# THU-DA-6D-Pose-Group/GDR-Net

Hardware: NVIDIA B200
Metric: crops/sec (fwd+bwd, 256x256, bs64 per GPU) (higher is better)
Workload: dtype fp16x3 fwd / fp16 bwd, f32 accumulate

## Files before the change

### gdr_net_b200/csrc/elementwise.cu

```cuda
#include <stdlib.h>

#include "gdrn_internal.h"
#include "ptx.cuh"

namespace gdrn {

typedef __nv_bfloat16 bf16;

__device__ __forceinline__ void unpack8(const uint4& q, float (&f)[8]) {
    const uint32_t w[4] = {q.x, q.y, q.z, q.w};
#pragma unroll
    for (int j = 0; j < 4; ++j) {
        unpack_hi2(w[j], f[2 * j], f[2 * j + 1]);
    }
}
__device__ __forceinline__ void load8(const bf16* hi, const bf16* lo, long off8, float (&f)[8]) {
    unpack8(__ldg(reinterpret_cast<const uint4*>(hi) + off8), f);
    if (lo != nullptr) {
        const uint4 q = __ldg(reinterpret_cast<const uint4*>(lo) + off8);
        const uint32_t w[4] = {q.x, q.y, q.z, q.w};
#pragma unroll
        for (int j = 0; j < 4; ++j) {
            float a, b;
            unpack_lo2(w[j], a, b);
// ... 127 lines not shown
                    if (LO) unpack8_lo(rl[t], r);
#pragma unroll
                    for (int j = 0; j < 8; ++j) v[j] += r[j];
                }
                if (relu) {
                    if (mask_out != nullptr) {
                        uint32_t bits = 0;
#pragma unroll
                        for (int j = 0; j < 8; ++j) bits |= (v[j] > 0.f ? 1u : 0u) << j;
                        mask_out[it] = (uint8_t)bits;
                    }
#pragma unroll
                    for (int j = 0; j < 8; ++j) v[j] = fmaxf(v[j], 0.f);
                }
                store8(y_hi, LO ? y_lo : nullptr, it, v);
            }
        }
    }
}

template <bool LO, bool RES>
__global__ void __launch_bounds__(256, 4) bn_act_kernel(const bf16* __restrict__ x_hi, const bf16* __restrict__ x_lo,
                                                        const bf16* __restrict__ r_hi, const bf16* __restrict__ r_lo,
                                                        bf16* __restrict__ y_hi, bf16* __restrict__ y_lo,
                                                        const float* __restrict__ scale, const float* __restrict__ shift,
                                                        long rows, int C, int relu) {
    pdl_ew_entry();
    __shared__ float s_sc[512], s_sh[512];
    for (int c = threadIdx.x; c < C; c += blockDim.x) {
        s_sc[c] = scale[c];
        s_sh[c] = shift[c];
    }
    __syncthreads();
    bn_apply_loop<LO, RES>(x_hi, x_lo, r_hi, r_lo, y_hi, y_lo, s_sc, s_sh, rows * (C / 8), C / 8, relu, nullptr);
}

template <bool LO, bool RES>
__global__ void __launch_bounds__(256, 4) bn_fwd_kernel(const bf16* __restrict__ x_hi, const bf16* __restrict__ x_lo,
                                                        const bf16* __restrict__ r_hi, const bf16* __restrict__ r_lo,
                                                        bf16* __restrict__ y_hi, bf16* __restrict__ y_lo,
                                                        const float* __restrict__ stats, const float* __restrict__ gamma,
                                                        const float* __restrict__ beta, float* running_mean, float* running_var,
                                                        float* __restrict__ mean_out, float* __restrict__ invstd_out, long rows,
                                                        int C, float eps, float momentum, int train, int relu,
                                                        uint8_t* __restrict__ mask_out, int rev) {
    pdl_ew_entry();
    __shared__ float s_sc[512], s_sh[512];
    const float count = (float)rows;
    for (int c = threadIdx.x; c < C; c += blockDim.x) {
        float mean, var;
        if (train) {
            const double m = (double)stats[c] / count;
            double v = (double)stats[C + c] / count - m * m;
            if (v < 0) v = 0;
            mean = (float)m;
            var = (float)v;
        } else {
            mean = running_mean[c];
            var = running_var[c];
        }
        const float invstd = rsqrtf(var + eps);
        const float sc = gamma[c] * invstd;
        s_sc[c] = sc;
        s_sh[c] = beta[c] - mean * sc;
        if (blockIdx.x == 0) {
            if (mean_out != nullptr) {
                mean_out[c] = mean;
                invstd_out[c] = invstd;
            }
            if (train && running_mean != nullptr) {
                running_mean[c] = (1.f - momentum) * running_mean[c] + momentum * mean;
                const float unbiased = count > 1.f ? var * (count / (count - 1.f)) : var;
                running_var[c] = (1.f - momentum) * running_var[c] + momentum * unbiased;
            }
        }
    }
    __syncthreads();
    bn_apply_loop<LO, RES>(x_hi, x_lo, r_hi, r_lo, y_hi, y_lo, s_sc, s_sh, rows * (C / 8), C / 8, relu, mask_out, rev != 0);
}


struct Pix {
    int g, x, y, b;
};
__device__ __forceinline__ bool is_pow2(int v) { return v > 0 && (v & (v - 1)) == 0; }
__device__ __forceinline__ Pix decode_pix(long idx, int cg, int W, int H) {
    unsigned t = (unsigned)idx;
    Pix p;
    if (is_pow2(cg) && is_pow2(W) && is_pow2(H)) {
        const int lc = 31 - __clz(cg), lw = 31 - __clz(W), lh = 31 - __clz(H);
        p.g = (int)(t & (unsigned)(cg - 1));
        t >>= lc;
        p.x = (int)(t & (unsigned)(W - 1));
        t >>= lw;
        p.y = (int)(t & (unsigned)(H - 1));
        p.b = (int)(t >> lh);
        return p;
    }
    unsigned q = t / (unsigned)cg;
    p.g = (int)(t - q * (unsigned)cg);
    t = q;
    q = t / (unsigned)W;
    p.x = (int)(t - q * (unsigned)W);
    t = q;
    q = t / (unsigned)H;
    p.y = (int)(t - q * (unsigned)H);
    p.b = (int)q;
    return p;
}

__global__ void maxpool_fwd_kernel(const bf16* __restrict__ x_hi, const bf16* __restrict__ x_lo, bf16* __restrict__ y_hi,
                                   bf16* __restrict__ y_lo, uint8_t* __restrict__ arg_out, int B, int H, int W, int C) {
    pdl_ew_entry();
    const int cg = C / 8, Ho = H / 2, Wo = W / 2;
    const long total = (long)B * Ho * Wo * cg;
    for (long idx = blockIdx.x * (long)blockDim.x + threadIdx.x; idx < total; idx += (long)gridDim.x * blockDim.x) {
        const Pix px = decode_pix(idx, cg, Wo, Ho);
        const int g = px.g, ox = px.x, oy = px.y, b = px.b;
        float m[8];
        uint32_t arg[8];
#pragma unroll
        for (int j = 0; j < 8; ++j) {
            m[j] = -INFINITY;
            arg[j] = 0;
        }
#pragma unroll
        for (int dy = 0; dy < 3; ++dy) {
            const int iy = oy * 2 + dy - 1;
            if (iy < 0 || iy >= H) continue;
#pragma unroll
            for (int dx = 0; dx < 3; ++dx) {
                const int ix = ox * 2 + dx - 1;
                if (ix < 0 || ix >= W) continue;
                float v[8];
                load8(x_hi, x_lo, (((long)b * H + iy) * W + ix) * cg + g, v);
#pragma unroll
                for (int j = 0; j < 8; ++j)
                    if (v[j] > m[j]) {
                        m[j] = v[j];
                        arg[j] = dy * 3 + dx;
                    }
            }
        }
        store8(y_hi, y_lo, idx, m);
        if (arg_out != nullptr) {
            uint2 packed;
            packed.x = arg[0] | (arg[1] << 8) | (arg[2] << 16) | (arg[3] << 24);
            packed.y = arg[4] | (arg[5] << 8) | (arg[6] << 16) | (arg[7] << 24);
            reinterpret_cast<uint2*>(arg_out)[idx] = packed;
        }
    }
}

__global__ void maxpool_bwd_kernel(const uint8_t* __restrict__ arg_in, const bf16* __restrict__ g_hi,
                                   const bf16* __restrict__ g_lo, bf16* __restrict__ dx_hi, bf16* __restrict__ dx_lo, int B, int H,
                                   int W, int C) {
    pdl_ew_entry();
    const int cg = C / 8, Ho = H / 2, Wo = W / 2;
    const long total = (long)B * H * W * cg;
    for (long idx = blockIdx.x * (long)blockDim.x + threadIdx.x; idx < total; idx += (long)gridDim.x * blockDim.x) {
        const Pix px = decode_pix(idx, cg, W, H);
        const int g = px.g, ix = px.x, iy = px.y, b = px.b;
        float acc[8];
#pragma unroll
        for (int j = 0; j < 8; ++j) acc[j] = 0.f;
        const int oyA = iy >> 1, oyB = (iy + 1) >> 1, oxA = ix >> 1, oxB = (ix + 1) >> 1;
        const bool vyB = (oyB != oyA) && (oyB < Ho), vxB = (oxB != oxA) && (oxB < Wo);
        const int oys[2] = {oyA, vyB ? oyB : oyA}, oxs[2] = {oxA, vxB ? oxB : oxA};
        uint2 codes[4];
        uint4 gh[4], gl[4];
#pragma unroll
        for (int q = 0; q < 4; ++q) {
            const long o = (((long)b * Ho + oys[q >> 1]) * Wo + oxs[q & 1]) * cg + g;
            codes[q] = __ldg(reinterpret_cast<const uint2*>(arg_in) + o);
            gh[q] = ld16(g_hi, o);
            if (g_lo != nullptr) gl[q] = ld16(g_lo, o);
        }
#pragma unroll
        for (int q = 0; q < 4; ++q) {
            const bool valid = ((q >> 1) == 0 || vyB) && ((q & 1) == 0 || vxB);
            if (!valid) continue;
            const uint32_t code = (uint32_t)((iy - (oys[q >> 1] * 2 - 1)) * 3 + (ix - (oxs[q & 1] * 2 - 1)));
            float gv[8];
            unpack8(gh[q], gv);
            if (g_lo != nullptr) unpack8_lo(gl[q], gv);
#pragma unroll
            for (int j = 0; j < 8; ++j) {
                const uint32_t aj = ((j < 4 ? codes[q].x : codes[q].y) >> (8 * (j & 3))) & 0xffu;
                if (aj == code) acc[j] += gv[j];
            }
        }
        store8(dx_hi, dx_lo, idx, acc);
    }
}

__global__ void upsample2x_fwd_kernel(const bf16* __restrict__ x_hi, const bf16* __restrict__ x_lo, bf16* __restrict__ y_hi,
                                      bf16* __restrict__ y_lo, int B, int H, int W, int C) {
    pdl_ew_entry();
    const int cg = C / 8, Ho = 2 * H, Wo = 2 * W;
    const float sh = (float)(H - 1) / (float)(Ho - 1), sw = (float)(W - 1) / (float)(Wo - 1);
    const long total = (long)B * Ho * Wo * cg;
    for (long idx = blockIdx.x * (long)blockDim.x + threadIdx.x; idx < total; idx += (long)gridDim.x * blockDim.x) {
        const Pix px = decode_pix(idx, cg, Wo, Ho);
        const int g = px.g, ox = px.x, oy = px.y, b = px.b;
        const float fy = sh * oy, fx = sw * ox;
        const int y0 = (int)fy, x0 = (int)fx;
        const int y1 = y0 + (y0 < H - 1 ? 1 : 0), x1 = x0 + (x0 < W - 1 ? 1 : 0);
        const float ly1 = fy - y0, lx1 = fx - x0, ly0 = 1.f - ly1, lx0 = 1.f - lx1;
        float v00[8], v01[8], v10[8], v11[8], o[8];
        const long base = (long)b * H;
        load8(x_hi, x_lo, ((base + y0) * W + x0) * cg + g, v00);
        load8(x_hi, x_lo, ((base + y0) * W + x1) * cg + g, v01);
        load8(x_hi, x_lo, ((base + y1) * W + x0) * cg + g, v10);
        load8(x_hi, x_lo, ((base + y1) * W + x1) * cg + g, v11);
#pragma unroll
        for (int j = 0; j < 8; ++j) o[j] = ly0 * (lx0 * v00[j] + lx1 * v01[j]) + ly1 * (lx0 * v10[j] + lx1 * v11[j]);
        store8(y_hi, y_lo, idx, o);
    }
}

__global__ void upsample2x_bwd_kernel(const bf16* __restrict__ g_hi, const bf16* __restrict__ g_lo, bf16* __restrict__ dx_hi,
                                      bf16* __restrict__ dx_lo, int B, int H, int W, int C) {
    pdl_ew_entry();
    const int cg = C / 8, Ho = 2 * H, Wo = 2 * W;
    const float sh = (float)(H - 1) / (float)(Ho - 1), sw = (float)(W - 1) / (float)(Wo - 1);
    const long total = (long)B * H * W * cg;
    for (long idx = blockIdx.x * (long)blockDim.x + threadIdx.x; idx < total; idx += (long)gridDim.x * blockDim.x) {
        const Pix px = decode_pix(idx, cg, W, H);
        const int g = px.g, ix = px.x, iy = px.y, b = px.b;
        float acc[8];
#pragma unroll
        for (int j = 0; j < 8; ++j) acc[j] = 0.f;
        const int oy0 = 2 * iy - 2, ox0 = 2 * ix - 2;
        float wxs[6];
#pragma unroll
        for (int c = 0; c < 6; ++c) {
            const int ox = ox0 + c;
            float wx = 0.f;
            if (ox >= 0 && ox < Wo) {
                const float fx = sw * ox;
                const int x0 = (int)fx;
                const int x1 = x0 + (x0 < W - 1 ? 1 : 0);
                const float lx1 = fx - x0, lx0 = 1.f - lx1;
                if (x0 == ix) wx += lx0;
                if (x1 == ix) wx += lx1;
            }
            wxs[c] = wx;
        }
        for (int r = 0; r < 6; ++r) {
            const int oy = oy0 + r;
            if (oy < 0 || oy >= Ho) continue;
            const float fy = sh * oy;
            const int y0 = (int)fy;
            const int y1 = y0 + (y0 < H - 1 ? 1 : 0);
            const float ly1 = fy - y0, ly0 = 1.f - ly1;
            float wy = 0.f;
            if (y0 == iy) wy += ly0;
            if (y1 == iy) wy += ly1;
            if (wy == 0.f) continue;
            const long rowbase = (((long)b * Ho + oy) * Wo + ox0) * cg + g;
            uint4 vh[6], vl[6];
#pragma unroll
            for (int c = 0; c < 6; ++c) {
                if (wxs[c] != 0.f) {
                    vh[c] = ld16(g_hi, rowbase + (long)c * cg);
                    if (g_lo != nullptr) vl[c] = ld16(g_lo, rowbase + (long)c * cg);
                }
            }
#pragma unroll
            for (int c = 0; c < 6; ++c) {
                if (wxs[c] != 0.f) {
                    float gv[8];
                    unpack8(vh[c], gv);
                    if (g_lo != nullptr) unpack8_lo(vl[c], gv);
                    const float w = wy * wxs[c];
#pragma unroll
                    for (int j = 0; j < 8; ++j) acc[j] = fmaf(w, gv[j], acc[j]);
                }
            }
        }
        store8(dx_hi, dx_lo, idx, acc);
    }
}

__global__ void zero_insert_kernel(const bf16* __restrict__ x_hi, const bf16* __restrict__ x_lo, bf16* __restrict__ y_hi,
                                   bf16* __restrict__ y_lo, int B, int H, int W, int C, int mode) {
    pdl_ew_entry();
    const int cg = C / 8;
    const int Hy = mode == 0 ? 2 * H : H, Wy = mode == 0 ? 2 * W : W;
    const long total = (long)B * Hy * Wy * cg;
    for (long idx = blockIdx.x * (long)blockDim.x + threadIdx.x; idx < total; idx += (long)gridDim.x * blockDim.x) {
        const int g = (int)(idx % cg);
        long t = idx / cg;
        const int x = (int)(t % Wy);
        t /= Wy;
        const int y = (int)(t % Hy);
        const int b = (int)(t / Hy);
        uint4 h = make_uint4(0, 0, 0, 0), l = make_uint4(0, 0, 0, 0);
        if (mode == 0) {
            if (((x | y) & 1) == 0) {
                const long s = (((long)b * H + (y >> 1)) * W + (x >> 1)) * cg + g;
                h = __ldg(reinterpret_cast<const uint4*>(x_hi) + s);
                if (x_lo != nullptr) l = __ldg(reinterpret_cast<const uint4*>(x_lo) + s);
            }
        } else {
            const long s = (((long)b * 2 * H + 2 * y) * 2 * W + 2 * x) * cg + g;
            h = __ldg(reinterpret_cast<const uint4*>(x_hi) + s);
            if (x_lo != nullptr) l = __ldg(reinterpret_cast<const uint4*>(x_lo) + s);
        }
        reinterpret_cast<uint4*>(y_hi)[idx] = h;
        if (y_lo != nullptr) reinterpret_cast<uint4*>(y_lo)[idx] = l;
    }
}

constexpr int kBnBwdThreads = 256;
constexpr int kRedRows = 4;

template <bool LO>
__device__ __forceinline__ void masked_grad(const uint4& gah, const uint4& gal, const uint4& gbh, const uint4& gbl, const uint4& yh,
                                            bool has_gb, bool has_y, float (&g)[8], bool has_bits = false, uint32_t bits = 0) {
    unpack8(gah, g);
    if (LO) unpack8_lo(gal, g);
    if (has_gb) {
        float t[8];
        unpack8(gbh, t);
        if (LO) unpack8_lo(gbl, t);
#pragma unroll
        for (int j = 0; j < 8; ++j) g[j] += t[j];
    }
    if (has_bits) {
#pragma unroll
        for (int j = 0; j < 8; ++j) g[j] = ((bits >> j) & 1u) ? g[j] : 0.f;
    } else if (has_y) {
        float y[8];
        unpack8(yh, y);
#pragma unroll
        for (int j = 0; j < 8; ++j) g[j] = y[j] > 0.f ? g[j] : 0.f;
    }
}
__device__ __forceinline__ void lds8(const float* p, float (&v)[8]) {
    const float4 a = *reinterpret_cast<const float4*>(p), b = *reinterpret_cast<const float4*>(p + 4);
    v[0] = a.x; v[1] = a.y; v[2] = a.z; v[3] = a.w;
    v[4] = b.x; v[5] = b.y; v[6] = b.z; v[7] = b.w;
}
__device__ __forceinline__ void mask_from_u(const float (&u)[8], const float* sc_, const float* sh_, float (&g)[8]) {
    float sc[8], sh[8];
    lds8(sc_, sc);
    lds8(sh_, sh);
#pragma unroll
    for (int j = 0; j < 8; ++j) g[j] = fmaf(sc[j], u[j], sh[j]) > 0.f ? g[j] : 0.f;
}

template <bool LO, bool MASKU>
__global__ void __launch_bounds__(kBnBwdThreads, 2) bn_bwd_reduce_kernel(
    const bf16* __restrict__ ga_hi, const bf16* __restrict__ ga_lo, const bf16* __restrict__ gb_hi,
    const bf16* __restrict__ gb_lo, const bf16* __restrict__ y_hi, const bf16* __restrict__ u_hi,
    const bf16* __restrict__ u_lo, const float* __restrict__ mean, const float* __restrict__ invstd,
    const float* __restrict__ gamma, const float* __restrict__ beta, float* __restrict__ sums, long rows, int C,
    const uint8_t* __restrict__ mask_in, float* __restrict__ partial_out) {
    pdl_ew_entry();
    const int cg = C / 8;
    const int rpb = kBnBwdThreads / cg;
    const int g = threadIdx.x % cg;
    const int rl = threadIdx.x / cg;
    __shared__ __align__(16) float s_mu[512], s_is[512], s_sc[512], s_sh[512];
    __shared__ float red[2][kBnBwdThreads][8 + 1];
    for (int c = threadIdx.x; c < C; c += kBnBwdThreads) {
        s_mu[c] = mean[c];
        s_is[c] = invstd[c];
        if (MASKU) {
            const float sc = gamma[c] * invstd[c];
            s_sc[c] = sc;
            s_sh[c] = beta[c] - mean[c] * sc;
        }
    }
    __syncthreads();
    const bool has_bits = !MASKU && mask_in != nullptr;
    const bool has_gb = gb_hi != nullptr, has_y = !MASKU && !has_bits && y_hi != nullptr;
    float s0[8], s1[8];
#pragma unroll
    for (int j = 0; j < 8; ++j) s0[j] = s1[j] = 0.f;
    const long rstride = (long)gridDim.x * rpb;
    for (long r0 = (long)blockIdx.x * rpb + rl; r0 < rows; r0 += kRedRows * rstride) {
        uint4 gah[kRedRows], gal[kRedRows], gbh[kRedRows], gbl[kRedRows], yh[kRedRows], uh[kRedRows], ul[kRedRows];
        uint32_t mb[kRedRows] = {};
#pragma unroll
        for (int t = 0; t < kRedRows; ++t) {
            const long r = r0 + t * rstride;
            if (r < rows) {
                const long off = r * cg + g;
                gah[t] = ld16(ga_hi, off);
                uh[t] = ld16(u_hi, off);
                if (has_bits) mb[t] = __ldg(mask_in + off);
                if (has_y) yh[t] = ld16(y_hi, off);
                if (has_gb) gbh[t] = ld16(gb_hi, off);
                if (LO) {
                    gal[t] = ld16(ga_lo, off);
                    ul[t] = ld16(u_lo, off);
                    if (has_gb) gbl[t] = ld16(gb_lo, off);
                }
            }
        }
#pragma unroll
        for (int t = 0; t < kRedRows; ++t) {
            const long r = r0 + t * rstride;
            if (r < rows) {
                float gv[8], u[8];
                masked_grad<LO>(gah[t], gal[t], gbh[t], gbl[t], yh[t], has_gb, has_y, gv, has_bits, mb[t]);
                unpack8(uh[t], u);
                if (LO) unpack8_lo(ul[t], u);
                if (MASKU) mask_from_u(u, s_sc + g * 8, s_sh + g * 8, gv);
                float mu[8], is[8];
                lds8(s_mu + g * 8, mu);
                lds8(s_is + g * 8, is);
#pragma unroll
                for (int j = 0; j < 8; ++j) {
                    s0[j] += gv[j];
                    s1[j] = fmaf(gv[j], (u[j] - mu[j]) * is[j], s1[j]);
                }
            }
        }
    }
#pragma unroll
    for (int j = 0; j < 8; ++j) {
        red[0][threadIdx.x][j] = s0[j];
        red[1][threadIdx.x][j] = s1[j];
    }
    __syncthreads();
    for (int t = threadIdx.x; t < 2 * C; t += kBnBwdThreads) {
        const int which = t / C, c = t % C;
        const int gg = c / 8, j = c % 8;
        float a = 0.f;
        for (int q = 0; q < rpb; ++q) a += red[which][q * cg + gg][j];
        if (partial_out != nullptr) partial_out[((long)blockIdx.x * 2 + which) * C + c] = a;
        else atomicAdd(sums + which * C + c, a);
    }
}

template <bool LO>
__global__ void __launch_bounds__(kBnBwdThreads, 3) bn_stats_partial_kernel(const bf16* __restrict__ u_hi, const bf16* __restrict__ u_lo,
                                                                            float* __restrict__ partials, long rows, int C) {
    const int cg = C / 8;
    const int rpb = kBnBwdThreads / cg;
    const int g = threadIdx.x % cg, rl = threadIdx.x / cg;
    __shared__ float red[2][kBnBwdThreads][8 + 1];
    float s0[8], s1[8];
#pragma unroll
    for (int j = 0; j < 8; ++j) s0[j] = s1[j] = 0.f;
    const long rstride = (long)gridDim.x * rpb;
    for (long r = (long)blockIdx.x * rpb + rl; r < rows; r += rstride) {
        float v[8];
        const long off = r * cg + g;
        unpack8(ld16(u_hi, off), v);
        if (LO) unpack8_lo(ld16(u_lo, off), v);
#pragma unroll
        for (int j = 0; j < 8; ++j) {
            s0[j] += v[j];
            s1[j] = fmaf(v[j], v[j], s1[j]);
        }
    }
#pragma unroll
    for (int j = 0; j < 8; ++j) {
        red[0][threadIdx.x][j] = s0[j];
        red[1][threadIdx.x][j] = s1[j];
    }
    __syncthreads();
    for (int t = threadIdx.x; t < 2 * C; t += kBnBwdThreads) {
        const int which = t / C, c = t % C;
        float a = 0.f;
        for (int q = 0; q < rpb; ++q) a += red[which][q * cg + c / 8][c % 8];
        partials[((long)blockIdx.x * 2 + which) * C + c] = a;
    }
}
__global__ void sum_partials_kernel(const float* __restrict__ partials, int nparts, int n, float* __restrict__ out) {
    const int i = blockIdx.x * blockDim.x + threadIdx.x;
    if (i >= n) return;
    double a = 0.0;
    for (int p = 0; p < nparts; ++p) a += (double)partials[(long)p * n + i];
    out[i] = (float)a;
}

template <bool LO, bool MASKU>
__global__ void __launch_bounds__(256, 4) bn_bwd_apply_kernel(
    const bf16* __restrict__ ga_hi, const bf16* __restrict__ ga_lo, const bf16* __restrict__ gb_hi,
    const bf16* __restrict__ gb_lo, const bf16* __restrict__ y_hi, const bf16* __restrict__ u_hi,
    const bf16* __restrict__ u_lo, const float* __restrict__ mean, const float* __restrict__ invstd,
    const float* __restrict__ gamma, const float* __restrict__ beta, const float* __restrict__ sums, bf16* __restrict__ du_hi,
    bf16* __restrict__ du_lo, bf16* __restrict__ gout_hi, bf16* __restrict__ gout_lo, float* __restrict__ dgamma,
    float* __restrict__ dbeta, long rows, int C, int train, const uint8_t* __restrict__ mask_in, int rev) {
    pdl_ew_entry();
    __shared__ __align__(16) float s_k1[512], s_k2[512], s_k3[512], s_sc[512], s_sh[512];
    const int cg = C / 8;
    const long total = rows * cg;
    const float inv_n = 1.f / (float)rows;
    for (int c = threadIdx.x; c < C; c += blockDim.x) {
        const float is = invstd[c];
        const float k1 = gamma[c] * is;
        float k2 = 0.f, k3 = 0.f;
        if (train) {
            const float m0 = sums[c] * inv_n, m1 = sums[C + c] * inv_n;
            k2 = -k1 * is * m1;
            k3 = k1 * (mean[c] * is * m1 - m0);
        }
        s_k1[c] = k1;
        s_k2[c] = k2;
        s_k3[c] = k3;
        if (MASKU) {
            s_sc[c] = k1;
            s_sh[c] = beta[c] - mean[c] * k1;
        }
        if (blockIdx.x == 0 && dgamma != nullptr) {
            dbeta[c] = sums[c];
            dgamma[c] = sums[C + c];
        }
    }
    __syncthreads();
    const bool has_bits = !MASKU && mask_in != nullptr;
    const bool has_gb = gb_hi != nullptr, has_y = !MASKU && !has_bits && y_hi != nullptr, has_gout = gout_hi != nullptr;
    const long stride = (long)gridDim.x * blockDim.x;
    const long first = blockIdx.x * (long)blockDim.x + threadIdx.x;
    const int c0 = (rev ? cg - 1 - (int)(first % cg) : (int)(first % cg)) * 8;
    for (long idx = first; idx < total; idx += 2 * stride) {
        uint4 gah[2], gal[2], gbh[2], gbl[2], yh[2], uh[2], ul[2];
        uint32_t mb[2] = {0, 0};
#pragma unroll
        for (int t = 0; t < 2; ++t) {
            const long it0 = idx + t * stride;
            const long it = rev ? total - 1 - it0 : it0;
            if (it0 < total) {
                gah[t] = ld16(ga_hi, it);
                uh[t] = ld16(u_hi, it);
                if (has_bits) mb[t] = __ldg(mask_in + it);
                if (has_y) yh[t] = ld16(y_hi, it);
                if (has_gb) gbh[t] = ld16(gb_hi, it);
                if (LO) {
                    gal[t] = ld16(ga_lo, it);
                    ul[t] = ld16(u_lo, it);
                    if (has_gb) gbl[t] = ld16(gb_lo, it);
                }
            }
        }
#pragma unroll
        for (int t = 0; t < 2; ++t) {
            const long it0 = idx + t * stride;
            const long it = rev ? total - 1 - it0 : it0;
            if (it0 < total) {
                float gv[8], u[8], o[8];
                masked_grad<LO>(gah[t], gal[t], gbh[t], gbl[t], yh[t], has_gb, has_y, gv, has_bits, mb[t]);
                unpack8(uh[t], u);
                if (LO) unpack8_lo(ul[t], u);
                if (MASKU) mask_from_u(u, s_sc + c0, s_sh + c0, gv);
                float k1[8], k2[8], k3[8];
                lds8(s_k1 + c0, k1);
                lds8(s_k2 + c0, k2);
                lds8(s_k3 + c0, k3);
#pragma unroll
                for (int j = 0; j < 8; ++j) o[j] = fmaf(k1[j], gv[j], fmaf(k2[j], u[j], k3[j]));
                store8(du_hi, LO ? du_lo : nullptr, it, o);
                if (has_gout) store8(gout_hi, LO ? gout_lo : nullptr, it, gv);
            }
        }
    }
}

constexpr int kGnCluster = 4;
__device__ __forceinline__ unsigned gn_cluster_rank() {
    unsigned r;
    asm volatile("mov.u32 %0, %%cluster_ctarank;" : "=r"(r));
    return r;
}
__device__ __forceinline__ void gn_cluster_sync() {
    asm volatile("barrier.cluster.arrive.release.aligned;\n\tbarrier.cluster.wait.acquire.aligned;" ::: "memory");
}
__device__ __forceinline__ double gn_remote_f64(const double* local_smem_ptr, unsigned rank) {
    const unsigned a = (unsigned)__cvta_generic_to_shared(local_smem_ptr);
    unsigned ra;
    asm volatile("mapa.shared::cluster.u32 %0, %1, %2;" : "=r"(ra) : "r"(a), "r"(rank));
    double v;
    asm volatile("ld.shared::cluster.f64 %0, [%1];" : "=d"(v) : "r"(ra) : "memory");
    return v;
}

__global__ void __launch_bounds__(256) gn_relu_fwd_kernel(const bf16* __restrict__ u_hi, const bf16* __restrict__ u_lo,
                                                          bf16* __restrict__ y_hi, bf16* __restrict__ y_lo,
                                                          const float* __restrict__ gamma, const float* __restrict__ beta,
                                                          float* __restrict__ stats, int HW, int C, int G, float eps, int ncl) {
    pdl_ew_entry();
    const int b = blockIdx.x / ncl;
    const unsigned crank = ncl > 1 ? gn_cluster_rank() : 0u;
    const int cg = C / 8;
    const int g = threadIdx.x % cg;
    const int rl = threadIdx.x / cg;
    const int rpb = 256 / cg;
    const int cpg = C / G;
    const int rows = HW / ncl, r_begin = (int)crank * rows;
    __shared__ float sm[2][256][8 + 1];
    __shared__ float gstat[64][2];
    __shared__ double part[64][2];
    float s0[8], s1[8];
#pragma unroll
    for (int j = 0; j < 8; ++j) s0[j] = s1[j] = 0.f;
    const long base = (long)b * HW * cg;
    for (int r = r_begin + rl; r < r_begin + rows; r += rpb) {
        float v[8];
        load8(u_hi, u_lo, base + (long)r * cg + g, v);
#pragma unroll
        for (int j = 0; j < 8; ++j) {
            s0[j] += v[j];
            s1[j] = fmaf(v[j], v[j], s1[j]);
        }
    }
#pragma unroll
    for (int j = 0; j < 8; ++j) {
        sm[0][threadIdx.x][j] = s0[j];
        sm[1][threadIdx.x][j] = s1[j];
    }
    __syncthreads();
    if (threadIdx.x < G) {
        const int grp = threadIdx.x;
        double a0 = 0, a1 = 0;
        for (int c = grp * cpg; c < (grp + 1) * cpg; ++c) {
            const int gg = c / 8, j = c % 8;
            for (int q = 0; q < rpb; ++q) {
                a0 += sm[0][q * cg + gg][j];
                a1 += sm[1][q * cg + gg][j];
            }
        }
        part[grp][0] = a0;
        part[grp][1] = a1;
    }
    if (ncl > 1) gn_cluster_sync(); else __syncthreads();
    if (threadIdx.x < G) {
// ... 122 lines not shown
        gred[grp][1] = (float)(a1 / n);
    }
    __syncthreads();
    for (int r = r_begin + rl; r < r_begin + rows; r += rpb) {
        const long off = base + (long)r * cg + g;
        float gv[8], y[8], u[8], o[8];
        load8(g_hi, g_lo, off, gv);
        unpack8(__ldg(reinterpret_cast<const uint4*>(y_hi) + off), y);
        load8(u_hi, u_lo, off, u);
#pragma unroll
        for (int j = 0; j < 8; ++j) {
            const int grp = (g * 8 + j) / cpg;
            const float gg = y[j] > 0.f ? gv[j] : 0.f;
            const float xh = (u[j] - mu[j]) * rs[j];
            o[j] = rs[j] * (gg * ga[j] - gred[grp][0] - xh * gred[grp][1]);
        }
        store8(du_hi, du_lo, off, o);
    }
    if (ncl > 1) gn_cluster_sync();
}

__global__ void add2_kernel(const bf16* __restrict__ a_hi, const bf16* __restrict__ a_lo, const bf16* __restrict__ b_hi,
                            const bf16* __restrict__ b_lo, bf16* __restrict__ o_hi, bf16* __restrict__ o_lo, long n8) {
    pdl_ew_entry();
    for (long idx = blockIdx.x * (long)blockDim.x + threadIdx.x; idx < n8; idx += (long)gridDim.x * blockDim.x) {
        float a[8], b[8];
        load8(a_hi, a_lo, idx, a);
        load8(b_hi, b_lo, idx, b);
#pragma unroll
        for (int j = 0; j < 8; ++j) a[j] += b[j];
        store8(o_hi, o_lo, idx, a);
    }
}

__global__ void f32_to_planes_kernel(const float* __restrict__ x, bf16* __restrict__ y_hi, bf16* __restrict__ y_lo, long n8) {
    for (long idx = blockIdx.x * (long)blockDim.x + threadIdx.x; idx < n8; idx += (long)gridDim.x * blockDim.x) {
        const float4 a = __ldg(reinterpret_cast<const float4*>(x) + 2 * idx), b = __ldg(reinterpret_cast<const float4*>(x) + 2 * idx + 1);
        const float v[8] = {a.x, a.y, a.z, a.w, b.x, b.y, b.z, b.w};
        store8(y_hi, y_lo, idx, v);
    }
}
__global__ void planes_to_f32_kernel(const bf16* __restrict__ x_hi, const bf16* __restrict__ x_lo, float* __restrict__ y, long n8) {
    for (long idx = blockIdx.x * (long)blockDim.x + threadIdx.x; idx < n8; idx += (long)gridDim.x * blockDim.x) {
        float v[8];
        load8(x_hi, x_lo, idx, v);
        reinterpret_cast<float4*>(y)[2 * idx] = make_float4(v[0], v[1], v[2], v[3]);
        reinterpret_cast<float4*>(y)[2 * idx + 1] = make_float4(v[4], v[5], v[6], v[7]);
    }
}


__global__ void __launch_bounds__(256) colsum_kernel(const bf16* __restrict__ x_hi, const bf16* __restrict__ x_lo,
                                                     float* __restrict__ out, long rows, int ld) {
    pdl_ew_entry();
    const int cg = ld / 8;
    const int rpb = 256 / cg;
    const int g = threadIdx.x % cg, rl = threadIdx.x / cg;
    float s[8];
#pragma unroll
    for (int j = 0; j < 8; ++j) s[j] = 0.f;
    if (rl < rpb) {
        for (long r = (long)blockIdx.x * rpb + rl; r < rows; r += (long)gridDim.x * rpb) {
            float v[8];
            load8(x_hi, x_lo, r * cg + g, v);
#pragma unroll
            for (int j = 0; j < 8; ++j) s[j] += v[j];
        }
    }
    __shared__ float red[256][8 + 1];
#pragma unroll
    for (int j = 0; j < 8; ++j) red[threadIdx.x][j] = s[j];
    __syncthreads();
    for (int c = threadIdx.x; c < ld; c += 256) {
        float a = 0.f;
        for (int q = 0; q < rpb; ++q) a += red[q * cg + c / 8][c % 8];
        atomicAdd(out + c, a);
    }
}

__global__ void leaky_bwd_kernel(const bf16* __restrict__ g_hi, const bf16* __restrict__ g_lo, const bf16* __restrict__ y_hi,
                                 bf16* __restrict__ o_hi, bf16* __restrict__ o_lo, long n8) {
    pdl_ew_entry();
    for (long idx = blockIdx.x * (long)blockDim.x + threadIdx.x; idx < n8; idx += (long)gridDim.x * blockDim.x) {
        float g[8], y[8];
        load8(g_hi, g_lo, idx, g);
        unpack8(__ldg(reinterpret_cast<const uint4*>(y_hi) + idx), y);
#pragma unroll
        for (int j = 0; j < 8; ++j) g[j] = y[j] > 0.f ? g[j] : 0.1f * g[j];
        store8(o_hi, o_lo, idx, g);
    }
}

}

using namespace gdrn;
#define STREAM cudaStream_t stream = reinterpret_cast<cudaStream_t>(stream_)
#define BF(p) reinterpret_cast<bf16*>(p)
#define CBF(p) reinterpret_cast<const bf16*>(p)
#define LAUNCH_DONE()                  \
    GDRN_CUDA_OK(cudaGetLastError()); \
    count_launch();                    \
    return 0

static int bn_reverse() {
    static int v = -1;
    if (v < 0) {
        const char* e = getenv("GDRN_BN_REVERSE");
        v = e ? atoi(e) : 1;
    }
    return v;
}

extern "C" int gdrn_bn_finalize(const float* stats, const float* gamma, const float* beta, float* running_mean,
                                float* running_var, float* scale, float* shift, float* mean_out, float* invstd_out, int C,
                                float count, float eps, float momentum, int train, void* stream_) {
    STREAM;
    bn_finalize_kernel<<<(C + 127) / 128, 128, 0, stream>>>(stats, gamma, beta, running_mean, running_var, scale, shift,
                                                          mean_out, invstd_out, C, count, eps, momentum, train);
    LAUNCH_DONE();
}

extern "C" int gdrn_bn_fold_batched(const void* jobs_dev, int njobs, void* stream_) {
    STREAM;
    static_assert(sizeof(BnFoldJob) == 64, "BnFoldJob layout is mirrored by the host (gdr_net_b200/engine.py)");
    if (njobs <= 0) return 0;
    bn_fold_batched_kernel<<<dim3(njobs, 2), 256, 0, stream>>>(reinterpret_cast<const BnFoldJob*>(jobs_dev));
    LAUNCH_DONE();
}

extern "C" int gdrn_bn_act(const void* x_hi, const void* x_lo, const void* r_hi, const void* r_lo, void* y_hi, void* y_lo,
                           const float* scale, const float* shift, long rows, int C, int relu, void* stream_) {
    STREAM;
    if (C % 8) return set_error(GDRN_ERR_ARG, "bn_act: C %% 8 != 0");
    if (C > 512 || 256 % (C / 8)) return set_error(GDRN_ERR_ARG, "bn_act: unsupported C=%d", C);
    const int grid = ew_grid_amortised(rows * (C / 8), 256, 4);
#define GDRN_BN_ACT(LO, RES) \
    GDRN_LAUNCH_PDL_FWD((bn_act_kernel<LO, RES>), grid, 256, 0, stream, CBF(x_hi), CBF(x_lo), CBF(r_hi), CBF(r_lo), BF(y_hi), BF(y_lo), scale, shift, rows, C, relu)
    if (x_lo != nullptr) {
        if (r_hi != nullptr) GDRN_BN_ACT(true, true); else GDRN_BN_ACT(true, false);
    } else {
        if (r_hi != nullptr) GDRN_BN_ACT(false, true); else GDRN_BN_ACT(false, false);
    }
#undef GDRN_BN_ACT
    LAUNCH_DONE();
}

extern "C" int gdrn_maxpool_fwd(const void* x_hi, const void* x_lo, void* y_hi, void* y_lo, void* arg_out, int B, int H,
                                int W, int C, void* stream_) {
    STREAM;
    GDRN_LAUNCH_PDL_FWD(maxpool_fwd_kernel, ew_grid((long)B * (H / 2) * (W / 2) * (C / 8), 256), 256, 0, stream, 
        CBF(x_hi), CBF(x_lo), BF(y_hi), BF(y_lo), reinterpret_cast<uint8_t*>(arg_out), B, H, W, C);
    LAUNCH_DONE();
}
extern "C" int gdrn_maxpool_bwd(const void* arg_in, const void* g_hi, const void* g_lo, void* dx_hi, void* dx_lo, int B,
                                int H, int W, int C, void* stream_) {
    STREAM;
    GDRN_LAUNCH_PDL(maxpool_bwd_kernel, ew_grid((long)B * H * W * (C / 8), 256), 256, 0, stream, 
        reinterpret_cast<const uint8_t*>(arg_in), CBF(g_hi), CBF(g_lo), BF(dx_hi), BF(dx_lo), B, H, W, C);
    LAUNCH_DONE();
}
extern "C" int gdrn_upsample2x_fwd(const void* x_hi, const void* x_lo, void* y_hi, void* y_lo, int B, int H, int W, int C,
                                   void* stream_) {
    STREAM;
    GDRN_LAUNCH_PDL_FWD(upsample2x_fwd_kernel, ew_grid((long)B * 4 * H * W * (C / 8), 256), 256, 0, stream, CBF(x_hi), CBF(x_lo), BF(y_hi),
                                                                                           BF(y_lo), B, H, W, C);
    LAUNCH_DONE();
}
extern "C" int gdrn_upsample2x_bwd(const void* g_hi, const void* g_lo, void* dx_hi, void* dx_lo, int B, int H, int W, int C,
                                   void* stream_) {
    STREAM;
    GDRN_LAUNCH_PDL(upsample2x_bwd_kernel, ew_grid((long)B * H * W * (C / 8), 256), 256, 0, stream, CBF(g_hi), CBF(g_lo), BF(dx_hi),
                                                                                       BF(dx_lo), B, H, W, C);
    LAUNCH_DONE();
}
extern "C" int gdrn_zero_insert(const void* x_hi, const void* x_lo, void* y_hi, void* y_lo, int B, int H, int W, int C,
                                int mode, void* stream_) {
    STREAM;
    const long total = (long)B * H * W * (C / 8) * (mode == 0 ? 4 : 1);
    GDRN_LAUNCH_PDL_FWD(zero_insert_kernel, ew_grid(total, 256), 256, 0, stream, CBF(x_hi), CBF(x_lo), BF(y_hi), BF(y_lo), B, H, W, C, mode);
    LAUNCH_DONE();
}

extern "C" int gdrn_bn_bwd(const void* ga_hi, const void* ga_lo, const void* gb_hi, const void* gb_lo, const void* y_hi,
                           const void* u_hi, const void* u_lo, const float* mean, const float* invstd, const float* gamma,
                           const float* beta, float* sums, void* du_hi, void* du_lo, void* gout_hi, void* gout_lo,
                           float* dgamma, float* dbeta, const void* relu_mask, float* det_ws, long rows, int C, int train,
                           int flags, void* stream_) {
    STREAM;
    const uint8_t* mask_in = reinterpret_cast<const uint8_t*>(relu_mask);
    const bool det = (flags & 4) != 0;
    if (det && det_ws == nullptr) return set_error(GDRN_ERR_ARG, "bn_bwd: deterministic mode needs a workspace of 2*C*%d floats", 2 * num_sms());
    if (C % 64 || C > 512) return set_error(GDRN_ERR_ARG, "bn_bwd: unsupported C=%d", C);
    const int mask_u = flags & 1;
    if (mask_u && (y_hi != nullptr || beta == nullptr)) return set_error(GDRN_ERR_ARG, "bn_bwd: mask-from-u needs beta and no y");
    {
        if (!(flags & 2) && !det) GDRN_CUDA_OK(cudaMemsetAsync(sums, 0, sizeof(float) * 2 * C, stream));
        const int rpb = kBnBwdThreads / (C / 8);
        long blocks = (rows + (long)rpb * 16 - 1) / ((long)rpb * 16);
        const long cap = (long)num_sms() * 2;
        if (blocks > cap) blocks = cap;
        if (blocks < 1) blocks = 1;
#define GDRN_BN_RED(LO, MU)                                                                                                   \
    GDRN_LAUNCH_PDL((bn_bwd_reduce_kernel<LO, MU>), (int)blocks, kBnBwdThreads, 0, stream, CBF(ga_hi), CBF(ga_lo), CBF(gb_hi), CBF(gb_lo),       \
                                                                            CBF(y_hi), CBF(u_hi), CBF(u_lo), mean, invstd, gamma, \
                                                                            beta, sums, rows, C, mask_in, det ? det_ws : nullptr)
        if (u_lo != nullptr) {
            if (mask_u) GDRN_BN_RED(true, true); else GDRN_BN_RED(true, false);
        } else {
            if (mask_u) GDRN_BN_RED(false, true); else GDRN_BN_RED(false, false);
        }
#undef GDRN_BN_RED
        GDRN_CUDA_OK(cudaGetLastError());
        count_launch();
        if (det) {
            sum_partials_kernel<<<(2 * C + 255) / 256, 256, 0, stream>>>(det_ws, (int)blocks, 2 * C, sums);
            GDRN_CUDA_OK(cudaGetLastError());
            count_launch();
        }
    }
    const int agrid = ew_grid_amortised(rows * (C / 8), 256, 4);
#define GDRN_BN_APP(LO, MU)                                                                                                      \
    GDRN_LAUNCH_PDL((bn_bwd_apply_kernel<LO, MU>), agrid, 256, 0, stream, CBF(ga_hi), CBF(ga_lo), CBF(gb_hi), CBF(gb_lo), CBF(y_hi), CBF(u_hi),    \
                                                           CBF(u_lo), mean, invstd, gamma, beta, sums, BF(du_hi), BF(du_lo),       \
                                                           BF(gout_hi), BF(gout_lo), dgamma, dbeta, rows, C, train, mask_in, bn_reverse())
    if (u_lo != nullptr) {
        if (mask_u) GDRN_BN_APP(true, true); else GDRN_BN_APP(true, false);
    } else {
        if (mask_u) GDRN_BN_APP(false, true); else GDRN_BN_APP(false, false);
    }
#undef GDRN_BN_APP
    LAUNCH_DONE();
}

extern "C" int gdrn_det_parts() { return 2 * num_sms(); }
extern "C" int gdrn_bn_stats(const void* u_hi, const void* u_lo, float* ws, float* stats, long rows, int C, void* stream_) {
    STREAM;
    if (C % 64 || C > 512) return set_error(GDRN_ERR_ARG, "bn_stats: unsupported C=%d", C);
    const int rpb = kBnBwdThreads / (C / 8);
    long blocks = (rows + (long)rpb * 16 - 1) / ((long)rpb * 16);
    const long cap = (long)num_sms() * 2;
    if (blocks > cap) blocks = cap;
    if (blocks < 1) blocks = 1;
    if (u_lo != nullptr) bn_stats_partial_kernel<true><<<(int)blocks, kBnBwdThreads, 0, stream>>>(CBF(u_hi), CBF(u_lo), ws, rows, C);
    else bn_stats_partial_kernel<false><<<(int)blocks, kBnBwdThreads, 0, stream>>>(CBF(u_hi), CBF(u_lo), ws, rows, C);
    GDRN_CUDA_OK(cudaGetLastError());
    count_launch();
    sum_partials_kernel<<<(2 * C + 255) / 256, 256, 0, stream>>>(ws, (int)blocks, 2 * C, stats);
    LAUNCH_DONE();
}

extern "C" int gdrn_gn_relu_fwd(const void* u_hi, const void* u_lo, void* y_hi, void* y_lo, const float* gamma,
                                const float* beta, float* stats, int B, int HW, int C, int G, float eps, void* stream_) {
    STREAM;
    if (C != 128 || G > 64 || C % G) return set_error(GDRN_ERR_ARG, "gn_relu_fwd: only C=128 supported");
    const int ncl = (HW % (kGnCluster * 16) == 0) ? kGnCluster : 1;
    cudaLaunchConfig_t cfg;
    memset(&cfg, 0, sizeof(cfg));
    cfg.gridDim = dim3(B * ncl);
    cfg.blockDim = dim3(256);
    cfg.stream = stream;
    cudaLaunchAttribute attr[1];
    attr[0].id = cudaLaunchAttributeClusterDimension;
    attr[0].val.clusterDim.x = ncl;
    attr[0].val.clusterDim.y = 1;
    attr[0].val.clusterDim.z = 1;
    cfg.attrs = attr;
    cfg.numAttrs = 1;
    GDRN_CUDA_OK(cudaLaunchKernelEx(&cfg, gn_relu_fwd_kernel, CBF(u_hi), CBF(u_lo), BF(y_hi), BF(y_lo), gamma, beta, stats, HW, C, G, eps, ncl));
    count_launch();
    return 0;
}
extern "C" int gdrn_gn_relu_bwd(const void* g_hi, const void* g_lo, const void* y_hi, const void* u_hi, const void* u_lo,
                                const float* gamma, const float* stats, void* du_hi, void* du_lo, float* dgamma,
                                float* dbeta, int B, int HW, int C, int G, void* stream_) {
    STREAM;
    if (C != 128 || G > 64 || C % G) return set_error(GDRN_ERR_ARG, "gn_relu_bwd: only C=128 supported");
    const int ncl = (HW % (kGnCluster * 16) == 0) ? kGnCluster : 1;
    cudaLaunchConfig_t cfg;
    memset(&cfg, 0, sizeof(cfg));
    cfg.gridDim = dim3(B * ncl);
    cfg.blockDim = dim3(256);
    cfg.stream = stream;
    cudaLaunchAttribute attr[1];
    attr[0].id = cudaLaunchAttributeClusterDimension;
    attr[0].val.clusterDim.x = ncl;
    attr[0].val.clusterDim.y = 1;
    attr[0].val.clusterDim.z = 1;
    cfg.attrs = attr;
    cfg.numAttrs = 1;
    GDRN_CUDA_OK(cudaLaunchKernelEx(&cfg, gn_relu_bwd_kernel, CBF(g_hi), CBF(g_lo), CBF(y_hi), CBF(u_hi), CBF(u_lo), gamma, stats,
                                    BF(du_hi), BF(du_lo), dgamma, dbeta, HW, C, G, ncl));
    count_launch();
    return 0;
}
extern "C" int gdrn_add2(const void* a_hi, const void* a_lo, const void* b_hi, const void* b_lo, void* o_hi, void* o_lo,
                         long n, void* stream_) {
    STREAM;
    GDRN_LAUNCH_PDL(add2_kernel, ew_grid(n / 8, 256), 256, 0, stream, CBF(a_hi), CBF(a_lo), CBF(b_hi), CBF(b_lo), BF(o_hi), BF(o_lo), n / 8);
    LAUNCH_DONE();
}
extern "C" int gdrn_f32_to_planes(const float* x, void* y_hi, void* y_lo, long n, void* stream_) {
    STREAM;
    f32_to_planes_kernel<<<ew_grid(n / 8, 256), 256, 0, stream>>>(x, BF(y_hi), BF(y_lo), n / 8);
    LAUNCH_DONE();
}
extern "C" int gdrn_planes_to_f32(const void* x_hi, const void* x_lo, float* y, long n, void* stream_) {
    STREAM;
    planes_to_f32_kernel<<<ew_grid(n / 8, 256), 256, 0, stream>>>(CBF(x_hi), CBF(x_lo), y, n / 8);
    LAUNCH_DONE();
}

extern "C" int gdrn_colsum(const void* x_hi, const void* x_lo, float* out, long rows, int ld, void* stream_) {
    STREAM;
    if (ld % 8 || ld / 8 > 256 || 256 % (ld / 8)) return set_error(GDRN_ERR_ARG, "colsum: unsupported ld=%d", ld);
    GDRN_CUDA_OK(cudaMemsetAsync(out, 0, sizeof(float) * ld, stream));
    const int rpb = 256 / (ld / 8);
    long blocks = (rows + rpb - 1) / rpb;
    const long cap = (long)num_sms() * 4;
    if (blocks > cap) blocks = cap;
    if (blocks < 1) blocks = 1;
    GDRN_LAUNCH_PDL(colsum_kernel, (int)blocks, 256, 0, stream, CBF(x_hi), CBF(x_lo), out, rows, ld);
    LAUNCH_DONE();
}
extern "C" int gdrn_leaky_bwd(const void* g_hi, const void* g_lo, const void* y_hi, void* o_hi, void* o_lo, long n,
                              void* stream_) {
    STREAM;
    GDRN_LAUNCH_PDL(leaky_bwd_kernel, ew_grid(n / 8, 256), 256, 0, stream, CBF(g_hi), CBF(g_lo), CBF(y_hi), BF(o_hi), BF(o_lo), n / 8);
    LAUNCH_DONE();
}

extern "C" int gdrn_bn_fwd(const void* x_hi, const void* x_lo, const void* r_hi, const void* r_lo, void* y_hi, void* y_lo,
                           const float* stats, const float* gamma, const float* beta, float* running_mean, float* running_var,
                           float* mean_out, float* invstd_out, void* relu_mask_out, long rows, int C, float eps, float momentum,
                           int train, int relu, void* stream_) {
    STREAM;
    if (C % 8 || C > 512 || 256 % (C / 8)) return set_error(GDRN_ERR_ARG, "bn_fwd: unsupported C=%d", C);
    if (train && stats == nullptr) return set_error(GDRN_ERR_ARG, "bn_fwd: batch statistics missing");
    const int grid = ew_grid_amortised(rows * (C / 8), 256, 4);
#define GDRN_BN_FWD(LO, RES)                                                                                                  \
    GDRN_LAUNCH_PDL_FWD((bn_fwd_kernel<LO, RES>), grid, 256, 0, stream, CBF(x_hi), CBF(x_lo), CBF(r_hi), CBF(r_lo), BF(y_hi), BF(y_lo), stats, gamma, beta, \
                                                     running_mean, running_var, mean_out, invstd_out, rows, C, eps, momentum, train, relu,  \
                                                     reinterpret_cast<uint8_t*>(relu_mask_out), bn_reverse())
    if (x_lo != nullptr) {
        if (r_hi != nullptr) GDRN_BN_FWD(true, true); else GDRN_BN_FWD(true, false);
    } else {
        if (r_hi != nullptr) GDRN_BN_FWD(false, true); else GDRN_BN_FWD(false, false);
    }
#undef GDRN_BN_FWD
// ... 3 lines not shown
```

### gdr_net_b200/csrc/gdrn_internal.h

```cpp
#pragma once
#include <cuda.h>
#include <cuda_bf16.h>
#include <cuda_runtime.h>
#include <stdint.h>
#include <stdio.h>
#include <string.h>

#define GDRN_OK 0
#define GDRN_ERR_ARG (-1)
#define GDRN_ERR_CUDA (-2)

namespace gdrn {

int set_error(int code, const char* fmt, ...);
int cuda_error(cudaError_t e, const char* file, int line);
int num_sms();
void count_launch();
bool pdl_enabled();
bool pdl_ew_enabled(bool forward_kernel);
void set_pdl(int on);

int make_tmap(CUtensorMap* out, const void* base, int rank, const uint64_t* dims, const uint64_t* strides_bytes,
              const uint32_t* box);

}

#ifdef __CUDACC__
namespace gdrn {
template <typename... KArgs, typename... Args>
inline cudaError_t launch_pdl(bool forward_kernel, void (*kernel)(KArgs...), dim3 grid, dim3 block, size_t smem, cudaStream_t stream,
                              Args&&... args) {
    cudaLaunchConfig_t cfg;
    memset(&cfg, 0, sizeof(cfg));
    cfg.gridDim = grid;
    cfg.blockDim = block;
    cfg.dynamicSmemBytes = smem;
    cfg.stream = stream;
    cudaLaunchAttribute attr[1];
    int na = 0;
    if (pdl_ew_enabled(forward_kernel)) {
        attr[0].id = cudaLaunchAttributeProgrammaticStreamSerialization;
        attr[0].val.programmaticStreamSerializationAllowed = 1;
        na = 1;
    }
    cfg.attrs = attr;
    cfg.numAttrs = na;
    return cudaLaunchKernelEx(&cfg, kernel, static_cast<KArgs>(args)...);
}
}
#define GDRN_LAUNCH_PDL(kernel, grid, block, smem, stream, ...) \
    (void)gdrn::launch_pdl(false, kernel, dim3(grid), dim3(block), smem, stream, __VA_ARGS__)
#define GDRN_LAUNCH_PDL_FWD(kernel, grid, block, smem, stream, ...) \
    (void)gdrn::launch_pdl(true, kernel, dim3(grid), dim3(block), smem, stream, __VA_ARGS__)
#endif

#ifndef GDRN_LAUNCH_SMEM
#define GDRN_LAUNCH_SMEM(kernel, grid, block, smem, stream, ...) kernel<<<grid, block, smem, stream>>>(__VA_ARGS__)
#endif

#define GDRN_CUDA_OK(expr)                                                      \
    do {                                                                        \
        cudaError_t _e = (expr);                                                \
        if (_e != cudaSuccess) return gdrn::cuda_error(_e, __FILE__, __LINE__); \
    } while (0)
```

### gdr_net_b200/csrc/gemm_epilogue.cuh

```cuda
#pragma once
#include "gdrn_internal.h"
#include "gemm_params.h"
#include "ptx.cuh"

namespace gdrn {

template <int BLOCK_N, int NSPLIT, int NMAIN>
__device__ __forceinline__ void gemm_epilogue_tile(const GemmParams& p, uint32_t t_acc, int lane, int row, int m_tile, int n_tile, int ph,
                                                   int c_begin, int c_end, float* tr, float* s_stats) {
    __nv_bfloat16* out_hi = reinterpret_cast<__nv_bfloat16*>(p.out_hi);
    __nv_bfloat16* out_lo = reinterpret_cast<__nv_bfloat16*>(p.out_lo);
    const long mrow = (long)m_tile * 128 + row;
    const bool row_ok = mrow < p.M;
    const bool all_rows = (long)(m_tile + 1) * 128 <= p.M;
    long grow = mrow;
    if (p.nphase) {
        const long j = mrow & ((1L << p.pw_log2) - 1);
        const long t = mrow >> p.pw_log2;
        const long i = t & ((1L << p.ph_log2) - 1);
        const long n = t >> p.ph_log2;
        grow = (((n << (p.ph_log2 + 1)) + 2 * i + p.ph_a[ph]) << (p.pw_log2 + 1)) + 2 * j + p.ph_b[ph];
    }
#pragma unroll 1
    for (int c = c_begin; c < c_end; ++c) {
        const int col0 = n_tile * BLOCK_N + c * 32;
        if (col0 >= p.N) continue;
        float f[32];
        {
            const uint32_t t0 = t_acc + c * 32;
            uint32_t raw[32];
            tmem_ld_32x32(t0, raw);
            tmem_ld_wait();
#pragma unroll
            for (int j = 0; j < 32; ++j) f[j] = __uint_as_float(raw[j]);
            if (NSPLIT == 3) {
                const int nmain = p.num_kb < NMAIN ? p.num_kb : NMAIN;
                for (int a2 = 1; a2 <= NMAIN; ++a2) {
                    if (a2 < NMAIN && a2 >= nmain) continue;
                    tmem_ld_32x32(t0 + a2 * BLOCK_N, raw);
                    tmem_ld_wait();
                    const float sc = (a2 == NMAIN) ? kLoInvScale : 1.f;
#pragma unroll
                    for (int j = 0; j < 32; ++j) f[j] = fmaf(__uint_as_float(raw[j]), sc, f[j]);
                }
            }
        }
        const bool full_chunk = (col0 + 32 <= p.N);
        if (p.bias != nullptr) {
#pragma unroll
            for (int j = 0; j < 32; ++j)
                if (full_chunk || col0 + j < p.N) f[j] += __ldg(p.bias + col0 + j);
        }
        if (p.res_hi != nullptr && row_ok && full_chunk) {
            const __nv_bfloat16* rh = reinterpret_cast<const __nv_bfloat16*>(p.res_hi) + grow * p.ldc + col0;
            const __nv_bfloat16* rl = p.res_lo ? reinterpret_cast<const __nv_bfloat16*>(p.res_lo) + grow * p.ldc + col0 : nullptr;
#pragma unroll
            for (int j = 0; j < 4; ++j) {
                const uint4 rq = __ldg(reinterpret_cast<const uint4*>(rh) + j);
                const uint32_t w[4] = {rq.x, rq.y, rq.z, rq.w};
#pragma unroll
                for (int t = 0; t < 4; ++t) {
                    float a, b;
                    unpack_hi2(w[t], a, b);
                    f[8 * j + 2 * t] += a;
                    f[8 * j + 2 * t + 1] += b;
                }
                if (rl != nullptr) {
                    const uint4 q2 = __ldg(reinterpret_cast<const uint4*>(rl) + j);
                    const uint32_t w2[4] = {q2.x, q2.y, q2.z, q2.w};
#pragma unroll
                    for (int t = 0; t < 4; ++t) {
                        float a, b;
                        unpack_lo2(w2[t], a, b);
                        f[8 * j + 2 * t] += a;
                        f[8 * j + 2 * t + 1] += b;
                    }
                }
            }
        }
        if (p.act == 1) {
#pragma unroll
            for (int j = 0; j < 32; ++j) f[j] = f[j] > 0.f ? f[j] : 0.1f * f[j];
        } else if (p.act == 2) {
#pragma unroll
            for (int j = 0; j < 32; ++j) f[j] = fmaxf(f[j], 0.f);
        }
        if (row_ok) {
            if (p.out_f32 != nullptr) {
                float* dst = p.out_f32 + grow * p.ldc + col0;
                if (full_chunk) {
#pragma unroll
                    for (int j = 0; j < 32; j += 4)
                        *reinterpret_cast<float4*>(dst + j) = make_float4(f[j], f[j + 1], f[j + 2], f[j + 3]);
                } else {
#pragma unroll
                    for (int j = 0; j < 32; ++j)
                        if (col0 + j < p.ldc) dst[j] = (col0 + j < p.N) ? f[j] : 0.f;
                }
            }
            if (out_hi != nullptr) {
                uint32_t hi[16], lo[16];
#pragma unroll
                for (int j = 0; j < 16; ++j) {
                    float a = f[2 * j], b = f[2 * j + 1];
                    if (!full_chunk) {
                        if (col0 + 2 * j >= p.N) a = 0.f;
                        if (col0 + 2 * j + 1 >= p.N) b = 0.f;
                    }
                    if (out_lo != nullptr) split2(a, b, hi[j], lo[j]); else hi[j] = pack_hi2(a, b);
                }
                const int ncopy = full_chunk ? 4 : ((min(p.ldc, col0 + 32) - col0) / 8);
                uint4* dh = reinterpret_cast<uint4*>(out_hi + grow * p.ldc + col0);
#pragma unroll
                for (int j = 0; j < 4; ++j)
                    if (j < ncopy) dh[j] = make_uint4(hi[4 * j], hi[4 * j + 1], hi[4 * j + 2], hi[4 * j + 3]);
                if (out_lo != nullptr) {
                    uint4* dl = reinterpret_cast<uint4*>(out_lo + grow * p.ldc + col0);
#pragma unroll
                    for (int j = 0; j < 4; ++j)
                        if (j < ncopy)
                            dl[j] = make_uint4(lo[4 * j], lo[4 * j + 1], lo[4 * j + 2], lo[4 * j + 3]);
                }
            }
        }
        if (p.stats != nullptr) {
#pragma unroll
            for (int h = 0; h < 2; ++h) {
                if (all_rows) {
#pragma unroll
                    for (int j = 0; j < 16; ++j) tr[lane * 17 + j] = f[h * 16 + j];
                } else {
#pragma unroll
                    for (int j = 0; j < 16; ++j) tr[lane * 17 + j] = row_ok ? f[h * 16 + j] : 0.f;
                }
                __syncwarp();
                float s1 = 0.f, s2 = 0.f;
                const int col = lane & 15, r0 = (lane >> 4) * 16;
#pragma unroll
                for (int i = 0; i < 16; ++i) {
                    const float v = tr[(r0 + i) * 17 + col];
                    s1 += v;
                    s2 = fmaf(v, v, s2);
                }
                s1 += __shfl_xor_sync(0xffffffffu, s1, 16);
                s2 += __shfl_xor_sync(0xffffffffu, s2, 16);
                __syncwarp();
                if (lane < 16) {
                    atomicAdd(&s_stats[c * 32 + h * 16 + lane], s1);
                    atomicAdd(&s_stats[BLOCK_N + c * 32 + h * 16 + lane], s2);
                }
            }
        }
    }
}

}
```

### gdr_net_b200/csrc/gemm_fwd.cu

```cuda
#include <stdlib.h>

#include <atomic>

#include "gdrn_internal.h"
#include "gemm_epilogue.cuh"
#include "gemm_params.h"
#include "ptx.cuh"

namespace gdrn {

constexpr int kBlockM = 128;
constexpr int kBlockK = 64;
constexpr int kSmemBudget = 227 * 1024;
constexpr int kEpiWarps = 8;
constexpr int kTrBytes = kEpiWarps * 32 * 17 * 4;
constexpr int kAuxBytes = 4096 + kTrBytes;

template <int BLOCK_N, int NSPLIT>
struct GemmCfg {
    static constexpr int NPL = (NSPLIT == 1) ? 1 : 2;
    static constexpr int A_BYTES = kBlockM * kBlockK * 2;
    static constexpr int B_BYTES = BLOCK_N * kBlockK * 2;
    static constexpr int STAGE_BYTES = NPL * (A_BYTES + B_BYTES);
    static constexpr int STAGES_RAW = (kSmemBudget - kAuxBytes - 1024) / STAGE_BYTES;
// ... 197 lines not shown
#pragma unroll
                        for (int k = 0; k < kBlockK / 16; ++k) {
                            const uint32_t ac = (k == 0) ? accum : 1u;
                            if (NSPLIT == 3) {
                                umma_bf16(d_main, da + 2 * k, db + 2 * k, idesc_wide, ac);
                                umma_bf16(d_cross, da + (Cfg::A_BYTES >> 4) + 2 * k, db + 2 * k, idesc, 1u);
                            } else {
                                umma_bf16(d_main, da + 2 * k, db + 2 * k, idesc, ac);
                            }
                        }
                        umma_commit_u32(empty0 + stage * 8);
                    }
                    __syncwarp();
                    accum = 1u;
                    if (++stage == STAGES) {
                        stage = 0;
                        phase ^= 1;
                    }
                }
                if (elect_one()) umma_commit_u32(tfull0 + acc * 8);
                __syncwarp();
            }
        }
    } else if (warp >= 4) {
        const int q = warp & 3;
        const int grp = (warp - 4) >> 2;
        const int row = q * 32 + lane;
        float* tr = s_tr + (warp - 4) * (32 * 17);
        constexpr int NCH = BLOCK_N / 32;
        const bool split_epi = num_groups <= num_clusters && !p.no_split_epi;
        const int c_begin = split_epi ? grp * (NCH / 2) : 0;
        const int c_end = split_epi ? (grp + 1) * (NCH / 2) : NCH;
        for (int tg = split_epi ? my_cluster : my_cluster + grp * num_clusters, it = split_epi ? 0 : grp; tg < num_groups;
             tg += 2 * num_clusters, it += 2) {
            int rem = tg, ph = 0;
            if (p.nphase) {
                ph = tg / num_tiles;
                rem = tg - ph * num_tiles;
            }
            const int n_tile = rem % p.num_n_tiles;
            const int m_tile = rem / p.num_n_tiles;
            const int acc = it & 1;
            const uint32_t acc_phase = (it >> 1) & 1;
            mbar_wait(&tfull_bar[acc], acc_phase);
            tc_fence_after();
            gemm_epilogue_tile<BLOCK_N, NSPLIT, Cfg::NMAIN>(p, tmem_base + ((uint32_t)(q * 32) << 16) + acc * Cfg::NACC * BLOCK_N, lane, row,
                                                            m_tile, n_tile, ph, c_begin, c_end, tr, s_stats);
            tc_fence_before();
            __syncwarp();
            if (lane == 0 && !(split_epi && grp == 1)) mbar_arrive(&tempty_bar[acc]);
        }
        if (p.stats != nullptr) {
            asm volatile("bar.sync 1, 256;" ::: "memory");
            const int n_tile = my_cluster % p.num_n_tiles;
            for (int i = threadIdx.x - 128; i < BLOCK_N; i += 256) {
                const int col = n_tile * BLOCK_N + i;
                if (col < p.N) {
                    atomicAdd(p.stats + col, s_stats[i]);
                    atomicAdd(p.stats + p.N + col, s_stats[BLOCK_N + i]);
                }
            }
        }
    }

    tc_fence_before();
    __syncthreads();
    if (warp == 2) {
        tc_fence_after();
        tmem_dealloc(tmem_base, Cfg::TMEM_COLS);
    }
}

template <int BLOCK_N, int NSPLIT>
static int launch_gemm(const GemmParams& p, cudaStream_t stream) {
    using Cfg = GemmCfg<BLOCK_N, NSPLIT>;
    auto kern = gemm_fwd_kernel<BLOCK_N, NSPLIT>;
    static bool attr_set = false;
    if (!attr_set) {
        GDRN_CUDA_OK(cudaFuncSetAttribute(kern, cudaFuncAttributeMaxDynamicSharedMemorySize, Cfg::SMEM_BYTES));
        attr_set = true;
    }
    const int groups = (p.nphase ? p.nphase : 1) * p.num_m_tiles * p.num_n_tiles;
    int clusters = groups < num_sms() ? groups : num_sms();
    clusters -= clusters % p.num_n_tiles;
    if (clusters <= 0) clusters = p.num_n_tiles;
    cudaLaunchConfig_t cfg;
    memset(&cfg, 0, sizeof(cfg));
    cfg.gridDim = dim3(clusters);
    cfg.blockDim = dim3(128 + 32 * kEpiWarps);
    cfg.dynamicSmemBytes = Cfg::SMEM_BYTES;
    cfg.stream = stream;
    cudaLaunchAttribute attr[2];
    attr[0].id = cudaLaunchAttributeClusterDimension;
    attr[0].val.clusterDim.x = 1;
    attr[0].val.clusterDim.y = 1;
    attr[0].val.clusterDim.z = 1;
    int na = 1;
    if (pdl_enabled()) {
        attr[na].id = cudaLaunchAttributeProgrammaticStreamSerialization;
        attr[na].val.programmaticStreamSerializationAllowed = 1;
        ++na;
    }
    cfg.attrs = attr;
    cfg.numAttrs = na;
    GDRN_CUDA_OK(cudaLaunchKernelEx(&cfg, kern, p));
    count_launch();
    return 0;
}

static thread_local int g_last_variant = 0;

static int dispatch_gemm(const GemmParams& p_in, int block_n, int nsplit, cudaStream_t stream) {
    static int no_split = -1;
    if (no_split < 0) {
        const char* e = getenv("GDRN_NO_SPLIT_EPI");
        no_split = e ? atoi(e) : 0;
    }
    GemmParams p = p_in;
    p.no_split_epi = no_split;
    g_last_variant = block_n * 10 + nsplit;
    if (nsplit == 1) {
        if (block_n == 256) return launch_gemm<256, 1>(p, stream);
        if (block_n == 128) return launch_gemm<128, 1>(p, stream);
        if (block_n == 64) return launch_gemm<64, 1>(p, stream);
    } else if (nsplit == 3) {
        if (block_n == 128) return launch_gemm<128, 3>(p, stream);
        if (block_n == 64) return launch_gemm<64, 3>(p, stream);
    }
    return set_error(GDRN_ERR_ARG, "gemm: unsupported block_n=%d nsplit=%d", block_n, nsplit);
}

static int pick_block_n(int n_pad, int nsplit, int num_m_tiles) {
    const int want = (num_sms() * 3) / 4;
    if (nsplit == 1 && n_pad % 256 == 0 && num_m_tiles * (n_pad / 256) >= want) return 256;
    if (n_pad % 128 == 0 && num_m_tiles * (n_pad / 128) >= want) return 128;
    if (n_pad % 64 == 0 && num_m_tiles * (n_pad / 128) < num_sms() / 2) return 64;
    if (n_pad % 128 == 0) return 128;
    if (n_pad % 64 == 0) return 64;
    return -1;
}

static int g_2cta_mode = -1;
static std::atomic<long> g_2cta_launches{0};
static bool want_2cta(int nsplit, int block_n, int num_m_tiles, int num_n_tiles) {
    if (g_2cta_mode < 0) {
        const char* e = getenv("GDRN_2CTA");
        g_2cta_mode = e ? atoi(e) : 1;
    }
    if (g_2cta_mode != 1 || (num_m_tiles & 1)) return false;
    if (!((nsplit == 1 && (block_n == 256 || block_n == 128)) || (nsplit == 3 && block_n == 128))) return false;
    return (num_m_tiles / 2) * num_n_tiles * 4 >= num_sms();
}

}

using namespace gdrn;

extern "C" int gdrn_set_2cta(int on) {
    g_2cta_mode = on ? 1 : 0;
    return 0;
}
extern "C" long gdrn_2cta_launch_count() { return gdrn::g_2cta_launches.load(); }

extern "C" int gdrn_conv_fwd(const void* x_hi, const void* x_lo, const void* w_hi, const void* w_lo, void* y_hi,
                             void* y_lo, float* y_f32, const float* bias, const void* res_hi, const void* res_lo, float* stats,
                             int N, int H, int W, int Cin, int Cout, int Cout_pad, int KH, int KW, int stride, int pad, int ldc,
                             int act, int nsplit, void* stream_) {
    cudaStream_t stream = reinterpret_cast<cudaStream_t>(stream_);
    if (nsplit != 1 && nsplit != 3) return set_error(GDRN_ERR_ARG, "conv_fwd: nsplit must be 1 or 3");
    if (nsplit == 3 && (x_lo == nullptr || w_lo == nullptr)) return set_error(GDRN_ERR_ARG, "conv_fwd: lo planes missing");
    if (Cin % 64 != 0) return set_error(GDRN_ERR_ARG, "conv_fwd: Cin=%d must be a multiple of 64", Cin);
    if (stride != 1 && stride != 2) return set_error(GDRN_ERR_ARG, "conv_fwd: stride must be 1 or 2");
    if (H % stride || W % stride) return set_error(GDRN_ERR_ARG, "conv_fwd: H, W must be divisible by stride");
    if (ldc % 8 != 0 || ldc < Cout) return set_error(GDRN_ERR_ARG, "conv_fwd: bad ldc=%d", ldc);
    if (res_hi != nullptr && (Cout % 32 != 0 || y_hi == nullptr))
        return set_error(GDRN_ERR_ARG, "conv_fwd: a residual needs Cout %% 32 == 0 and a 16-bit output");
    if (act < 0 || act > 2) return set_error(GDRN_ERR_ARG, "conv_fwd: act must be 0 (none), 1 (LeakyReLU 0.1) or 2 (ReLU)");
    const int Ho = H / stride, Wo = W / stride;
    if (Wo > 128 || 128 % Wo != 0) return set_error(GDRN_ERR_ARG, "conv_fwd: unsupported output width %d", Wo);
    int TH = 128 / Wo;
    if (TH > Ho) TH = Ho;
    const int TN = 128 / (Wo * TH);
    if (Ho % TH != 0) return set_error(GDRN_ERR_ARG, "conv_fwd: Ho=%d not divisible by tile rows %d", Ho, TH);
    const int block_n = pick_block_n(Cout_pad, nsplit, (N * Ho * Wo + 127) / 128);
    if (block_n < 0) return set_error(GDRN_ERR_ARG, "conv_fwd: Cout_pad=%d must be a multiple of 64", Cout_pad);

    GemmParams p;
    memset(&p, 0, sizeof(p));
    const bool two_cta = want_2cta(nsplit, block_n, (N * Ho * Wo + 127) / 128, Cout_pad / block_n);
    const int cluster = two_cta ? 2 : 1;
    const int npl = nsplit == 1 ? 1 : 2;
    const void* xs[2] = {x_hi, x_lo};
    const void* ws[2] = {w_hi, w_lo};
    const int K = KH * KW * Cin;
    for (int pl = 0; pl < npl; ++pl) {
        const __nv_bfloat16* xb = reinterpret_cast<const __nv_bfloat16*>(xs[pl]);
        for (int ph = 0; ph < (stride == 2 ? 4 : 1); ++ph) {
            const int phh = ph >> 1, phw = ph & 1;
            uint64_t dims[4] = {(uint64_t)Cin, (uint64_t)Wo, (uint64_t)Ho, (uint64_t)N};
            uint64_t strides[3] = {(uint64_t)stride * Cin * 2, (uint64_t)stride * W * Cin * 2, (uint64_t)H * W * Cin * 2};
            uint32_t box[4] = {64, (uint32_t)Wo, (uint32_t)TH, (uint32_t)TN};
            const void* base = xb + ((size_t)phh * W + phw) * Cin;
            if (make_tmap(&p.tmA[pl][ph], base, 4, dims, strides, box)) return GDRN_ERR_CUDA;
        }
        uint64_t wdims[2] = {(uint64_t)K, (uint64_t)Cout_pad};
        uint64_t wstr[1] = {(uint64_t)K * 2};
        uint32_t wbox[2] = {64, (uint32_t)(block_n / cluster)};
        if (make_tmap(&p.tmB[pl], ws[pl], 2, wdims, wstr, wbox)) return GDRN_ERR_CUDA;
    }
    p.cluster = cluster;
    p.mode = 1;
    p.M = N * Ho * Wo;
    p.N = Cout;
    p.num_m_tiles = (p.M + 127) / 128;
    p.num_n_tiles = Cout_pad / block_n;
    p.cchunks = Cin / 64;
    p.num_kb = KH * KW * p.cchunks;
    p.KW = KW;
    p.pad = pad;
    p.stride = stride;
    p.TH = TH;
    p.TN = TN;
    p.tiles_per_img = (TN == 1) ? Ho / TH : 0;
    p.out_hi = y_hi;
    p.out_lo = y_lo;
    p.out_f32 = y_f32;
    p.ldc = ldc;
    p.bias = bias;
    p.res_hi = res_hi;
    p.res_lo = res_lo;
    p.act = act;
    p.stats = stats;
    if (two_cta) {
        g_2cta_launches.fetch_add(1, std::memory_order_relaxed);
        g_last_variant = 10000 + block_n * 10 + nsplit;
        return launch_gemm_2cta(p, block_n, nsplit, stream);
    }
    return dispatch_gemm(p, block_n, nsplit, stream);
}

extern "C" int gdrn_conv_dgrad_s2(const void* du_hi, const void* du_lo, const void* w_hi, const void* w_lo, void* dx_hi,
                                  void* dx_lo, const float* bias, float* stats, int N, int Ho, int Wo, int Cy, int Cx, int Cx_pad,
                                  int K, int pad, int ldc, int act, int nsplit, void* stream_) {
    cudaStream_t stream = reinterpret_cast<cudaStream_t>(stream_);
    if (nsplit != 1 && nsplit != 3) return set_error(GDRN_ERR_ARG, "conv_dgrad_s2: nsplit must be 1 or 3");
    if (nsplit == 3 && (du_lo == nullptr || w_lo == nullptr)) return set_error(GDRN_ERR_ARG, "conv_dgrad_s2: lo planes missing");
    if (!((K == 3 && pad == 1) || (K == 1 && pad == 0))) return set_error(GDRN_ERR_ARG, "conv_dgrad_s2: k3 p1 or k1 p0 only");
    if (Cy % 64 != 0) return set_error(GDRN_ERR_ARG, "conv_dgrad_s2: Cy=%d must be a multiple of 64", Cy);
    if (ldc % 8 != 0 || ldc < Cx) return set_error(GDRN_ERR_ARG, "conv_dgrad_s2: bad ldc=%d", ldc);
    if (Wo > 128 || 128 % Wo != 0 || (Ho & (Ho - 1)) != 0) return set_error(GDRN_ERR_ARG, "conv_dgrad_s2: unsupported dY size %dx%d", Ho, Wo);
    int TH = 128 / Wo;
    if (TH > Ho) TH = Ho;
    const int TN = 128 / (Wo * TH);
    if (Ho % TH != 0) return set_error(GDRN_ERR_ARG, "conv_dgrad_s2: Ho=%d not divisible by tile rows %d", Ho, TH);
    const int num_m_tiles = (N * Ho * Wo + 127) / 128;
    const int nphase = K == 3 ? 4 : 1;
    const int block_n = pick_block_n(Cx_pad, nsplit, num_m_tiles * nphase);
    if (block_n < 0) return set_error(GDRN_ERR_ARG, "conv_dgrad_s2: Cx_pad=%d must be a multiple of 64", Cx_pad);

    GemmParams p;
    memset(&p, 0, sizeof(p));
    const int npl = nsplit == 1 ? 1 : 2;
    const void* xs[2] = {du_hi, du_lo};
    const void* ws[2] = {w_hi, w_lo};
    const int Kw = K * K * Cy;
    for (int pl = 0; pl < npl; ++pl) {
        uint64_t dims[4] = {(uint64_t)Cy, (uint64_t)Wo, (uint64_t)Ho, (uint64_t)N};
        uint64_t strides[3] = {(uint64_t)Cy * 2, (uint64_t)Wo * Cy * 2, (uint64_t)Ho * Wo * Cy * 2};
        uint32_t box[4] = {64, (uint32_t)Wo, (uint32_t)TH, (uint32_t)TN};
        if (make_tmap(&p.tmA[pl][0], xs[pl], 4, dims, strides, box)) return GDRN_ERR_CUDA;
        uint64_t wdims[2] = {(uint64_t)Kw, (uint64_t)Cx_pad};
        uint64_t wstr[1] = {(uint64_t)Kw * 2};
        uint32_t wbox[2] = {64, (uint32_t)block_n};
        if (make_tmap(&p.tmB[pl], ws[pl], 2, wdims, wstr, wbox)) return GDRN_ERR_CUDA;
    }
    p.cluster = 1;
    p.mode = 1;
    p.M = N * Ho * Wo;
    p.N = Cx;
    p.num_m_tiles = num_m_tiles;
    p.num_n_tiles = Cx_pad / block_n;
    p.cchunks = Cy / 64;
    p.KW = K;
    p.pad = pad;
    p.stride = 1;
    p.TH = TH;
    p.TN = TN;
    p.tiles_per_img = (TN == 1) ? Ho / TH : 0;
    p.out_hi = dx_hi;
    p.out_lo = dx_lo;
    p.ldc = ldc;
    p.bias = bias;
    p.act = act;
    p.stats = stats;
    p.nphase = nphase;
    int nt = 0;
    const int order[4][2] = {{1, 1}, {1, 0}, {0, 1}, {0, 0}};
    for (int q = 0; q < nphase; ++q) {
        const int a = K == 3 ? order[q][0] : 0, b = K == 3 ? order[q][1] : 0;
        p.ph_a[q] = a;
        p.ph_b[q] = b;
        p.ph_tap0[q] = nt;
        for (int r = 0; r < K; ++r) {
            if ((a + pad - r) & 1) continue;
            for (int s2 = 0; s2 < K; ++s2) {
                if ((b + pad - s2) & 1) continue;
                p.tap_dh[nt] = (signed char)((a + pad - r) / 2);
                p.tap_dw[nt] = (signed char)((b + pad - s2) / 2);
                p.tap_w[nt] = (signed char)((K - 1 - r) * K + (K - 1 - s2));
                ++nt;
            }
        }
    }
    p.ph_tap0[nphase] = nt;
    p.num_kb = nt * p.cchunks;
    for (p.pw_log2 = 0; (1 << p.pw_log2) < Wo; ++p.pw_log2) {}
    for (p.ph_log2 = 0; (1 << p.ph_log2) < Ho; ++p.ph_log2) {}
    return dispatch_gemm(p, block_n, nsplit, stream);
}

extern "C" int gdrn_gemm_fwd(const void* a_hi, const void* a_lo, const void* w_hi, const void* w_lo, void* y_hi,
                             void* y_lo, float* y_f32, const float* bias, float* stats, int M, int N, int N_pad, int K,
                             int ldc, int act, int nsplit, void* stream_) {
    cudaStream_t stream = reinterpret_cast<cudaStream_t>(stream_);
    if (nsplit != 1 && nsplit != 3) return set_error(GDRN_ERR_ARG, "gemm_fwd: nsplit must be 1 or 3");
    if (nsplit == 3 && (a_lo == nullptr || w_lo == nullptr)) return set_error(GDRN_ERR_ARG, "gemm_fwd: lo planes missing");
    if (K % 64 != 0) return set_error(GDRN_ERR_ARG, "gemm_fwd: K=%d must be a multiple of 64", K);
    if (ldc % 8 != 0 || ldc < N) return set_error(GDRN_ERR_ARG, "gemm_fwd: bad ldc=%d", ldc);
    const int block_n = pick_block_n(N_pad, nsplit, (M + 127) / 128);
    if (block_n < 0) return set_error(GDRN_ERR_ARG, "gemm_fwd: N_pad=%d must be a multiple of 64", N_pad);
    GemmParams p;
    memset(&p, 0, sizeof(p));
    const int cluster = 1;
    const int npl = nsplit == 1 ? 1 : 2;
    const void* as[2] = {a_hi, a_lo};
    const void* ws[2] = {w_hi, w_lo};
    for (int pl = 0; pl < npl; ++pl) {
        uint64_t adims[2] = {(uint64_t)K, (uint64_t)M};
        uint64_t astr[1] = {(uint64_t)K * 2};
        uint32_t abox[2] = {64, 128};
        if (make_tmap(&p.tmA[pl][0], as[pl], 2, adims, astr, abox)) return GDRN_ERR_CUDA;
        uint64_t wdims[2] = {(uint64_t)K, (uint64_t)N_pad};
        uint32_t wbox[2] = {64, (uint32_t)(block_n / cluster)};
        if (make_tmap(&p.tmB[pl], ws[pl], 2, wdims, astr, wbox)) return GDRN_ERR_CUDA;
    }
    p.cluster = cluster;
    p.mode = 0;
    p.M = M;
    p.N = N;
    p.num_m_tiles = (M + 127) / 128;
    p.num_n_tiles = N_pad / block_n;
    p.num_kb = K / 64;
    p.out_hi = y_hi;
    p.out_lo = y_lo;
    p.out_f32 = y_f32;
    p.ldc = ldc;
    p.bias = bias;
    p.act = act;
    p.stats = stats;
    return dispatch_gemm(p, block_n, nsplit, stream);
}

extern "C" int gdrn_last_gemm_variant() { return g_last_variant; }
```

### gdr_net_b200/csrc/gemm_params.h

```cpp
#pragma once
#include <cuda.h>

namespace gdrn {

struct GemmParams {
    CUtensorMap tmA[2][4];
    CUtensorMap tmB[2];
    int mode;
    int M, N;
    int num_m_tiles, num_n_tiles, num_kb;
    int cchunks, KW, pad, stride;
    int tiles_per_img, TH, TN;
    void* out_hi;
    void* out_lo;
    float* out_f32;
    int ldc;
    const float* bias;
    const void* res_hi;
    const void* res_lo;
    int act;
    float* stats;
    int cluster;
    int nphase;
    int ph_tap0[5];
    int ph_a[4], ph_b[4];
    signed char tap_dh[12], tap_dw[12], tap_w[12];
    int pw_log2, ph_log2;
    int no_split_epi;
};


int launch_gemm_2cta(const GemmParams& p, int block_n, int nsplit, cudaStream_t stream);

}
```

### gdr_net_b200/engine.py

```python
from __future__ import annotations

from typing import Dict, List, Optional

import torch

from . import ops
from .capi import C
from .ops import PT, _stream

import os

_DGRAD_ZERO_INSERT = os.environ.get("GDRN_DGRAD_ZERO_INSERT") == "1"

_BN_MASK_FROM_U = os.environ.get("GDRN_BN_MASK_FROM_U") == "1"
_DECONV_PHASES = os.environ.get("GDRN_DECONV_PHASES", "1") == "1"
_BN_BITMASK = os.environ.get("GDRN_BN_BITMASK", "1") == "1"

LOSS_NAMES = ["loss_coor_x", "loss_coor_y", "loss_coor_z", "loss_mask", "loss_region", "loss_PM_R", "loss_centroid", "loss_z"]
HEAD_CONVS = [(3, 4, False), (6, 7, False), (10, 11, True), (13, 14, False), (17, 18, True), (20, 21, False)]


class _BN:

    def __init__(self, C_, dev):
        self.scale = torch.empty(C_, device=dev)
        self.shift = torch.empty(C_, device=dev)
        self.mean = torch.empty(C_, device=dev)
        self.invstd = torch.empty(C_, device=dev)
        self.sums = torch.empty(2, C_, device=dev)
        self.stats = None


class SymTable:

    CAPACITY = 16384

    def __init__(self, dev):
        self.dev = dev
        self.table = torch.zeros(self.CAPACITY, 3, 3, device=dev)
        self.rows = 0
        self._by_id = {}
        self._by_bytes = {}

    def _register(self, s):
        import numpy as np

        arr = s.detach().cpu().numpy() if isinstance(s, torch.Tensor) else np.asarray(s)
        arr = np.ascontiguousarray(arr, dtype=np.float32).reshape(-1, 3, 3)
        key = arr.tobytes()
        ent = self._by_bytes.get(key)
        if ent is None:
            k = arr.shape[0]
            if self.rows + k > self.CAPACITY:
                raise RuntimeError(f"symmetry table full ({self.rows} + {k} > {self.CAPACITY} rows)")
            self.table[self.rows:self.rows + k].copy_(torch.from_numpy(arr))
            ent = (self.rows, k)
            self.rows += k
            self._by_bytes[key] = ent
        return ent

    def indices(self, sym_infos) -> torch.Tensor:
        out = torch.zeros(len(sym_infos), 2, dtype=torch.int32).pin_memory()
        for b, s in enumerate(sym_infos):
            if s is None:
                continue
            hit = self._by_id.get(id(s))
            if hit is None or hit[0] is not s:
                first, count = self._register(s)
                if len(self._by_id) > 4096:
                    self._by_id.clear()
                self._by_id[id(s)] = (s, first, count)
            else:
                first, count = hit[1], hit[2]
            out[b, 0], out[b, 1] = first, count
        return out.to(self.dev, non_blocking=True)


class Engine:
    def __init__(self, model, precision: str = "half"):
        precision = {"bf16": "half", "fp16": "half"}.get(precision, precision)
        assert precision in ("half", "fp32x3", "mixed"), precision
        C.load()
        self.model = model
        self.precision = precision
        self.planes = 1 if precision == "half" else 2
        self.bplanes = 2 if precision == "fp32x3" else 1
        self.dev = next(model.parameters()).device
        if self.dev.type != "cuda":
            raise RuntimeError("gdr_net_b200 engine needs CUDA parameters (model.to('cuda')); no CPU fallback exists")
        self.ws = ops.Workspace(self.dev)
        self.sym_table = SymTable(self.dev)
        self.wgrad_side_stream = os.environ.get("GDRN_WGRAD_STREAM", "1") == "1"
        self._side_stream, self._side_keep = None, []
        self.deterministic = os.environ.get("GDRN_DETERMINISTIC") == "1"
        self._det_ws = None
        self.fold_eval = os.environ.get("GDRN_NO_FOLD_EVAL") != "1"
        self.with_2d = int(model.pnp_net.features[0].in_channels == 69)
        assert model.pnp_net.features[0].in_channels in (67, 69), model.pnp_net.features[0].in_channels
        self.named_params = list(model.named_parameters())
        self.bn: Dict[str, _BN] = {}
        total = 0
        self._bn_mods = {}
        for name, m in model.named_modules():
            if isinstance(m, torch.nn.BatchNorm2d):
                self.bn[name] = _BN(m.num_features, self.dev)
                self._bn_mods[name] = m
                total += 2 * m.num_features
        self.stats_all = torch.zeros(total, device=self.dev)
        self.bwd_sums_all = torch.zeros(total, device=self.dev)
        off = 0
        for name, m in self._bn_mods.items():
            n = 2 * m.num_features
            self.bn[name].stats = self.stats_all[off:off + n]
            self.bn[name].sums = self.bwd_sums_all[off:off + n].view(2, m.num_features)
            off += n
        self.flat_grad = torch.zeros(sum(p.numel() for _, p in self.named_params), device=self.dev)
        self.grads: Dict[str, torch.Tensor] = {}
        off = 0
        for name, p in self.named_params:
            self.grads[name] = self.flat_grad[off:off + p.numel()].view_as(p)
            off += p.numel()
        self.saved = None
        self.wf: Dict[str, PT] = {}
        self.wd: Dict[str, PT] = {}
        self.grad_hook = None
        self.use_cuda_graphs = False
        self._graphed = None
        self.storage_name = ops.storage_format()[2]
        self.grad_scale = 1024.0 if self.storage_name == "fp16" else 1.0
        from .dist import SEGMENTS, segment_bounds

        self._seg = segment_bounds(self.named_params, SEGMENTS)

    def _conv_modules(self):
        m = self.model
        out = [("backbone.conv1", m.backbone.conv1)]
        for li in range(1, 5):
            for bi, blk in enumerate(getattr(m.backbone, f"layer{li}")):
                p = f"backbone.layer{li}.{bi}"
                out.append((p + ".conv1", blk.conv1))
                out.append((p + ".conv2", blk.conv2))
                if blk.downsample is not None:
                    out.append((p + ".downsample.0", blk.downsample[0]))
        for ci, _bi, _u in HEAD_CONVS:
            out.append((f"rot_head_net.features.{ci}", m.rot_head_net.features[ci]))
        out.append(("rot_head_net.features.23", m.rot_head_net.features[23]))
        for ci in (0, 3, 6):
            out.append((f"pnp_net.features.{ci}", m.pnp_net.features[ci]))
        return out

    def prepare_weights(self, need_dgrad: bool):
        import numpy as np

        key = (need_dgrad, tuple(p.data_ptr() for _, p in self.named_params))
        tables = self.__dict__.setdefault("_pack_tables", {})
        tab = tables.get(key)
        if tab is None:
            ops._pack_recorder = []
            try:
                self._prepare_weights_calls(need_dgrad)
                self._pack_stem()
                jobs = ops._pack_recorder
            finally:
                ops._pack_recorder = None
            dt = np.dtype([("src", "<u8"), ("hi", "<u8"), ("lo", "<u8"), ("so", "<i8"), ("si", "<i8"), ("sr", "<i8"), ("ss", "<i8"),
                           ("begin", "<i8"), ("O", "<i4"), ("I", "<i4"), ("KH", "<i4"), ("KW", "<i4"), ("opad", "<i4"),
                           ("ipad", "<i4"), ("krow", "<i4"), ("flip", "<i4"), ("row_scale", "<u8")])
            assert dt.itemsize == 104
            arr = np.zeros(len(jobs), dtype=dt)
            begin = 0
            for n, (src, out, O, I, KH, KW, opad, ipad, krow, so, si, sr, ss, flip) in enumerate(jobs):
                arr[n] = (src.data_ptr(), out.hi_ptr, out.lo_ptr or 0, so, si, sr, ss, begin, O, I, KH, KW, opad, ipad, krow, flip, 0)
                begin += -(-opad // 16) * -(-ipad // 64) * -(-(KH * KW) // 9)
            tab = dict(jobs=torch.from_numpy(arr.view(np.uint8).copy()).to(self.dev), njobs=len(jobs), blocks=begin,
                       keep=[j[0] for j in jobs] + [j[1] for j in jobs])
            tables[key] = tab
        with torch.no_grad():
            torch.cat([self.model.pnp_net.fc_r.weight, self.model.pnp_net.fc_t.weight], 0, out=self.w_rt)
            torch.cat([self.model.pnp_net.fc_r.bias, self.model.pnp_net.fc_t.bias], 0, out=self.b_rt)
        C.gdrn_pack_weight_batched(tab["jobs"].data_ptr(), tab["njobs"], tab["blocks"], _stream())

    def _conv_bn_pairs(self):
        m = self.model
        out = [("stem", "backbone.bn1")]
        for li in range(1, 5):
            for bi, blk in enumerate(getattr(m.backbone, f"layer{li}")):
                p = f"backbone.layer{li}.{bi}"
                out += [(p + ".conv1", p + ".bn1"), (p + ".conv2", p + ".bn2")]
                if blk.downsample is not None:
                    out.append((p + ".downsample.0", p + ".downsample.1"))
        out.append(("deconv", "rot_head_net.features.1"))
        out += [(f"rot_head_net.features.{ci}", f"rot_head_net.features.{bi}") for ci, bi, _u in HEAD_CONVS]
        return out

    def prepare_weights_folded(self):
        import numpy as np

        key = tuple(p.data_ptr() for _, p in self.named_params)
        fold = getattr(self, "_fold", None)
        if fold is None or fold["key"] != key:
            pl = self.planes
            pairs = self._conv_bn_pairs()
            convs = dict(self._conv_modules())
            wfe, sc, sh = {}, {}, {}
            fdt = np.dtype([("gamma", "<u8"), ("beta", "<u8"), ("mean", "<u8"), ("var", "<u8"), ("scale", "<u8"), ("shift", "<u8"),
                            ("C", "<i4"), ("eps", "<f4"), ("pad", "<i8")])
            assert fdt.itemsize == 64
            farr = np.zeros(len(pairs), dtype=fdt)
            for n, (ck, bk) in enumerate(pairs):
                mod = self._bn_mods[bk]
                sc[bk] = torch.empty(mod.num_features, device=self.dev)
                sh[bk] = torch.empty(mod.num_features, device=self.dev)
                farr[n] = (mod.weight.data_ptr(), mod.bias.data_ptr(), mod.running_mean.data_ptr(), mod.running_var.data_ptr(),
                           sc[bk].data_ptr(), sh[bk].data_ptr(), mod.num_features, float(mod.eps), 0)
            ops._pack_recorder = []
            try:
                scales = []
                for ck, bk in pairs:
                    if ck == "stem":
                        w = self.model.backbone.conv1.weight
                        wfe[ck] = PT((64, 192), pl, device=self.dev, zero=True)
                        ops._pack(w, wfe[ck], 64, 3, 7, 7, 64, 3, 192, 147, 49, 7, 1, 0)
                    elif ck == "deconv":
                        pk = ops.pack_deconv_fwd_phases if _DECONV_PHASES else ops.pack_deconv_fwd
                        wfe[ck] = pk(self.model.rot_head_net.features[0].weight, pl)
                    else:
                        wfe[ck] = ops.pack_conv_fwd(convs[ck].weight, pl)
                    scales.append(sc[bk])
                jobs = ops._pack_recorder
            finally:
                ops._pack_recorder = None
            dt = np.dtype([("src", "<u8"), ("hi", "<u8"), ("lo", "<u8"), ("so", "<i8"), ("si", "<i8"), ("sr", "<i8"), ("ss", "<i8"),
                           ("begin", "<i8"), ("O", "<i4"), ("I", "<i4"), ("KH", "<i4"), ("KW", "<i4"), ("opad", "<i4"),
                           ("ipad", "<i4"), ("krow", "<i4"), ("flip", "<i4"), ("row_scale", "<u8")])
            assert dt.itemsize == 104
            arr = np.zeros(len(jobs), dtype=dt)
            begin = 0
            for n, (src, out, O, I, KH, KW, opad, ipad, krow, so, si, sr, ss, flip) in enumerate(jobs):
                arr[n] = (src.data_ptr(), out.hi_ptr, out.lo_ptr or 0, so, si, sr, ss, begin, O, I, KH, KW, opad, ipad, krow, flip,
                          scales[n].data_ptr())
                begin += -(-opad // 16) * -(-ipad // 64) * -(-(KH * KW) // 9)
            fold = self._fold = dict(key=key, wf=wfe, scale=sc, shift=sh, njobs=len(jobs), blocks=begin, nfold=len(pairs),
                                     fjobs=torch.from_numpy(farr.view(np.uint8).copy()).to(self.dev),
                                     jobs=torch.from_numpy(arr.view(np.uint8).copy()).to(self.dev), keep=[j[0] for j in jobs])
        C.gdrn_bn_fold_batched(fold["fjobs"].data_ptr(), fold["nfold"], _stream())
        C.gdrn_pack_weight_batched(fold["jobs"].data_ptr(), fold["njobs"], fold["blocks"], _stream())
        return fold

    def forward_eval_folded(self, x: torch.Tensor, aux: dict, want_maps: bool = False) -> dict:
        m, pl, dev = self.model, self.planes, self.dev
        B = x.shape[0]
        assert x.shape[1:] == (3, 256, 256), x.shape
        fold_box = {}

        def packs():
            self.prepare_weights(need_dgrad=False)
            fold_box["F"] = self.prepare_weights_folded()

        self._on_side(packs)

        def cbr(xin, ck, bk, conv, relu=True, res=None, kind="conv"):
            if kind == "deconv":
                if _DECONV_PHASES:
                    return ops.conv_dgrad_s2(xin, wfe[ck], conv.out_channels, 3, 1, bias=shift[bk], act=2 if relu else 0)
                return ops.conv_fwd(ops.zero_insert(xin), wfe[ck], conv.out_channels, 3, 3, 1, 1, bias=shift[bk], act=2 if relu else 0,
                                    res=res, algo_scale=0.25)
            k, stride, pad = conv.kernel_size[0], conv.stride[0], conv.padding[0]
            return ops.conv_fwd(xin, wfe[ck], conv.out_channels, k, k, stride, pad, bias=shift[bk], act=2 if relu else 0, res=res)

        a_col = PT((B * 128 * 128, 192), pl, device=dev)
        C.gdrn_stem_im2col(x.data_ptr(), a_col.hi_ptr, a_col.lo_ptr, B, 256, 256, _stream())
        self._join_side(force=True)
        wfe, shift = fold_box["F"]["wf"], fold_box["F"]["shift"]
        a0 = ops.gemm_fwd(a_col, wfe["stem"], 64, bias=shift["backbone.bn1"], act=2).view(B, 128, 128, 64)
        cur = ops.maxpool_fwd(a0)
        for li in range(1, 5):
            for bi, blk in enumerate(getattr(m.backbone, f"layer{li}")):
                p = f"backbone.layer{li}.{bi}"
                a1 = cbr(cur, p + ".conv1", p + ".bn1", blk.conv1)
                idn = cur
                if blk.downsample is not None:
                    idn = cbr(cur, p + ".downsample.0", p + ".downsample.1", blk.downsample[0], relu=False)
                cur = cbr(a1, p + ".conv2", p + ".bn2", blk.conv2, res=idn)
        hf = m.rot_head_net.features
        cur = cbr(cur, "deconv", "rot_head_net.features.1", hf[0], kind="deconv")
        for ci, bi, up in HEAD_CONVS:
            if up:
                cur = ops.upsample2x_fwd(cur)
            cur = cbr(cur, f"rot_head_net.features.{ci}", f"rot_head_net.features.{bi}", hf[ci])
        return self._tail_inference(cur, aux, want_maps)

    def _eval_graphed(self, x: torch.Tensor, aux: dict, want_maps: bool) -> dict:
        tens = {k: v for k, v in aux.items() if isinstance(v, torch.Tensor)}
        key = (tuple(x.shape), want_maps, tuple(sorted((k, tuple(v.shape)) for k, v in tens.items())),
               tuple(p.data_ptr() for _, p in self.named_params))
        cache = self.__dict__.setdefault("_eval_graphs", {})
        g = cache.get(key)
        if g is None:
            st = dict(x=x.clone(), aux={k: (v.clone() if isinstance(v, torch.Tensor) else v) for k, v in aux.items()})
            side = torch.cuda.Stream()
            side.wait_stream(torch.cuda.current_stream())
            with torch.cuda.stream(side):
                self.forward_eval_folded(st["x"], st["aux"], want_maps=want_maps)
            torch.cuda.current_stream().wait_stream(side)
            torch.cuda.synchronize()
            st["graph"] = torch.cuda.CUDAGraph()
            with torch.cuda.graph(st["graph"], capture_error_mode=_capture_mode()):
                st["res"] = self.forward_eval_folded(st["x"], st["aux"], want_maps=want_maps)
            if len(cache) > 8:
                cache.clear()
            g = cache[key] = st
        g["x"].copy_(x, non_blocking=True)
        for k, v in tens.items():
            g["aux"][k].copy_(v, non_blocking=True)
        g["graph"].replay()
        return {k: (v.clone() if isinstance(v, torch.Tensor) else v) for k, v in g["res"].items()}

    def _tail_inference(self, head_in: PT, aux: dict, want_maps: bool) -> dict:
        m, pl, dev = self.model, self.planes, self.dev
        B = head_in.shape[0]
        hf, pn, pf = m.rot_head_net.features, m.pnp_net, m.pnp_net.features
        logits = torch.empty(B * 4096, 72, device=dev)
        ops.conv_fwd(head_in, self.wf["rot_head_net.features.23"], 69, 1, 1, 1, 0, out_f32=logits, bias=hf[23].bias, ldc=72,
                     want_planes=False)
        pnp_in = PT((B, 64, 64, 128), pl, device=dev)
        C.gdrn_head_glue_fwd(logits.data_ptr(), ops.ptr(aux.get("roi_coord_2d")), aux["roi_extents"].data_ptr(), pnp_in.hi_ptr,
                             pnp_in.lo_ptr, B, 4096, self.with_2d, _stream())
        cur = pnp_in
        for ci, gi in ((0, 1), (3, 4), (6, 7)):
            u = ops.conv_fwd(cur, self.wf[f"pnp_net.features.{ci}"], 128, 3, 3, 2, 1)
            gstats = torch.empty(B, 32, 2, device=dev)
            cur = ops.gn_relu_fwd(u, pf[gi].weight, pf[gi].bias, gstats, G=pf[gi].num_groups, eps=pf[gi].eps)
        h1 = ops.gemm_fwd(cur.view(B, 8192), self.wf["fc1"], 1024, bias=pn.fc1.bias, act=1)
        h2 = ops.gemm_fwd(h1, self.wf["fc2"], 256, bias=pn.fc2.bias, act=1)
        pred = torch.zeros(B, 16, device=dev)
        ops.gemm_fwd(h2, self.wf["fc_rt"], 9, out_f32=pred, bias=self.b_rt, ldc=16, want_planes=False)
        out_rot = torch.empty(B, 3, 3, device=dev)
        out_trans = torch.empty(B, 3, device=dev)
        C.gdrn_pose_loss(pred.data_ptr(), 16, aux["roi_cams"].data_ptr(), aux["roi_centers"].data_ptr(),
                         aux["roi_whs"].data_ptr(), aux["resize_ratios"].data_ptr(), aux["roi_extents"].data_ptr(), None,
                         None, None, None, None, None, None, out_rot.data_ptr(), out_trans.data_ptr(), None, None, None,
                         None, B, 0, 0, 0.0, _stream())
        res = dict(rot=out_rot, trans=out_trans, pred=pred, logits=logits)
        if want_maps:
            maps = logits.view(B, 64, 64, 72).permute(0, 3, 1, 2)
            res.update(mask=maps[:, 0:1], coor_x=maps[:, 1:2], coor_y=maps[:, 2:3], coor_z=maps[:, 3:4], region=maps[:, 4:69])
        return res

    def _prepare_weights_calls(self, need_dgrad: bool):
        m, pl, bpl = self.model, self.planes, self.bplanes
        wf, wd = self.wf, self.wd
        for key, conv in self._conv_modules():
            if key == "backbone.conv1":
                continue
            wf[key] = ops.pack_conv_fwd(conv.weight, pl, out=wf.get(key))
            if need_dgrad:
                wd[key] = ops.pack_conv_dgrad(conv.weight, bpl, out=wd.get(key))
        dc = m.rot_head_net.features[0]
        wf["deconv"] = (ops.pack_deconv_fwd_phases if _DECONV_PHASES else ops.pack_deconv_fwd)(dc.weight, pl, out=wf.get("deconv"))
        if need_dgrad:
            wd["deconv"] = ops.pack_deconv_dgrad(dc.weight, bpl, out=wd.get("deconv"))
        pn = m.pnp_net
        wf["fc1"] = ops.pack_linear(pn.fc1.weight, pl, out=wf.get("fc1"), nhwc_from=(128, 8, 8))
        wf["fc2"] = ops.pack_linear(pn.fc2.weight, pl, out=wf.get("fc2"))
        if not hasattr(self, "w_rt"):
            self.w_rt = torch.empty(pn.fc_r.out_features + 3, pn.fc_r.in_features, device=self.dev)
            self.b_rt = torch.empty(pn.fc_r.out_features + 3, device=self.dev)
        wf["fc_rt"] = ops.pack_linear(self.w_rt, pl, out=wf.get("fc_rt"))
        if need_dgrad:
            wd["fc1"] = ops.pack_linear(pn.fc1.weight, bpl, out=wd.get("fc1"), nhwc_from=(128, 8, 8), transpose=True)
            wd["fc2"] = ops.pack_linear(pn.fc2.weight, bpl, out=wd.get("fc2"), transpose=True)
            wd["fc_rt"] = ops.pack_linear(self.w_rt, bpl, out=wd.get("fc_rt"), transpose=True)

    def _pack_stem(self):
        w = self.model.backbone.conv1.weight
        out = self.wf.get("stem") or PT((64, 192), self.planes, device=self.dev, zero=True)
        ops._pack(w, out, 64, 3, 7, 7, 64, 3, 192, 147, 49, 7, 1, 0)
        self.wf["stem"] = out

    def _bn_fwd(self, key: str, u: PT, relu: bool, train_bn: bool, res: Optional[PT] = None) -> PT:
        mod, st = self._bn_mods[key], self.bn[key]
        Cc = mod.num_features
        count = u.numel() // Cc
        mom = mod.momentum if mod.momentum is not None else 0.1
        if train_bn and mod.num_batches_tracked is not None:
            self._nbt.append(mod.num_batches_tracked)
        if train_bn and self.deterministic:
            C.gdrn_bn_stats(u.hi_ptr, u.lo_ptr, self._det_workspace().data_ptr(), st.stats.data_ptr(), count, Cc, _stream())
        y = ops.like(u)
        mask = None
        if relu and getattr(self, "_want_masks", False) and _BN_BITMASK:
            mask = torch.empty(u.numel() // 8, dtype=torch.uint8, device=self.dev)
        self._last_mask = mask
        C.gdrn_bn_fwd(u.hi_ptr, u.lo_ptr, res.hi_ptr if res else None, res.lo_ptr if res else None, y.hi_ptr, y.lo_ptr,
                      ops.ptr(st.stats) if train_bn else None, mod.weight.data_ptr(), mod.bias.data_ptr(),
                      mod.running_mean.data_ptr(), mod.running_var.data_ptr(), st.mean.data_ptr(), st.invstd.data_ptr(),
                      ops.ptr(mask), count, Cc, float(mod.eps), float(mom), int(train_bn), int(relu), _stream())
        return y

    def _det_workspace(self):
        if self._det_ws is None:
            self._det_ws = torch.empty(2 * 512 * int(C.load().gdrn_det_parts()), device=self.dev)
        return self._det_ws

    def _conv_bn(self, x: PT, ckey: str, conv, bkey: str, relu: bool, train_bn: bool, res: Optional[PT] = None,
                 wkey: Optional[str] = None, kind: str = "conv"):
        st = self.bn[bkey]
        stats = st.stats if (train_bn and not self.deterministic) else None
        k, stride, pad = conv.kernel_size[0], conv.stride[0], conv.padding[0]
        if kind == "deconv" and _DECONV_PHASES:
            u = ops.conv_dgrad_s2(x, self.wf["deconv"], conv.out_channels, 3, 1, stats=stats)
        elif kind == "deconv":
            u = ops.conv_fwd(x, self.wf["deconv"], conv.out_channels, 3, 3, 1, 1, stats=stats, algo_scale=0.25)
        else:
            u = ops.conv_fwd(x, self.wf[wkey or ckey], conv.out_channels, k, k, stride, pad, stats=stats)
        y = self._bn_fwd(bkey, u, relu, train_bn, res)
        return u, y

    def run(self, x, *, roi_coord_2d, roi_cams, roi_centers, roi_whs, roi_extents, resize_ratios, gt_xyz=None,
            gt_mask_trunc=None, gt_mask_visib=None, gt_region=None, gt_ego_rot=None, gt_points=None, sym_infos=None,
            gt_trans=None, gt_trans_ratio=None, do_loss=False, train_bn=False, want_maps=False):
        aux = dict(roi_coord_2d=roi_coord_2d, roi_cams=roi_cams, roi_centers=roi_centers, roi_whs=roi_whs,
                   roi_extents=roi_extents, resize_ratios=resize_ratios, gt_xyz=gt_xyz, gt_mask_trunc=gt_mask_trunc,
                   gt_mask_visib=gt_mask_visib, gt_region=gt_region, gt_ego_rot=gt_ego_rot, gt_points=gt_points,
                   sym_infos=sym_infos, gt_trans=gt_trans, gt_trans_ratio=gt_trans_ratio)
        B = x.shape[0]
        for k_, v in aux.items():
            if isinstance(v, torch.Tensor):
                v = v.to(self.dev)
                aux[k_] = (v.long() if k_ == "gt_region" else v.float()).contiguous()
        if roi_cams is not None and aux["roi_cams"].dim() == 2:
            aux["roi_cams"] = aux["roi_cams"].unsqueeze(0).expand(B, 3, 3).contiguous()
        want = dict(roi_coord_2d=(B, 2, 64, 64), roi_cams=(B, 3, 3), roi_centers=(B, 2), roi_whs=(B, 2), roi_extents=(B, 3),
                    resize_ratios=(B,), gt_xyz=(B, 3, 64, 64), gt_mask_trunc=(B, 64, 64), gt_mask_visib=(B, 64, 64),
                    gt_region=(B, 64, 64), gt_ego_rot=(B, 3, 3), gt_trans=(B, 3), gt_trans_ratio=(B, 3))
        for k_, shp in want.items():
            v = aux.get(k_)
            if isinstance(v, torch.Tensor):
                if v.numel() != int(torch.Size(shp).numel()):
                    raise ValueError(f"{k_}: expected shape {shp} for a batch of {B}, got {tuple(v.shape)}")
                aux[k_] = v.view(shp)
        if isinstance(aux.get("gt_points"), torch.Tensor) and (aux["gt_points"].dim() != 3 or aux["gt_points"].shape[0] != B
                                                               or aux["gt_points"].shape[2] != 3):
            raise ValueError(f"gt_points: expected [B={B}, n, 3], got {tuple(aux['gt_points'].shape)}")
        if aux.get("sym_infos") is not None:
            if len(aux["sym_infos"]) != B:
                raise ValueError(f"sym_infos: expected a list of {B} entries, got {len(aux['sym_infos'])}")
            aux["sym_idx"] = self.sym_table.indices(aux["sym_infos"])
        aux.pop("sym_infos", None)
        x = x.to(self.dev).float().contiguous()
        if not do_loss:
            with torch.no_grad():
                if not train_bn and self.fold_eval:
                    if self.use_cuda_graphs:
                        return self._eval_graphed(x, aux, want_maps)
                    return self.forward_eval_folded(x, aux, want_maps=want_maps)
                return self.forward(x, aux, train_bn=train_bn, do_loss=False, want_maps=want_maps)
        params = [p for _, p in self.named_params]
        losses, vis = _GDRNFunction.apply(self, x, aux, train_bn, *params)
        return dict(losses=losses, vis=vis)

    def forward(self, x: torch.Tensor, aux: dict, train_bn: bool, do_loss: bool, want_maps: bool = False) -> dict:
        m, pl, dev = self.model, self.planes, self.dev
        B = x.shape[0]
        assert x.shape[1:] == (3, 256, 256), x.shape
        self._on_side(lambda: self.prepare_weights(need_dgrad=do_loss))
        self._nbt = []
        if train_bn:
            self.stats_all.zero_()
        S = dict(B=B, train_bn=train_bn) if do_loss else None
        self._want_masks = do_loss

        a_col = PT((B * 128 * 128, 192), pl, device=dev)
        C.gdrn_stem_im2col(x.data_ptr(), a_col.hi_ptr, a_col.lo_ptr, B, 256, 256, _stream())
        self._join_side(force=True)
        st0 = self.bn["backbone.bn1"]
        u0 = ops.gemm_fwd(a_col, self.wf["stem"], 64, stats=st0.stats if (train_bn and not self.deterministic) else None).view(B, 128, 128, 64)
        a0 = self._bn_fwd("backbone.bn1", u0, True, train_bn)
        if S is not None:
            cur, pool_arg = ops.maxpool_fwd(a0, want_arg=True)
            S["stem"] = dict(a_col=a_col, u0=u0, a0=a0, pool_arg=pool_arg, m0=self._last_mask)
            S["blocks"] = []
        else:
            cur = ops.maxpool_fwd(a0)
        for li in range(1, 5):
            for bi, blk in enumerate(getattr(m.backbone, f"layer{li}")):
                p = f"backbone.layer{li}.{bi}"
                u1, a1 = self._conv_bn(cur, p + ".conv1", blk.conv1, p + ".bn1", True, train_bn)
                m1 = self._last_mask
                ud = None
                if blk.downsample is not None:
                    ud, idn = self._conv_bn(cur, p + ".downsample.0", blk.downsample[0], p + ".downsample.1", False, train_bn)
                else:
                    idn = cur
                u2, out = self._conv_bn(a1, p + ".conv2", blk.conv2, p + ".bn2", True, train_bn, res=idn)
                if S is not None:
                    S["blocks"].append(dict(p=p, blk=blk, x_in=cur, u1=u1, a1=a1, u2=u2, out=out, ud=ud, m1=m1, m2=self._last_mask))
                cur = out
        feat = cur

        hf = m.rot_head_net.features
        z = feat if _DECONV_PHASES else ops.zero_insert(feat)
        u, y = self._conv_bn(z, "deconv", hf[0], "rot_head_net.features.1", True, train_bn, kind="deconv")
        if S is not None:
            S["deconv"] = dict(z=z, u=u, y=y, m=self._last_mask)
            S["head"] = []
        cur = y
        for ci, bi, up in HEAD_CONVS:
            if up:
                cur = ops.upsample2x_fwd(cur)
            u, y = self._conv_bn(cur, f"rot_head_net.features.{ci}", hf[ci], f"rot_head_net.features.{bi}", True, train_bn)
            if S is not None:
                S["head"].append(dict(ci=ci, bi=bi, up=up, x_in=cur, u=u, y=y, m=self._last_mask))
            cur = y
        head_in = cur
        if self._nbt:
            torch._foreach_add_(self._nbt, 1)
        logits = torch.empty(B * 4096, 72, device=dev)
        ops.conv_fwd(head_in, self.wf["rot_head_net.features.23"], 69, 1, 1, 1, 0, out_f32=logits, bias=hf[23].bias, ldc=72,
                     want_planes=False)

        pnp_in = PT((B, 64, 64, 128), pl, device=dev)
        C.gdrn_head_glue_fwd(logits.data_ptr(), ops.ptr(aux.get("roi_coord_2d")), aux["roi_extents"].data_ptr(), pnp_in.hi_ptr,
                             pnp_in.lo_ptr, B, 4096, self.with_2d, _stream())
        pf = m.pnp_net.features
        cur = pnp_in
        pnp_saved = []
        for ci, gi in ((0, 1), (3, 4), (6, 7)):
            u = ops.conv_fwd(cur, self.wf[f"pnp_net.features.{ci}"], 128, 3, 3, 2, 1)
            gstats = torch.empty(B, 32, 2, device=dev)
            y = ops.gn_relu_fwd(u, pf[gi].weight, pf[gi].bias, gstats, G=pf[gi].num_groups, eps=pf[gi].eps)
            pnp_saved.append(dict(ci=ci, gi=gi, x_in=cur, u=u, y=y, gstats=gstats))
            cur = y
        flat = cur.view(B, 8192)
        pn = m.pnp_net
        h1 = ops.gemm_fwd(flat, self.wf["fc1"], 1024, bias=pn.fc1.bias, act=1)
        h2 = ops.gemm_fwd(h1, self.wf["fc2"], 256, bias=pn.fc2.bias, act=1)
        pred = torch.zeros(B, 16, device=dev)
        ops.gemm_fwd(h2, self.wf["fc_rt"], 9, out_f32=pred, bias=self.b_rt, ldc=16, want_planes=False)

        out_rot = torch.empty(B, 3, 3, device=dev)
        out_trans = torch.empty(B, 3, device=dev)
        res = dict(rot=out_rot, trans=out_trans, pred=pred)
        if not do_loss:
            C.gdrn_pose_loss(pred.data_ptr(), 16, aux["roi_cams"].data_ptr(), aux["roi_centers"].data_ptr(),
                             aux["roi_whs"].data_ptr(), aux["resize_ratios"].data_ptr(), aux["roi_extents"].data_ptr(), None,
                             None, None, None, None, None, None, out_rot.data_ptr(), out_trans.data_ptr(), None, None, None,
                             None, B, 0, 0, 0.0, _stream())
            if want_maps:
                maps = logits.view(B, 64, 64, 72).permute(0, 3, 1, 2)
                res.update(mask=maps[:, 0:1], coor_x=maps[:, 1:2], coor_y=maps[:, 2:3], coor_z=maps[:, 3:4], region=maps[:, 4:69])
            res["logits"] = logits
            return res

        pix_sums = torch.empty(6, dtype=torch.float64, device=dev)
        C.gdrn_pixel_loss_fwd(logits.data_ptr(), aux["gt_xyz"].data_ptr(), aux["gt_mask_visib"].data_ptr(),
                              aux["gt_mask_trunc"].data_ptr(), aux["gt_region"].data_ptr(), pix_sums.data_ptr(), B, 4096, _stream())
        S.update(logits=logits, pnp_in=pnp_in, pnp=pnp_saved, flat=flat, h1=h1, h2=h2, pred=pred, head_in=head_in,
                 pix_sums=pix_sums, aux=aux)
        self.saved = S
        self._pose(S, gw=None)
        losses = torch.empty(8, device=dev)
        vis2 = torch.empty(2, device=dev)
        n_pts = aux["gt_points"].shape[1]
        C.gdrn_loss_finalize(pix_sums.data_ptr(), S["pose_sums"].data_ptr(), S["vis_ps"].data_ptr(), losses.data_ptr(),
                             vis2.data_ptr(), B, 4096, n_pts, _stream())
        vis = torch.cat([vis2, out_trans_first(S["out_trans"]), pred[0, 6:9], aux["gt_trans"][0], aux["gt_trans_ratio"][0]])
        res.update(rot=S["out_rot"], trans=S["out_trans"], losses=losses, vis=vis, logits=logits)
        return res

    def _pose(self, S, gw):
        aux, B, dev = S["aux"], S["B"], self.dev
        if "out_rot" not in S:
            S["out_rot"] = torch.empty(B, 3, 3, device=dev)
            S["out_trans"] = torch.empty(B, 3, device=dev)
            S["pose_sums"] = torch.empty(4, dtype=torch.float64, device=dev)
            S["vis_ps"] = torch.empty(B, 2, device=dev)
            S["dy9"] = PT((B, 64), self.bplanes, device=dev)
        sym_idx = aux.get("sym_idx")
        if sym_idx is None and aux.get("sym_infos") is not None:
            sym_idx = aux["sym_idx"] = self.sym_table.indices(aux["sym_infos"])
        syms = self.sym_table.table if sym_idx is not None else None
        if gw is None:
            gw = torch.ones(3, device=dev)
        n_pts = aux["gt_points"].shape[1]
        C.gdrn_pose_loss(S["pred"].data_ptr(), 16, aux["roi_cams"].data_ptr(), aux["roi_centers"].data_ptr(),
                         aux["roi_whs"].data_ptr(), aux["resize_ratios"].data_ptr(), aux["roi_extents"].data_ptr(),
                         aux["gt_points"].data_ptr(), aux["gt_ego_rot"].data_ptr(), aux["gt_trans"].data_ptr(),
                         aux["gt_trans_ratio"].data_ptr(), ops.ptr(syms), ops.ptr(sym_idx), gw.data_ptr(),
                         S["out_rot"].data_ptr(), S["out_trans"].data_ptr(), S["pose_sums"].data_ptr(), S["vis_ps"].data_ptr(),
                         S["dy9"].hi_ptr, S["dy9"].lo_ptr, B, n_pts, 1, 1e-4, _stream())

    def _on_side(self, fn, keep=()):
        if not self.wgrad_side_stream:
            return fn()
        if self._side_stream is None:
            self._side_stream = torch.cuda.Stream()
        side = self._side_stream
        side.wait_stream(torch.cuda.current_stream())
        with torch.cuda.stream(side):
            fn()
        self._side_keep.extend(keep)

    def _join_side(self, force: bool = False):
        if self._side_stream is not None and (self._side_keep or force):
            torch.cuda.current_stream().wait_stream(self._side_stream)
        self._side_keep.clear()

    def _wgrad_conv(self, du: PT, x_in: PT, conv, wname: str, ipad: Optional[int] = None):
        O, I, k = conv.out_channels, conv.in_channels, conv.kernel_size[0]

        def work():
            buf, ks, kss = ops.conv_wgrad(du, x_in, self.ws, O, k, k, conv.stride[0], conv.padding[0])
            ops.unpack_wgrad(buf, self.grads[wname], O, I, k, k, ipad or x_in.shape[-1], ks, kss, I * k * k, k * k, k, 1)

        self._on_side(work, keep=(du, x_in))

    def _dgrad_conv(self, du: PT, conv, wkey: str) -> PT:
        k, stride, pad = conv.kernel_size[0], conv.stride[0], conv.padding[0]
        if stride == 2 and not _DGRAD_ZERO_INSERT:
            return ops.conv_dgrad_s2(du, self.wd[wkey], conv.in_channels, k, pad)
        z = ops.zero_insert(du) if stride == 2 else du
        return ops.conv_fwd(z, self.wd[wkey], conv.in_channels, k, k, 1, k - 1 - pad, algo_scale=0.25 if stride == 2 else 1.0)

    def _bn_bwd(self, bkey: str, ga: PT, gb: Optional[PT], y: Optional[PT], u: PT, want_gout=False, relu_from_u=False, mask=None):
        mod, st = self._bn_mods[bkey], self.bn[bkey]
        relu_from_u = relu_from_u and _BN_MASK_FROM_U and mask is None
        return ops.bn_bwd(ga, gb, None if (relu_from_u or mask is not None) else y, u, st.mean, st.invstd, mod.weight, st.sums,
                          self.grads[bkey + ".weight"], self.grads[bkey + ".bias"], self.saved["train_bn"], want_gout=want_gout,
                          beta=mod.bias, relu_from_u=relu_from_u, sums_zeroed=True, relu_mask=mask,
                          det_ws=self._det_workspace() if self.deterministic else None)

    def backward(self, grad_losses: torch.Tensor):
        S, m, dev = self.saved, self.model, self.dev
        assert S is not None, "backward called without a do_loss forward"
        B, aux, pn = S["B"], S["aux"], m.pnp_net
        bp = self.bplanes

        def h(t: PT) -> PT:
            return t.as_planes(bp)

        self.flat_grad.zero_()
        self.bwd_sums_all.zero_()
        gw = grad_losses.float().contiguous()
        if self.grad_scale != 1.0:
            gw = gw * self.grad_scale
        self._pose(S, gw=gw[5:8].contiguous())
        dy9 = S["dy9"]
        tmp = torch.empty(1024, device=dev)

        buf, ks, kss = ops.gemm_wgrad(dy9, h(S["h2"]), self.ws)
        ops.unpack_wgrad(buf, self.grads["pnp_net.fc_r.weight"], 6, 256, 1, 1, 256, ks, kss, 256, 1, 0, 0)
        ops.unpack_wgrad(buf[6 * 256:], self.grads["pnp_net.fc_t.weight"], 3, 256, 1, 1, 256, ks, kss, 256, 1, 0, 0)
        C.gdrn_colsum(dy9.hi_ptr, dy9.lo_ptr, tmp.data_ptr(), B, 64, _stream())
        self.grads["pnp_net.fc_r.bias"].copy_(tmp[0:6])
        self.grads["pnp_net.fc_t.bias"].copy_(tmp[6:9])
        dh2 = ops.gemm_fwd(dy9, self.wd["fc_rt"], 256)
        dz2 = self._leaky_bwd(dh2, h(S["h2"]))
        buf, ks, kss = ops.gemm_wgrad(dz2, h(S["h1"]), self.ws)
        ops.unpack_wgrad(buf, self.grads["pnp_net.fc2.weight"], 256, 1024, 1, 1, 1024, ks, kss, 1024, 1, 0, 0)
        C.gdrn_colsum(dz2.hi_ptr, dz2.lo_ptr, self.grads["pnp_net.fc2.bias"].data_ptr(), B, 256, _stream())
        dh1 = ops.gemm_fwd(dz2, self.wd["fc2"], 1024)
        dz1 = self._leaky_bwd(dh1, h(S["h1"]))
        buf, ks, kss = ops.gemm_wgrad(dz1, h(S["flat"]), self.ws)
        ops.unpack_wgrad(buf, self.grads["pnp_net.fc1.weight"], 1024, 128, 8, 8, 128, ks, kss, 8192, 64, 8, 1)
        C.gdrn_colsum(dz1.hi_ptr, dz1.lo_ptr, self.grads["pnp_net.fc1.bias"].data_ptr(), B, 1024, _stream())
        g = ops.gemm_fwd(dz1, self.wd["fc1"], 8192).view(B, 8, 8, 128)

        pf = pn.features
        for L in reversed(S["pnp"]):
            ci, gi = L["ci"], L["gi"]
            du = ops.gn_relu_bwd(g, h(L["y"]), h(L["u"]), pf[gi].weight, L["gstats"], self.grads[f"pnp_net.features.{gi}.weight"],
                                 self.grads[f"pnp_net.features.{gi}.bias"], G=pf[gi].num_groups)
            self._wgrad_conv(du, h(L["x_in"]), pf[ci], f"pnp_net.features.{ci}.weight")
            g = self._dgrad_conv(du, pf[ci], f"pnp_net.features.{ci}")
        d_pnp_in = g
        self._segment_done("pnp_net")

        dlog = PT((B * 4096, 128), bp, device=dev)
        C.gdrn_head_bwd(S["logits"].data_ptr(), aux["gt_xyz"].data_ptr(), aux["gt_mask_visib"].data_ptr(),
                        aux["gt_mask_trunc"].data_ptr(), aux["gt_region"].data_ptr(), S["pix_sums"].data_ptr(), gw.data_ptr(),
                        d_pnp_in.hi_ptr, d_pnp_in.lo_ptr, aux["roi_extents"].data_ptr(), dlog.hi_ptr, dlog.lo_ptr, B, 4096,
                        self.with_2d, _stream())
        hf = m.rot_head_net.features
        head_in = h(S["head_in"])
        def head_out_wgrad():
            buf, ks, kss = ops.gemm_wgrad(dlog, head_in.view(B * 4096, 256), self.ws)
            ops.unpack_wgrad(buf, self.grads["rot_head_net.features.23.weight"], 69, 256, 1, 1, 256, ks, kss, 256, 1, 0, 0)

        self._on_side(head_out_wgrad, keep=(dlog,))
        tmp128 = torch.empty(128, device=dev)
        C.gdrn_colsum(dlog.hi_ptr, dlog.lo_ptr, tmp128.data_ptr(), B * 4096, 128, _stream())
        self.grads["rot_head_net.features.23.bias"].copy_(tmp128[:69])
        g = ops.gemm_fwd(dlog, self.wd["rot_head_net.features.23"], 256).view(B, 64, 64, 256)

        for L in reversed(S["head"]):
            ci, bi = L["ci"], L["bi"]
            du, _ = self._bn_bwd(f"rot_head_net.features.{bi}", g, None, h(L["y"]), h(L["u"]), relu_from_u=True, mask=L["m"])
            self._wgrad_conv(du, h(L["x_in"]), hf[ci], f"rot_head_net.features.{ci}.weight")
            g = self._dgrad_conv(du, hf[ci], f"rot_head_net.features.{ci}")
            if L["up"]:
                g = ops.upsample2x_bwd(g)
        D = S["deconv"]
        du, _ = self._bn_bwd("rot_head_net.features.1", g, None, h(D["y"]), h(D["u"]), relu_from_u=True, mask=D["m"])
        def deconv_wgrad(du=du):
            if _DECONV_PHASES:
                buf, ks, kss = ops.conv_wgrad(h(D["z"]), du, self.ws, 512, 3, 3, 2, 1)
                ops.unpack_wgrad(buf, self.grads["rot_head_net.features.0.weight"], 512, 256, 3, 3, 256, ks, kss, 256 * 9, 9, 3, 1)
                return
            buf, ks, kss = ops.conv_wgrad(du, h(D["z"]), self.ws, 256, 3, 3, 1, 1)
            ops.unpack_wgrad(buf, self.grads["rot_head_net.features.0.weight"], 256, 512, 3, 3, 512, ks, kss, 9, 256 * 9, 3, 1, flip=1)

        self._on_side(deconv_wgrad, keep=(du,))
        g = ops.conv_fwd(du, self.wd["deconv"], 512, 3, 3, 2, 1)
        self._segment_done("rot_head_net")

        ga, gb = g, None
        for Lb in reversed(S["blocks"]):
            p, blk = Lb["p"], Lb["blk"]
            du2, gout = self._bn_bwd(p + ".bn2", ga, gb, h(Lb["out"]), h(Lb["u2"]), want_gout=True, mask=Lb["m2"])
            self._wgrad_conv(du2, h(Lb["a1"]), blk.conv2, p + ".conv2.weight")
            da1 = self._dgrad_conv(du2, blk.conv2, p + ".conv2")
            du1, _ = self._bn_bwd(p + ".bn1", da1, None, h(Lb["a1"]), h(Lb["u1"]), relu_from_u=True, mask=Lb["m1"])
            self._wgrad_conv(du1, h(Lb["x_in"]), blk.conv1, p + ".conv1.weight")
            dx_main = self._dgrad_conv(du1, blk.conv1, p + ".conv1")
            if blk.downsample is not None:
                dud, _ = self._bn_bwd(p + ".downsample.1", gout, None, None, h(Lb["ud"]))
                self._wgrad_conv(dud, h(Lb["x_in"]), blk.downsample[0], p + ".downsample.0.weight")
                dx_ds = self._dgrad_conv(dud, blk.downsample[0], p + ".downsample.0")
                ga, gb = dx_main, dx_ds
            else:
                ga, gb = dx_main, gout
            if p.endswith(".0") and not p.startswith("backbone.layer1"):
                self._segment_done(p[:-2])
        g_pool = ops.add2(ga, gb)
        St = S["stem"]
        g_a0 = ops.maxpool_bwd(St["pool_arg"], g_pool)
        du0, _ = self._bn_bwd("backbone.bn1", g_a0, None, h(St["a0"]), h(St["u0"]), relu_from_u=True, mask=St["m0"])
        def stem_wgrad():
            buf, ks, kss = ops.gemm_wgrad(du0.view(B * 128 * 128, 64), h(St["a_col"]), self.ws)
            ops.unpack_wgrad(buf, self.grads["backbone.conv1.weight"], 64, 3, 7, 7, 3, ks, kss, 147, 49, 7, 1, krow=192)

        self._on_side(stem_wgrad, keep=(du0,))
        self._segment_done("backbone.stem")
        self.saved = None
        return self.grads

    def materialize_aliased_grads(self):
        lo = self.flat_grad.data_ptr()
        hi = lo + self.flat_grad.numel() * self.flat_grad.element_size()
        for _, p in self.named_params:
            g = p.grad
            if g is not None and lo <= g.data_ptr() < hi:
                p.grad = g.clone()

    def _segment_done(self, stage: str):
        self._join_side()
        self._segment_done_joined(stage)

    def _segment_done_joined(self, stage: str):
        if self.grad_scale != 1.0:
            names = ("backbone.conv1", "backbone.bn1", "backbone.layer1") if stage == "backbone.stem" else (stage,)
            lo = min(self._seg[n][0] for n in names)
            hi = max(self._seg[n][1] for n in names)
            C.gdrn_scale_f32(self.flat_grad.data_ptr() + 4 * lo, hi - lo, 1.0 / self.grad_scale, _stream())
        if self.grad_hook:
            self.grad_hook(self, stage)

    def _leaky_bwd(self, g: PT, y: PT) -> PT:
        out = ops.like(g)
        C.gdrn_leaky_bwd(g.hi_ptr, g.lo_ptr, y.hi_ptr, out.hi_ptr, out.lo_ptr, g.numel(), _stream())
        return out


def out_trans_first(t):
    return t[0]


def _bn_snapshot(engine: "Engine"):
    return [(m, m.running_mean.clone(), m.running_var.clone(),
             None if m.num_batches_tracked is None else m.num_batches_tracked.clone()) for m in engine._bn_mods.values()]


def _bn_restore(snap):
    with torch.no_grad():
        for m, rm, rv, nbt in snap:
            m.running_mean.copy_(rm)
            m.running_var.copy_(rv)
            if nbt is not None:
                m.num_batches_tracked.copy_(nbt)


def _capture_mode():
    import torch.distributed as dist

    return "thread_local" if (dist.is_available() and dist.is_initialized()) else "global"


def _finish_hook(engine: "Engine"):
    hook = engine.grad_hook
    if hook is not None and hasattr(hook, "finish"):
        hook.finish()


class GraphedTrainStep:

    def __init__(self, engine: "Engine", x: torch.Tensor, aux: dict, train_bn: bool = True, warmup: int = 2, after_backward=None):
        self.engine = engine
        self.x = x.clone()
        self.aux = {k: (v.clone() if isinstance(v, torch.Tensor) else v) for k, v in aux.items()}
        if self.aux.get("sym_infos") is not None:
            self.aux["sym_idx"] = engine.sym_table.indices(self.aux["sym_infos"])
        self.aux.pop("sym_infos", None)
        self.gw = torch.ones(8, device=x.device)

        def one_step():
            res = engine.forward(self.x, self.aux, train_bn=train_bn, do_loss=True)
            engine.backward(self.gw)
            _finish_hook(engine)
            if after_backward is not None:
                after_backward()
            return res

        snap = _bn_snapshot(engine)
        side = torch.cuda.Stream()
        side.wait_stream(torch.cuda.current_stream())
        with torch.cuda.stream(side):
            for _ in range(warmup):
                one_step()
        torch.cuda.current_stream().wait_stream(side)
        torch.cuda.synchronize()
        _bn_restore(snap)
        self.graph = torch.cuda.CUDAGraph()
        with torch.cuda.graph(self.graph, capture_error_mode=_capture_mode()):
            res = one_step()
        self.losses, self.vis, self.rot, self.trans = res["losses"], res["vis"], res["rot"], res["trans"]
        self.logits = res["logits"]

    def __call__(self, x: Optional[torch.Tensor] = None, aux: Optional[dict] = None, grad_losses: Optional[torch.Tensor] = None):
        if x is not None:
            self.x.copy_(x, non_blocking=True)
        if aux is not None:
            if aux.get("sym_infos") is not None:
                self.aux["sym_idx"].copy_(self.engine.sym_table.indices(aux["sym_infos"]), non_blocking=True)
            for k, v in aux.items():
                if isinstance(v, torch.Tensor):
                    self.aux[k].copy_(v, non_blocking=True)
        if grad_losses is not None:
            self.gw.copy_(grad_losses)
        self.graph.replay()
        return self.losses


class GraphedFwdBwd:

    def __init__(self, engine: "Engine", x: torch.Tensor, aux: dict, train_bn: bool):
        self.engine, self.train_bn = engine, train_bn
        self.x = x.clone()
        self.aux = {k: (v.clone() if isinstance(v, torch.Tensor) else v) for k, v in aux.items()}
        self.gw = torch.ones(8, device=x.device)
        self.key = self.signature(x, aux, train_bn)
        snap = _bn_snapshot(engine)
        side = torch.cuda.Stream()
        side.wait_stream(torch.cuda.current_stream())
        with torch.cuda.stream(side), torch.no_grad():
            for _ in range(2):
                engine.forward(self.x, self.aux, train_bn=train_bn, do_loss=True)
                engine.backward(self.gw)
                _finish_hook(engine)
        torch.cuda.current_stream().wait_stream(side)
        torch.cuda.synchronize()
        _bn_restore(snap)
        self.g_fwd, self.g_bwd = torch.cuda.CUDAGraph(), torch.cuda.CUDAGraph()
        pool = torch.cuda.graph_pool_handle()
        mode = _capture_mode()
        with torch.no_grad():
            with torch.cuda.graph(self.g_fwd, pool=pool, capture_error_mode=mode):
                res = engine.forward(self.x, self.aux, train_bn=train_bn, do_loss=True)
            with torch.cuda.graph(self.g_bwd, pool=pool, capture_error_mode=mode):
                engine.backward(self.gw)
                _finish_hook(engine)
        self.losses, self.vis = res["losses"], res["vis"]

    @staticmethod
    def signature(x, aux, train_bn):
        return (tuple(x.shape), train_bn, tuple(sorted((k, tuple(v.shape)) for k, v in aux.items() if isinstance(v, torch.Tensor))))

    def forward(self, x, aux):
        self.x.copy_(x, non_blocking=True)
        for k, v in aux.items():
            if isinstance(v, torch.Tensor):
# ... 46 lines not shown
```

### gdr_net_b200/ops.py

```python
from __future__ import annotations

import ctypes

import torch

from .capi import C


def _stream():
    return torch.cuda.current_stream().cuda_stream


_FMT = {}


def storage_format():
    if not _FMT:
        dll = C.load()
        dll.gdrn_lo_scale.restype = ctypes.c_float
        f16 = bool(dll.gdrn_storage_format())
        _FMT.update(dtype=torch.float16 if f16 else torch.bfloat16, lo_scale=float(dll.gdrn_lo_scale()), name="fp16" if f16 else "bf16")
    return _FMT["dtype"], _FMT["lo_scale"], _FMT["name"]


# ... 2 lines not shown


def ptr(t):
    return None if t is None else t.data_ptr()


class PT:

    __slots__ = ("buf", "shape", "planes")

    def __init__(self, shape, planes: int, device="cuda", buf=None, zero=False):
        self.shape = tuple(int(s) for s in shape)
        self.planes = planes
        if buf is None:
            alloc = torch.zeros if zero else torch.empty
            buf = alloc((planes,) + self.shape, dtype=storage_format()[0], device=device)
        self.buf = buf

    @property
    def hi(self):
        return self.buf[0]

    @property
    def lo(self):
        return self.buf[1] if self.planes == 2 else None

    @property
    def hi_ptr(self):
        return self.buf.data_ptr()

    @property
    def lo_ptr(self):
        return (self.buf.data_ptr() + self.buf[0].numel() * 2) if self.planes == 2 else None

    @property
    def nsplit(self):
        return 1 if self.planes == 1 else 3

    def numel(self):
        return self.buf[0].numel()

    def float(self):
        x = self.buf[0].float()
        if self.planes == 2:
            x = x + self.buf[1].float() * (1.0 / storage_format()[1])
        return x

    def as_planes(self, planes: int) -> "PT":
        if planes == self.planes:
            return self
        assert planes == 1 and self.planes == 2, (planes, self.planes)
        return PT(self.shape, 1, buf=self.buf[0:1])

    def view(self, *shape):
        return PT(shape, self.planes, buf=self.buf.view((self.planes,) + tuple(shape)))

    @staticmethod
    def from_float(x: torch.Tensor, planes: int) -> "PT":
        x = x.contiguous().float()
        out = PT(x.shape, planes, device=x.device)
        assert x.numel() % 8 == 0
        C.gdrn_f32_to_planes(x.data_ptr(), out.hi_ptr, out.lo_ptr, x.numel(), _stream())
        return out

    def to_float(self) -> torch.Tensor:
        y = torch.empty(self.shape, dtype=torch.float32, device=self.buf.device)
        C.gdrn_planes_to_f32(self.hi_ptr, self.lo_ptr, y.data_ptr(), y.numel(), _stream())
        return y


def _round_up(x, m):
    return (x + m - 1) // m * m


_pack_recorder = None


def _pack(src: torch.Tensor, out: "PT", O, I, KH, KW, opad, ipad, krow, so, si, sr, ss, flip):
    if _pack_recorder is not None:
        _pack_recorder.append((src, out, O, I, KH, KW, opad, ipad, krow, so, si, sr, ss, flip))
        return
    C.gdrn_pack_weight(src.data_ptr(), out.hi_ptr, out.lo_ptr, O, I, KH, KW, opad, ipad, krow, so, si, sr, ss, flip, _stream())


def pack_conv_fwd(w: torch.Tensor, planes: int, out: PT | None = None, ipad: int | None = None) -> PT:
    O, I, KH, KW = w.shape
    ipad = ipad or _round_up(I, 64)
    opad = _round_up(O, 64)
    krow = KH * KW * ipad
    out = out or PT((opad, krow), planes, device=w.device)
    _pack(w, out, O, I, KH, KW, opad, ipad, krow, I * KH * KW, KH * KW, KW, 1, 0)
    return out


def pack_conv_dgrad(w: torch.Tensor, planes: int, out: PT | None = None) -> PT:
    O, I, KH, KW = w.shape
    opad, ipad = _round_up(I, 64), _round_up(O, 64)
    krow = KH * KW * ipad
    out = out or PT((opad, krow), planes, device=w.device)
    _pack(w, out, I, O, KH, KW, opad, ipad, krow, KH * KW, I * KH * KW, KW, 1, 1)
    return out


def pack_deconv_fwd_phases(wt: torch.Tensor, planes: int, out: PT | None = None) -> PT:
    return pack_conv_dgrad(wt, planes, out=out)


def pack_deconv_fwd(wt: torch.Tensor, planes: int, out: PT | None = None) -> PT:
    I, O, KH, KW = wt.shape
    opad, ipad = _round_up(O, 64), _round_up(I, 64)
    krow = KH * KW * ipad
    out = out or PT((opad, krow), planes, device=wt.device)
    _pack(wt, out, O, I, KH, KW, opad, ipad, krow, KH * KW, O * KH * KW, KW, 1, 1)
    return out


def pack_deconv_dgrad(wt: torch.Tensor, planes: int, out: PT | None = None) -> PT:
    I, O, KH, KW = wt.shape
    opad, ipad = _round_up(I, 64), _round_up(O, 64)
    krow = KH * KW * ipad
    out = out or PT((opad, krow), planes, device=wt.device)
    _pack(wt, out, I, O, KH, KW, opad, ipad, krow, O * KH * KW, KH * KW, KW, 1, 0)
    return out


def pack_linear(w: torch.Tensor, planes: int, out: PT | None = None, nhwc_from: tuple | None = None,
                transpose: bool = False) -> PT:
    N, K = w.shape
    if nhwc_from is not None:
        Cc, H, W = nhwc_from
        assert Cc * H * W == K
        if not transpose:
            opad = _round_up(N, 64)
            out = out or PT((opad, K), planes, device=w.device)
            _pack(w, out, N, Cc, H, W, opad, Cc, K, K, H * W, W, 1, 0)
            return out
        taps = H * W
        npad = _round_up(N, 64)
        assert npad == N
        out = out or PT((K, N), planes, device=w.device)
        _pack(w, out, taps, N, Cc, 1, taps, N, Cc * N, 1, K, taps, 0, 0)
        return out
    if not transpose:
        opad = _round_up(N, 64)
        out = out or PT((opad, K), planes, device=w.device)
        _pack(w, out, N, K, 1, 1, opad, K, K, K, 1, 0, 0, 0)
    else:
        opad, ipad = _round_up(K, 64), _round_up(N, 64)
        out = out or PT((opad, ipad), planes, device=w.device)
        _pack(w, out, K, N, 1, 1, opad, ipad, ipad, 1, K, 0, 0, 0)
    return out


def conv_fwd(x: PT, wp: PT, Cout: int, KH: int, KW: int, stride: int, pad: int, *, out: PT | None = None,
             out_f32: torch.Tensor | None = None, bias=None, stats=None, act: int = 0, ldc: int | None = None,
             want_planes: bool = True, algo_scale: float = 1.0, res: PT | None = None) -> PT | None:
    N, H, W, Cin = x.shape
    Ho, Wo = H // stride, W // stride
    ldc = ldc or _round_up(Cout, 64)
    if want_planes and out is None:
        out = PT((N, Ho, Wo, ldc), x.planes, device=x.buf.device, zero=(ldc != Cout))
    C.gdrn_conv_fwd(x.hi_ptr, x.lo_ptr, wp.hi_ptr, wp.lo_ptr, out.hi_ptr if out is not None else None,
                    out.lo_ptr if out is not None else None, ptr(out_f32), ptr(bias), res.hi_ptr if res is not None else None,
                    res.lo_ptr if res is not None else None, ptr(stats), N, H, W, Cin, Cout, wp.shape[0], KH, KW, stride, pad,
                    ldc, act, x.nsplit, _stream())
    return out


def conv_dgrad_s2(du: PT, wd: PT, Cx: int, K: int, pad: int, *, out: PT | None = None, bias=None, stats=None, act: int = 0) -> PT:
    N, Ho, Wo, Cy = du.shape
    ldc = _round_up(Cx, 64)
    if out is None:
        out = PT((N, 2 * Ho, 2 * Wo, ldc), du.planes, device=du.buf.device, zero=(K == 1 or ldc != Cx))
    C.gdrn_conv_dgrad_s2(du.hi_ptr, du.lo_ptr, wd.hi_ptr, wd.lo_ptr, out.hi_ptr, out.lo_ptr, ptr(bias), ptr(stats), N, Ho, Wo, Cy, Cx,
                         wd.shape[0], K, pad, ldc, act, du.nsplit, _stream())
    return out


def gemm_fwd(a: PT, wp: PT, N: int, *, out: PT | None = None, out_f32: torch.Tensor | None = None, bias=None, stats=None,
             act: int = 0, ldc: int | None = None, want_planes: bool = True) -> PT | None:
    M, K = a.shape
    ldc = ldc or _round_up(N, 64)
    if want_planes and out is None:
        out = PT((M, ldc), a.planes, device=a.buf.device, zero=(ldc != N))
    C.gdrn_gemm_fwd(a.hi_ptr, a.lo_ptr, wp.hi_ptr, wp.lo_ptr, out.hi_ptr if out is not None else None,
                    out.lo_ptr if out is not None else None, ptr(out_f32), ptr(bias), ptr(stats), M, N, wp.shape[0], K, ldc,
                    act, a.nsplit, _stream())
    return out


class Workspace:

    def __init__(self, device="cuda"):
        self.device = device
        self.buf = None

    def get(self, nfloats: int) -> torch.Tensor:
        if self.buf is None or self.buf.numel() < nfloats:
            self.buf = torch.empty(int(nfloats), dtype=torch.float32, device=self.device)
        return self.buf


def conv_wgrad(dy: PT, x: PT, ws: Workspace, Cout: int, KH: int, KW: int, stride: int, pad: int, ksplit: int = 0):
    N, H, W, Cin = x.shape
    need = ctypes.c_long(0)
    ks = ctypes.c_int(0)
    cout_ld = dy.shape[-1]
    args = (N, H, W, Cin, cout_ld, KH, KW, stride, pad, ksplit, x.nsplit, _stream())
    C.gdrn_conv_wgrad(None, None, None, None, None, 0, ctypes.addressof(need), ctypes.addressof(ks), *args)
    buf = ws.get(need.value)
    C.gdrn_conv_wgrad(dy.hi_ptr, dy.lo_ptr, x.hi_ptr, x.lo_ptr, buf.data_ptr(), buf.numel(), None, None, *args)
    mpad = _round_up(cout_ld, 128)
    return buf, ks.value, mpad * KH * KW * Cin


def gemm_wgrad(dy: PT, x: PT, ws: Workspace, ksplit: int = 0):
    P, M = dy.shape
    P2, Ntot = x.shape
    assert P == P2
    need = ctypes.c_long(0)
    ks = ctypes.c_int(0)
    args = (P, M, Ntot, ksplit, x.nsplit, _stream())
    C.gdrn_gemm_wgrad(None, None, None, None, None, 0, ctypes.addressof(need), ctypes.addressof(ks), *args)
    buf = ws.get(need.value)
    C.gdrn_gemm_wgrad(dy.hi_ptr, dy.lo_ptr, x.hi_ptr, x.lo_ptr, buf.data_ptr(), buf.numel(), None, None, *args)
    return buf, ks.value, _round_up(M, 128) * Ntot


def unpack_wgrad(buf, grad: torch.Tensor, O, I, KH, KW, ipad, ksplit, ks_stride, so, si, sr, ss, flip=0, accumulate=0, krow=None):
    C.gdrn_unpack_wgrad(buf.data_ptr(), grad.data_ptr(), O, I, KH, KW, ipad, krow or KH * KW * ipad, ksplit, ks_stride, so, si, sr,
                        ss, flip, accumulate, _stream())


def like(x: PT, shape=None) -> PT:
    return PT(shape or x.shape, x.planes, device=x.buf.device)


def bn_finalize(stats, gamma, beta, rm, rv, scale, shift, mean, invstd, C_, count, eps, momentum, train):
    C.gdrn_bn_finalize(ptr(stats), gamma.data_ptr(), beta.data_ptr(), ptr(rm), ptr(rv), scale.data_ptr(), shift.data_ptr(),
                       ptr(mean), ptr(invstd), C_, float(count), float(eps), float(momentum), int(train), _stream())


def bn_act(x: PT, scale, shift, relu: bool, res: PT | None = None, out: PT | None = None) -> PT:
    out = out or like(x)
    Cc = x.shape[-1]
    rows = x.numel() // Cc
    C.gdrn_bn_act(x.hi_ptr, x.lo_ptr, res.hi_ptr if res else None, res.lo_ptr if res else None, out.hi_ptr, out.lo_ptr,
                  scale.data_ptr(), shift.data_ptr(), rows, Cc, int(relu), _stream())
    return out


def bn_bwd(ga: PT, gb: PT | None, y: PT | None, u: PT, mean, invstd, gamma, sums, dgamma, dbeta, train: bool,
           want_gout: bool = False, beta=None, relu_from_u: bool = False, sums_zeroed: bool = False, relu_mask=None, det_ws=None):
    du = like(u)
    gout = like(u) if want_gout else None
    Cc = u.shape[-1]
    rows = u.numel() // Cc
    assert not (relu_from_u and y is not None)
    C.gdrn_bn_bwd(ga.hi_ptr, ga.lo_ptr, gb.hi_ptr if gb else None, gb.lo_ptr if gb else None, y.hi_ptr if y else None,
                  u.hi_ptr, u.lo_ptr, mean.data_ptr(), invstd.data_ptr(), gamma.data_ptr(), ptr(beta), sums.data_ptr(), du.hi_ptr,
                  du.lo_ptr, gout.hi_ptr if gout else None, gout.lo_ptr if gout else None, ptr(dgamma), ptr(dbeta), ptr(relu_mask),
                  ptr(det_ws), rows, Cc, int(train),
                  (1 if relu_from_u else 0) | (2 if sums_zeroed else 0) | (4 if det_ws is not None else 0), _stream())
    return du, gout


def maxpool_fwd(x: PT, want_arg: bool = False):
    B, H, W, Cc = x.shape
    out = like(x, (B, H // 2, W // 2, Cc))
    arg = torch.empty((B, H // 2, W // 2, Cc), dtype=torch.uint8, device=x.buf.device) if want_arg else None
    C.gdrn_maxpool_fwd(x.hi_ptr, x.lo_ptr, out.hi_ptr, out.lo_ptr, ptr(arg), B, H, W, Cc, _stream())
    return (out, arg) if want_arg else out


def maxpool_bwd(arg: torch.Tensor, g: PT) -> PT:
    B, Ho, Wo, Cc = g.shape
    out = like(g, (B, 2 * Ho, 2 * Wo, Cc))
    C.gdrn_maxpool_bwd(arg.data_ptr(), g.hi_ptr, g.lo_ptr, out.hi_ptr, out.lo_ptr, B, 2 * Ho, 2 * Wo, Cc, _stream())
    return out


def upsample2x_fwd(x: PT) -> PT:
    B, H, W, Cc = x.shape
    out = like(x, (B, 2 * H, 2 * W, Cc))
    C.gdrn_upsample2x_fwd(x.hi_ptr, x.lo_ptr, out.hi_ptr, out.lo_ptr, B, H, W, Cc, _stream())
    return out


def upsample2x_bwd(g: PT) -> PT:
    B, Ho, Wo, Cc = g.shape
    out = like(g, (B, Ho // 2, Wo // 2, Cc))
    C.gdrn_upsample2x_bwd(g.hi_ptr, g.lo_ptr, out.hi_ptr, out.lo_ptr, B, Ho // 2, Wo // 2, Cc, _stream())
    return out


def zero_insert(x: PT) -> PT:
    B, H, W, Cc = x.shape
    out = like(x, (B, 2 * H, 2 * W, Cc))
    C.gdrn_zero_insert(x.hi_ptr, x.lo_ptr, out.hi_ptr, out.lo_ptr, B, H, W, Cc, 0, _stream())
    return out


def extract_even(x: PT) -> PT:
    B, H2, W2, Cc = x.shape
    out = like(x, (B, H2 // 2, W2 // 2, Cc))
    C.gdrn_zero_insert(x.hi_ptr, x.lo_ptr, out.hi_ptr, out.lo_ptr, B, H2 // 2, W2 // 2, Cc, 1, _stream())
    return out


def gn_relu_fwd(u: PT, gamma, beta, stats, G=32, eps=1e-5) -> PT:
    B, H, W, Cc = u.shape
    out = like(u)
    C.gdrn_gn_relu_fwd(u.hi_ptr, u.lo_ptr, out.hi_ptr, out.lo_ptr, gamma.data_ptr(), beta.data_ptr(), stats.data_ptr(), B, H * W,
                       Cc, G, float(eps), _stream())
    return out


def gn_relu_bwd(g: PT, y: PT, u: PT, gamma, stats, dgamma, dbeta, G=32) -> PT:
    B, H, W, Cc = u.shape
    du = like(u)
    C.gdrn_gn_relu_bwd(g.hi_ptr, g.lo_ptr, y.hi_ptr, u.hi_ptr, u.lo_ptr, gamma.data_ptr(), stats.data_ptr(), du.hi_ptr, du.lo_ptr,
                       dgamma.data_ptr(), dbeta.data_ptr(), B, H * W, Cc, G, _stream())
    return du


def add2(a: PT, b: PT) -> PT:
    out = like(a)
    C.gdrn_add2(a.hi_ptr, a.lo_ptr, b.hi_ptr, b.lo_ptr, out.hi_ptr, out.lo_ptr, a.numel(), _stream())
    return out
```

### include/gdrn_b200.h

```cpp
#ifndef GDRN_B200_H
#define GDRN_B200_H

#ifdef __cplusplus
extern "C" {
#endif

#define GDRN_OK 0
#define GDRN_ERR_ARG (-1)
#define GDRN_ERR_CUDA (-2)

const char* gdrn_last_error(void);
long gdrn_launch_count(void);
int gdrn_abi_version(void);
int gdrn_storage_format(void);
float gdrn_lo_scale(void);
int gdrn_set_2cta(int on);
long gdrn_2cta_launch_count(void);
int gdrn_set_pdl(int on);
int gdrn_set_wgrad_2cta(int on);
long gdrn_wgrad_2cta_launch_count(void);
int gdrn_last_gemm_variant(void);

int gdrn_conv_fwd(const void* x_hi, const void* x_lo, const void* w_hi, const void* w_lo, void* y_hi, void* y_lo,
                  float* y_f32, const float* bias, const void* res_hi, const void* res_lo, float* stats, int N, int H, int W,
                  int Cin, int Cout, int Cout_pad, int KH, int KW, int stride, int pad, int ldc, int act, int nsplit,
                  void* stream);

int gdrn_conv_dgrad_s2(const void* du_hi, const void* du_lo, const void* w_hi, const void* w_lo, void* dx_hi, void* dx_lo,
                       const float* bias, float* stats, int N, int Ho, int Wo, int Cy, int Cx, int Cx_pad, int K, int pad, int ldc,
                       int act, int nsplit, void* stream);

int gdrn_gemm_fwd(const void* a_hi, const void* a_lo, const void* w_hi, const void* w_lo, void* y_hi, void* y_lo,
                  float* y_f32, const float* bias, float* stats, int M, int N, int N_pad, int K, int ldc, int act,
                  int nsplit, void* stream);

int gdrn_conv_wgrad(const void* dy_hi, const void* dy_lo, const void* x_hi, const void* x_lo, float* ws, long ws_floats,
                    long* ws_need_out, int* ksplit_out, int N, int H, int W, int Cin, int Cout, int KH, int KW,
                    int stride, int pad, int ksplit, int nsplit, void* stream);
int gdrn_gemm_wgrad(const void* dy_hi, const void* dy_lo, const void* x_hi, const void* x_lo, float* ws, long ws_floats,
                    long* ws_need_out, int* ksplit_out, long P, int M, int Ntot, int ksplit, int nsplit, void* stream);

int gdrn_pack_weight(const float* src, void* dst_hi, void* dst_lo, int O, int I, int KH, int KW, int opad, int ipad,
                     int krow, long so, long si, long sr, long ss, int flip, void* stream);
int gdrn_pack_weight_batched(const void* jobs_dev, int njobs, long total_blocks, void* stream);
int gdrn_unpack_wgrad(const float* ws, float* grad, int O, int I, int KH, int KW, int ipad, int krow, int ksplit, long ks_stride,
                      long so, long si, long sr, long ss, int flip, int accumulate, void* stream);
int gdrn_stem_im2col(const float* x, void* a_hi, void* a_lo, int B, int H, int W, void* stream);

int gdrn_bn_fold_batched(const void* jobs_dev, int njobs, void* stream);
int gdrn_bn_finalize(const float* stats, const float* gamma, const float* beta, float* running_mean, float* running_var,
                     float* scale, float* shift, float* mean_out, float* invstd_out, int C, float count, float eps,
                     float momentum, int train, void* stream);
int gdrn_bn_fwd(const void* x_hi, const void* x_lo, const void* r_hi, const void* r_lo, void* y_hi, void* y_lo,
                const float* stats, const float* gamma, const float* beta, float* running_mean, float* running_var,
                float* mean_out, float* invstd_out, void* relu_mask_out, long rows, int C, float eps, float momentum, int train,
                int relu, void* stream);
int gdrn_bn_act(const void* x_hi, const void* x_lo, const void* r_hi, const void* r_lo, void* y_hi, void* y_lo,
                const float* scale, const float* shift, long rows, int C, int relu, void* stream);
int gdrn_bn_bwd(const void* ga_hi, const void* ga_lo, const void* gb_hi, const void* gb_lo, const void* y_hi,
                const void* u_hi, const void* u_lo, const float* mean, const float* invstd, const float* gamma,
                const float* beta, float* sums, void* du_hi, void* du_lo, void* gout_hi, void* gout_lo, float* dgamma,
                float* dbeta, const void* relu_mask, float* det_ws, long rows, int C, int train, int flags, void* stream);
int gdrn_det_parts(void);
int gdrn_bn_stats(const void* u_hi, const void* u_lo, float* ws, float* stats, long rows, int C, void* stream);

int gdrn_maxpool_fwd(const void* x_hi, const void* x_lo, void* y_hi, void* y_lo, void* arg_out, int B, int H, int W, int C,
                     void* stream);
int gdrn_maxpool_bwd(const void* arg_in, const void* g_hi, const void* g_lo, void* dx_hi, void* dx_lo, int B, int H, int W,
                     int C, void* stream);
int gdrn_upsample2x_fwd(const void* x_hi, const void* x_lo, void* y_hi, void* y_lo, int B, int H, int W, int C, void* stream);
int gdrn_upsample2x_bwd(const void* g_hi, const void* g_lo, void* dx_hi, void* dx_lo, int B, int H, int W, int C, void* stream);
int gdrn_zero_insert(const void* x_hi, const void* x_lo, void* y_hi, void* y_lo, int B, int H, int W, int C, int mode,
                     void* stream);
int gdrn_gn_relu_fwd(const void* u_hi, const void* u_lo, void* y_hi, void* y_lo, const float* gamma, const float* beta,
                     float* stats, int B, int HW, int C, int G, float eps, void* stream);
int gdrn_gn_relu_bwd(const void* g_hi, const void* g_lo, const void* y_hi, const void* u_hi, const void* u_lo,
                     const float* gamma, const float* stats, void* du_hi, void* du_lo, float* dgamma, float* dbeta, int B,
                     int HW, int C, int G, void* stream);
int gdrn_add2(const void* a_hi, const void* a_lo, const void* b_hi, const void* b_lo, void* o_hi, void* o_lo, long n,
              void* stream);
int gdrn_colsum(const void* x_hi, const void* x_lo, float* out, long rows, int ld, void* stream);
int gdrn_leaky_bwd(const void* g_hi, const void* g_lo, const void* y_hi, void* o_hi, void* o_lo, long n, void* stream);
int gdrn_f32_to_planes(const float* x, void* y_hi, void* y_lo, long n, void* stream);
int gdrn_planes_to_f32(const void* x_hi, const void* x_lo, float* y, long n, void* stream);

int gdrn_head_glue_fwd(const float* logits, const float* coord2d, const float* extents, void* out_hi, void* out_lo, int B,
                       int HW, int with_2d, void* stream);
int gdrn_pnp_pack_input(const float* coor_feat, int c_feat, const float* region, int c_reg, const float* extents,
                        void* out_hi, void* out_lo, int B, int HW, void* stream);
int gdrn_pixel_loss_fwd(const float* logits, const float* gt_xyz, const float* m_visib, const float* m_trunc,
                        const long long* labels, double* sums, int B, int HW, void* stream);
int gdrn_head_bwd(const float* logits, const float* gt_xyz, const float* m_visib, const float* m_trunc,
                  const long long* labels, const double* sums, const float* gw, const void* din_hi, const void* din_lo,
                  const float* extents, void* out_hi, void* out_lo, int B, int HW, int with_2d, void* stream);

int gdrn_pose_loss(const float* pred, int ld_pred, const float* cams, const float* centers, const float* whs,
                   const float* ratios, const float* extents, const float* points, const float* gt_rot,
                   const float* gt_trans, const float* gt_ratio, const float* syms, const int* sym_idx, const float* gw,
                   float* out_rot, float* out_trans, double* sums, float* vis, void* dy_hi, void* dy_lo, int B, int n_pts,
                   int do_loss, float eps, void* stream);
int gdrn_loss_finalize(const double* pix_sums, const double* pose_sums, const float* vis, float* losses, float* vis_out,
                       int B, int HW, int n_pts, void* stream);

int gdrn_roi_crop_image(const void* image_u8, const double* centers, const double* scales, float* roi_img, int B, int H, int W,
                        int out_res, float pixel_std, void* stream);
int gdrn_roi_targets(const float* xyz, const float* mask_visib, const float* mask_trunc, const double* centers, const double* scales,
                     const float* extents, const float* fps_points, int n_fps, float* roi_xyz, float* roi_mask_trunc,
                     float* roi_mask_visib, float* roi_mask_obj, long long* roi_region, float* roi_coord_2d, int B, int H, int W,
                     int out_res, void* stream);

int gdrn_pose_errors(const float* R_est, const float* t_est, const float* R_gt, const float* t_gt, const float* points, int B,
                     int n_pts, int want_adi, float* out, void* stream);

long gdrn_pnp_ransac_workspace_bytes(int B, int HW, int iters);
int gdrn_pnp_ransac(const float* mask, const float* xyz, const float* coord2d, const float* extents, const float* im_wh,
                    const float* K, int B, int H, int W, int mask_mode, float mask_thr, double reproj_err, int iters,
                    double confidence, void* workspace, long workspace_bytes, float* out_pose, int* out_info,
                    unsigned char* out_inliers, void* stream);

int gdrn_ranger_step(const void* jobs_dev, const void* blocks_dev, int nblocks, float step_lr, float wd_lr, float beta1,
                     float beta2, float eps, float alpha, float grad_scale, int adaptive, int lookahead, void* stream);
int gdrn_scale_f32(float* x, long n, float s, void* stream);

#ifdef __cplusplus
}
#endif
#endif
```

Baseline: 5748.

## Fuse BatchNorm-backward reduction sums into maxpool, upsample and GEMM epilogues

Computes the BatchNorm-backward channel sums (sum of g and sum of g times normalized u, with optional ReLU mask) inside the producers of the gradient: maxpool backward, upsample backward and the GEMM/conv-dgrad epilogue. bn_bwd gains an apply-only flag that skips its own reduction pass. This removes a separate full read of the gradient and activation for the stats, and it adds extra loads of u and the mask plus shared-memory and atomic or partial-sum work in those kernels. A deterministic path writes per-block partials and launches a sum_partials kernel afterwards.

Result: slower. 5582, median of 6 (-2.9%).

```diff
diff --git a/gdr_net_b200/csrc/elementwise.cu b/gdr_net_b200/csrc/elementwise.cu
--- a/gdr_net_b200/csrc/elementwise.cu
+++ b/gdr_net_b200/csrc/elementwise.cu
@@ -303,12 +303,70 @@
     }
 }
 
-__global__ void maxpool_bwd_kernel(const uint8_t* __restrict__ arg_in, const bf16* __restrict__ g_hi,
-                                   const bf16* __restrict__ g_lo, bf16* __restrict__ dx_hi, bf16* __restrict__ dx_lo, int B, int H,
-                                   int W, int C) {
+constexpr int kBnBwdThreads = 256;
+
+struct BnBwdFeed {
+    const uint8_t* mask;
+    const bf16* u_hi;
+    const bf16* u_lo;
+    const float* mean;
+    const float* invstd;
+    float* sums;
+    float* part;
+};
+
+__device__ __forceinline__ void bn_sums_block_flush(const float (&s0)[8], const float (&s1)[8], int C, float* sums,
+                                                    float* partial_out) {
+    __shared__ float red[2][kBnBwdThreads][8 + 1];
+    const int cg = C / 8, rpb = kBnBwdThreads / cg;
+#pragma unroll
+    for (int j = 0; j < 8; ++j) {
+        red[0][threadIdx.x][j] = s0[j];
+        red[1][threadIdx.x][j] = s1[j];
+    }
+    __syncthreads();
+    for (int t = threadIdx.x; t < 2 * C; t += kBnBwdThreads) {
+        const int which = t / C, c = t % C;
+        const int gg = c / 8, j = c % 8;
+        float a = 0.f;
+        for (int q = 0; q < rpb; ++q) a += red[which][q * cg + gg][j];
+        if (partial_out != nullptr) partial_out[((long)blockIdx.x * 2 + which) * C + c] = a;
+        else atomicAdd(sums + which * C + c, a);
+    }
+}
+
+__device__ __forceinline__ void bn_feed_accum(const BnBwdFeed& bn, long idx8, const float* s_mu, const float* s_is, float (&g)[8],
+                                              float (&s0)[8], float (&s1)[8]) {
+    if (bn.mask != nullptr) {
+        const uint32_t bits = __ldg(bn.mask + idx8);
+#pragma unroll
+        for (int j = 0; j < 8; ++j) g[j] = ((bits >> j) & 1u) ? g[j] : 0.f;
+    }
+    float u[8];
+    load8(bn.u_hi, bn.u_lo, idx8, u);
+#pragma unroll
+    for (int j = 0; j < 8; ++j) {
+        s0[j] += g[j];
+        s1[j] = fmaf(g[j], (u[j] - s_mu[j]) * s_is[j], s1[j]);
+    }
+}
+
+template <bool BN>
+__global__ void __launch_bounds__(kBnBwdThreads) maxpool_bwd_kernel(const uint8_t* __restrict__ arg_in, const bf16* __restrict__ g_hi,
+                                                                  const bf16* __restrict__ g_lo, bf16* __restrict__ dx_hi,
+                                                                  bf16* __restrict__ dx_lo, int B, int H, int W, int C, BnBwdFeed bn) {
     pdl_ew_entry();
     const int cg = C / 8, Ho = H / 2, Wo = W / 2;
     const long total = (long)B * H * W * cg;
+    float s0[8] = {}, s1[8] = {}, mu[8], is[8];
+    if (BN) {
+        const int c0 = (int)(((long)blockIdx.x * blockDim.x + threadIdx.x) % cg) * 8;
+#pragma unroll
+        for (int j = 0; j < 8; ++j) {
+            mu[j] = __ldg(bn.mean + c0 + j);
+            is[j] = __ldg(bn.invstd + c0 + j);
+        }
+    }
     for (long idx = blockIdx.x * (long)blockDim.x + threadIdx.x; idx < total; idx += (long)gridDim.x * blockDim.x) {
         const Pix px = decode_pix(idx, cg, W, H);
         const int g = px.g, ix = px.x, iy = px.y, b = px.b;
@@ -341,8 +399,10 @@
                 if (aj == code) acc[j] += gv[j];
             }
         }
+        if (BN) bn_feed_accum(bn, idx, mu, is, acc, s0, s1);
         store8(dx_hi, dx_lo, idx, acc);
     }
+    if (BN) bn_sums_block_flush(s0, s1, C, bn.sums, bn.part);
 }
 
 __global__ void upsample2x_fwd_kernel(const bf16* __restrict__ x_hi, const bf16* __restrict__ x_lo, bf16* __restrict__ y_hi,
@@ -370,12 +430,23 @@
     }
 }
 
-__global__ void upsample2x_bwd_kernel(const bf16* __restrict__ g_hi, const bf16* __restrict__ g_lo, bf16* __restrict__ dx_hi,
-                                      bf16* __restrict__ dx_lo, int B, int H, int W, int C) {
+template <bool BN>
+__global__ void __launch_bounds__(kBnBwdThreads) upsample2x_bwd_kernel(const bf16* __restrict__ g_hi, const bf16* __restrict__ g_lo,
+                                                                     bf16* __restrict__ dx_hi, bf16* __restrict__ dx_lo, int B, int H,
+                                                                     int W, int C, BnBwdFeed bn) {
     pdl_ew_entry();
     const int cg = C / 8, Ho = 2 * H, Wo = 2 * W;
     const float sh = (float)(H - 1) / (float)(Ho - 1), sw = (float)(W - 1) / (float)(Wo - 1);
     const long total = (long)B * H * W * cg;
+    float s0[8] = {}, s1[8] = {}, mu[8], is[8];
+    if (BN) {
+        const int c0 = (int)(((long)blockIdx.x * blockDim.x + threadIdx.x) % cg) * 8;
+#pragma unroll
+        for (int j = 0; j < 8; ++j) {
+            mu[j] = __ldg(bn.mean + c0 + j);
+            is[j] = __ldg(bn.invstd + c0 + j);
+        }
+    }
     for (long idx = blockIdx.x * (long)blockDim.x + threadIdx.x; idx < total; idx += (long)gridDim.x * blockDim.x) {
         const Pix px = decode_pix(idx, cg, W, H);
         const int g = px.g, ix = px.x, iy = px.y, b = px.b;
@@ -430,8 +501,10 @@
                 }
             }
         }
+        if (BN) bn_feed_accum(bn, idx, mu, is, acc, s0, s1);
         store8(dx_hi, dx_lo, idx, acc);
     }
+    if (BN) bn_sums_block_flush(s0, s1, C, bn.sums, bn.part);
 }
 
 __global__ void zero_insert_kernel(const bf16* __restrict__ x_hi, const bf16* __restrict__ x_lo, bf16* __restrict__ y_hi,
@@ -464,7 +537,6 @@
     }
 }
 
-constexpr int kBnBwdThreads = 256;
 constexpr int kRedRows = 4;
 
 template <bool LO>
@@ -515,7 +587,6 @@
     const int g = threadIdx.x % cg;
     const int rl = threadIdx.x / cg;
     __shared__ __align__(16) float s_mu[512], s_is[512], s_sc[512], s_sh[512];
-    __shared__ float red[2][kBnBwdThreads][8 + 1];
     for (int c = threadIdx.x; c < C; c += kBnBwdThreads) {
         s_mu[c] = mean[c];
         s_is[c] = invstd[c];
@@ -572,20 +643,7 @@
             }
         }
     }
-#pragma unroll
-    for (int j = 0; j < 8; ++j) {
-        red[0][threadIdx.x][j] = s0[j];
-        red[1][threadIdx.x][j] = s1[j];
-    }
-    __syncthreads();
-    for (int t = threadIdx.x; t < 2 * C; t += kBnBwdThreads) {
-        const int which = t / C, c = t % C;
-        const int gg = c / 8, j = c % 8;
-        float a = 0.f;
-        for (int q = 0; q < rpb; ++q) a += red[which][q * cg + gg][j];
-        if (partial_out != nullptr) partial_out[((long)blockIdx.x * 2 + which) * C + c] = a;
-        else atomicAdd(sums + which * C + c, a);
-    }
+    bn_sums_block_flush(s0, s1, C, sums, partial_out);
 }
 
 template <bool LO>
@@ -629,6 +687,12 @@
     double a = 0.0;
     for (int p = 0; p < nparts; ++p) a += (double)partials[(long)p * n + i];
     out[i] = (float)a;
+}
+int launch_sum_partials(const float* partials, int nparts, int n, float* out, cudaStream_t stream) {
+    sum_partials_kernel<<<(n + 255) / 256, 256, 0, stream>>>(partials, nparts, n, out);
+    GDRN_CUDA_OK(cudaGetLastError());
+    count_launch();
+    return 0;
 }
 
 template <bool LO, bool MASKU>
@@ -1057,12 +1121,37 @@
         CBF(x_hi), CBF(x_lo), BF(y_hi), BF(y_lo), reinterpret_cast<uint8_t*>(arg_out), B, H, W, C);
     LAUNCH_DONE();
 }
-extern "C" int gdrn_maxpool_bwd(const void* arg_in, const void* g_hi, const void* g_lo, void* dx_hi, void* dx_lo, int B,
-                                int H, int W, int C, void* stream_) {
-    STREAM;
-    GDRN_LAUNCH_PDL(maxpool_bwd_kernel, ew_grid((long)B * H * W * (C / 8), 256), 256, 0, stream, 
-        reinterpret_cast<const uint8_t*>(arg_in), CBF(g_hi), CBF(g_lo), BF(dx_hi), BF(dx_lo), B, H, W, C);
-    LAUNCH_DONE();
+static int bn_feed_args(BnBwdFeed& bn, const void* mask, const void* u_hi, const void* u_lo, const float* mean, const float* invstd,
+                        float* sums, float* det_ws, int C, long total, int* grid, const char* who) {
+    bn = BnBwdFeed{reinterpret_cast<const uint8_t*>(mask), CBF(u_hi), CBF(u_lo), mean, invstd, sums, det_ws};
+    *grid = ew_grid(total, 256);
+    if (u_hi == nullptr) return 0;
+    if (sums == nullptr || mean == nullptr || invstd == nullptr)
+        return set_error(GDRN_ERR_ARG, "%s: BatchNorm-backward sums need sums, mean and invstd", who);
+    if (C % 64 || C > 512 || 256 % (C / 8)) return set_error(GDRN_ERR_ARG, "%s: BatchNorm-backward sums need C in {64, 128, 256, 512}", who);
+    if (det_ws != nullptr && *grid > 2 * num_sms()) *grid = 2 * num_sms();
+    return 0;
+}
+
+extern "C" int gdrn_maxpool_bwd_bn(const void* arg_in, const void* g_hi, const void* g_lo, void* dx_hi, void* dx_lo, int B,
+                                int H, int W, int C, const void* bn_mask, const void* bn_u_hi, const void* bn_u_lo,
+                                const float* bn_mean, const float* bn_invstd, float* bn_sums, float* det_ws, void* stream_) {
+    STREAM;
+    BnBwdFeed bn;
+    int grid;
+    if (int rc = bn_feed_args(bn, bn_mask, bn_u_hi, bn_u_lo, bn_mean, bn_invstd, bn_sums, det_ws, C, (long)B * H * W * (C / 8), &grid,
+                              "maxpool_bwd"))
+        return rc;
+    if (bn_u_hi != nullptr)
+        GDRN_LAUNCH_PDL(maxpool_bwd_kernel<true>, grid, 256, 0, stream, reinterpret_cast<const uint8_t*>(arg_in), CBF(g_hi), CBF(g_lo),
+                        BF(dx_hi), BF(dx_lo), B, H, W, C, bn);
+    else
+        GDRN_LAUNCH_PDL(maxpool_bwd_kernel<false>, grid, 256, 0, stream, reinterpret_cast<const uint8_t*>(arg_in), CBF(g_hi), CBF(g_lo),
+                        BF(dx_hi), BF(dx_lo), B, H, W, C, bn);
+    GDRN_CUDA_OK(cudaGetLastError());
+    count_launch();
+    if (bn_u_hi != nullptr && det_ws != nullptr) return launch_sum_partials(det_ws, grid, 2 * C, bn_sums, stream);
+    return 0;
 }
 extern "C" int gdrn_upsample2x_fwd(const void* x_hi, const void* x_lo, void* y_hi, void* y_lo, int B, int H, int W, int C,
                                    void* stream_) {
@@ -1071,12 +1160,33 @@
                                                                                            BF(y_lo), B, H, W, C);
     LAUNCH_DONE();
 }
+extern "C" int gdrn_upsample2x_bwd_bn(const void* g_hi, const void* g_lo, void* dx_hi, void* dx_lo, int B, int H, int W, int C,
+                                   const void* bn_mask, const void* bn_u_hi, const void* bn_u_lo, const float* bn_mean,
+                                   const float* bn_invstd, float* bn_sums, float* det_ws, void* stream_) {
+    STREAM;
+    BnBwdFeed bn;
+    int grid;
+    if (int rc = bn_feed_args(bn, bn_mask, bn_u_hi, bn_u_lo, bn_mean, bn_invstd, bn_sums, det_ws, C, (long)B * H * W * (C / 8), &grid,
+                              "upsample2x_bwd"))
+        return rc;
+    if (bn_u_hi != nullptr)
+        GDRN_LAUNCH_PDL(upsample2x_bwd_kernel<true>, grid, 256, 0, stream, CBF(g_hi), CBF(g_lo), BF(dx_hi), BF(dx_lo), B, H, W, C, bn);
+    else
+        GDRN_LAUNCH_PDL(upsample2x_bwd_kernel<false>, grid, 256, 0, stream, CBF(g_hi), CBF(g_lo), BF(dx_hi), BF(dx_lo), B, H, W, C, bn);
+    GDRN_CUDA_OK(cudaGetLastError());
+    count_launch();
+    if (bn_u_hi != nullptr && det_ws != nullptr) return launch_sum_partials(det_ws, grid, 2 * C, bn_sums, stream);
+    return 0;
+}
+extern "C" int gdrn_maxpool_bwd(const void* arg_in, const void* g_hi, const void* g_lo, void* dx_hi, void* dx_lo, int B,
+                                int H, int W, int C, void* stream) {
+    return gdrn_maxpool_bwd_bn(arg_in, g_hi, g_lo, dx_hi, dx_lo, B, H, W, C, nullptr, nullptr, nullptr, nullptr, nullptr, nullptr,
+                               nullptr, stream);
+}
 extern "C" int gdrn_upsample2x_bwd(const void* g_hi, const void* g_lo, void* dx_hi, void* dx_lo, int B, int H, int W, int C,
-                                   void* stream_) {
-    STREAM;
-    GDRN_LAUNCH_PDL(upsample2x_bwd_kernel, ew_grid((long)B * H * W * (C / 8), 256), 256, 0, stream, CBF(g_hi), CBF(g_lo), BF(dx_hi),
-                                                                                       BF(dx_lo), B, H, W, C);
-    LAUNCH_DONE();
+                                   void* stream) {
+    return gdrn_upsample2x_bwd_bn(g_hi, g_lo, dx_hi, dx_lo, B, H, W, C, nullptr, nullptr, nullptr, nullptr, nullptr, nullptr, nullptr,
+                                  stream);
 }
 extern "C" int gdrn_zero_insert(const void* x_hi, const void* x_lo, void* y_hi, void* y_lo, int B, int H, int W, int C,
                                 int mode, void* stream_) {
@@ -1098,7 +1208,7 @@
     if (C % 64 || C > 512) return set_error(GDRN_ERR_ARG, "bn_bwd: unsupported C=%d", C);
     const int mask_u = flags & 1;
     if (mask_u && (y_hi != nullptr || beta == nullptr)) return set_error(GDRN_ERR_ARG, "bn_bwd: mask-from-u needs beta and no y");
-    {
+    if (!(flags & 8)) {
         if (!(flags & 2) && !det) GDRN_CUDA_OK(cudaMemsetAsync(sums, 0, sizeof(float) * 2 * C, stream));
         const int rpb = kBnBwdThreads / (C / 8);
         long blocks = (rows + (long)rpb * 16 - 1) / ((long)rpb * 16);
diff --git a/gdr_net_b200/csrc/gdrn_internal.h b/gdr_net_b200/csrc/gdrn_internal.h
--- a/gdr_net_b200/csrc/gdrn_internal.h
+++ b/gdr_net_b200/csrc/gdrn_internal.h
@@ -19,6 +19,7 @@
 bool pdl_enabled();
 bool pdl_ew_enabled(bool forward_kernel);
 void set_pdl(int on);
+int launch_sum_partials(const float* partials, int nparts, int n, float* out, cudaStream_t stream);
 
 int make_tmap(CUtensorMap* out, const void* base, int rank, const uint64_t* dims, const uint64_t* strides_bytes,
               const uint32_t* box);
diff --git a/gdr_net_b200/csrc/gemm_epilogue.cuh b/gdr_net_b200/csrc/gemm_epilogue.cuh
--- a/gdr_net_b200/csrc/gemm_epilogue.cuh
+++ b/gdr_net_b200/csrc/gemm_epilogue.cuh
@@ -13,6 +13,7 @@
     const long mrow = (long)m_tile * 128 + row;
     const bool row_ok = mrow < p.M;
     const bool all_rows = (long)(m_tile + 1) * 128 <= p.M;
+    const bool bn_bwd = p.bn_u_hi != nullptr;
     long grow = mrow;
     if (p.nphase) {
         const long j = mrow & ((1L << p.pw_log2) - 1);
@@ -46,6 +47,19 @@
             }
         }
         const bool full_chunk = (col0 + 32 <= p.N);
+        uint4 uh[4];
+        uint32_t bits = 0xffffffffu;
+        if (bn_bwd) {
+            const long e = grow * p.ldc + col0;
+#pragma unroll
+            for (int j = 0; j < 4; ++j) uh[j] = make_uint4(0, 0, 0, 0);
+            if (row_ok) {
+                const uint4* uq = reinterpret_cast<const uint4*>(reinterpret_cast<const __nv_bfloat16*>(p.bn_u_hi) + e);
+#pragma unroll
+                for (int j = 0; j < 4; ++j) uh[j] = __ldg(uq + j);
+                if (p.bn_mask != nullptr) bits = __ldg(reinterpret_cast<const uint32_t*>(p.bn_mask + e / 8));
+            }
+        }
         if (p.bias != nullptr) {
 #pragma unroll
             for (int j = 0; j < 32; ++j)
@@ -78,6 +92,10 @@
                 }
             }
         }
+        if (bn_bwd) {
+#pragma unroll
+            for (int j = 0; j < 32; ++j) f[j] = ((bits >> j) & 1u) ? f[j] : 0.f;
+        }
         if (p.act == 1) {
 #pragma unroll
             for (int j = 0; j < 32; ++j) f[j] = f[j] > 0.f ? f[j] : 0.1f * f[j];
@@ -123,7 +141,63 @@
                 }
             }
         }
-        if (p.stats != nullptr) {
+        if (bn_bwd) {
+#pragma unroll
+            for (int h = 0; h < 2; ++h) {
+#pragma unroll
+                for (int j = 0; j < 16; ++j) tr[lane * 17 + j] = row_ok ? f[h * 16 + j] : 0.f;
+                __syncwarp();
+                const int col = lane & 15, r0 = (lane >> 4) * 16;
+                float gc[16];
+#pragma unroll
+                for (int i = 0; i < 16; ++i) gc[i] = tr[(r0 + i) * 17 + col];
+                __syncwarp();
+#pragma unroll
+                for (int k = 0; k < 2; ++k) {
+                    const uint4 q = uh[2 * h + k];
+                    const uint32_t w[4] = {q.x, q.y, q.z, q.w};
+                    float uv[8];
+#pragma unroll
+                    for (int t = 0; t < 4; ++t) unpack_hi2(w[t], uv[2 * t], uv[2 * t + 1]);
+                    if (p.bn_u_lo != nullptr && row_ok) {
+                        const uint4 q2 = __ldg(reinterpret_cast<const uint4*>(reinterpret_cast<const __nv_bfloat16*>(p.bn_u_lo) +
+                                                                             grow * p.ldc + col0) + 2 * h + k);
+                        const uint32_t w2[4] = {q2.x, q2.y, q2.z, q2.w};
+#pragma unroll
+                        for (int t = 0; t < 4; ++t) {
+                            float a, b;
+                            unpack_lo2(w2[t], a, b);
+                            uv[2 * t] += a;
+                            uv[2 * t + 1] += b;
+                        }
+                    }
+#pragma unroll
+                    for (int t = 0; t < 8; ++t) tr[lane * 17 + k * 8 + t] = uv[t];
+                }
+                __syncwarp();
+                const int gcol = col0 + h * 16 + col;
+                const float mu = __ldg(p.bn_mean + gcol), is = __ldg(p.bn_invstd + gcol);
+                float s1 = 0.f, s2 = 0.f;
+#pragma unroll
+                for (int i = 0; i < 16; ++i) {
+                    s1 += gc[i];
+                    s2 = fmaf(gc[i], (tr[(r0 + i) * 17 + col] - mu) * is, s2);
+                }
+                s1 += __shfl_xor_sync(0xffffffffu, s1, 16);
+                s2 += __shfl_xor_sync(0xffffffffu, s2, 16);
+                __syncwarp();
+                if (lane < 16) {
+                    if (p.bn_part != nullptr) {
+                        const long part = ((long)ph * p.num_m_tiles + m_tile) * 4 + (row >> 5);
+                        p.bn_part[part * 2 * p.N + gcol] = s1;
+                        p.bn_part[(part * 2 + 1) * p.N + gcol] = s2;
+                    } else {
+                        atomicAdd(&s_stats[c * 32 + h * 16 + lane], s1);
+                        atomicAdd(&s_stats[BLOCK_N + c * 32 + h * 16 + lane], s2);
+                    }
+                }
+            }
+        } else if (p.stats != nullptr) {
 #pragma unroll
             for (int h = 0; h < 2; ++h) {
                 if (all_rows) {
diff --git a/gdr_net_b200/csrc/gemm_fwd.cu b/gdr_net_b200/csrc/gemm_fwd.cu
--- a/gdr_net_b200/csrc/gemm_fwd.cu
+++ b/gdr_net_b200/csrc/gemm_fwd.cu
@@ -373,6 +373,42 @@
     return (num_m_tiles / 2) * num_n_tiles * 4 >= num_sms();
 }
 
+struct BnBwdArgs {
+    const void* mask;
+    const void* u_hi;
+    const void* u_lo;
+    const float* mean;
+    const float* invstd;
+    float* sums;
+    float* part;
+    long part_floats;
+    int nparts;
+};
+
+static int set_bn_bwd(GemmParams& p, BnBwdArgs& bn, const char* who) {
+    if (bn.u_hi == nullptr) return 0;
+    if (bn.sums == nullptr || bn.mean == nullptr || bn.invstd == nullptr)
+        return set_error(GDRN_ERR_ARG, "%s: a BatchNorm-backward epilogue needs sums, mean and invstd", who);
+    if (p.N % 64 != 0 || p.ldc != p.N || p.out_hi == nullptr || p.out_f32 != nullptr || p.bias != nullptr || p.act != 0)
+        return set_error(GDRN_ERR_ARG, "%s: a BatchNorm-backward epilogue needs N %% 64 == 0, ldc == N, 16-bit output only, no bias / act", who);
+    bn.nparts = (p.nphase ? p.nphase : 1) * p.num_m_tiles * 4;
+    if (bn.part != nullptr && bn.part_floats < (long)bn.nparts * 2 * p.N)
+        return set_error(GDRN_ERR_ARG, "%s: deterministic BatchNorm-backward workspace needs %ld floats", who, (long)bn.nparts * 2 * p.N);
+    p.bn_mask = reinterpret_cast<const uint8_t*>(bn.mask);
+    p.bn_u_hi = bn.u_hi;
+    p.bn_u_lo = bn.u_lo;
+    p.bn_mean = bn.mean;
+    p.bn_invstd = bn.invstd;
+    p.bn_part = bn.part;
+    p.stats = bn.part != nullptr ? nullptr : bn.sums;
+    return 0;
+}
+
+static int finish_bn_bwd(int rc, const GemmParams& p, const BnBwdArgs& bn, cudaStream_t stream) {
+    if (rc != 0 || bn.u_hi == nullptr || bn.part == nullptr) return rc;
+    return launch_sum_partials(bn.part, bn.nparts, 2 * p.N, bn.sums, stream);
+}
+
 }
 
 using namespace gdrn;
@@ -383,10 +419,11 @@
 }
 extern "C" long gdrn_2cta_launch_count() { return gdrn::g_2cta_launches.load(); }
 
-extern "C" int gdrn_conv_fwd(const void* x_hi, const void* x_lo, const void* w_hi, const void* w_lo, void* y_hi,
+extern "C" int gdrn_conv_fwd_bn(const void* x_hi, const void* x_lo, const void* w_hi, const void* w_lo, void* y_hi,
                              void* y_lo, float* y_f32, const float* bias, const void* res_hi, const void* res_lo, float* stats,
                              int N, int H, int W, int Cin, int Cout, int Cout_pad, int KH, int KW, int stride, int pad, int ldc,
-                             int act, int nsplit, void* stream_) {
+                             int act, int nsplit, const void* bn_mask, const void* bn_u_hi, const void* bn_u_lo,
+                             const float* bn_mean, const float* bn_invstd, float* bn_part, long bn_part_floats, void* stream_) {
     cudaStream_t stream = reinterpret_cast<cudaStream_t>(stream_);
     if (nsplit != 1 && nsplit != 3) return set_error(GDRN_ERR_ARG, "conv_fwd: nsplit must be 1 or 3");
     if (nsplit == 3 && (x_lo == nullptr || w_lo == nullptr)) return set_error(GDRN_ERR_ARG, "conv_fwd: lo planes missing");
@@ -452,23 +489,30 @@
     p.res_lo = res_lo;
     p.act = act;
     p.stats = stats;
+    BnBwdArgs bn = {bn_mask, bn_u_hi, bn_u_lo, bn_mean, bn_invstd, stats, bn_part, bn_part_floats, 0};
+    if (int rc = set_bn_bwd(p, bn, "conv_fwd")) return rc;
     if (two_cta) {
         g_2cta_launches.fetch_add(1, std::memory_order_relaxed);
         g_last_variant = 10000 + block_n * 10 + nsplit;
-        return launch_gemm_2cta(p, block_n, nsplit, stream);
-    }
-    return dispatch_gemm(p, block_n, nsplit, stream);
-}
-
-extern "C" int gdrn_conv_dgrad_s2(const void* du_hi, const void* du_lo, const void* w_hi, const void* w_lo, void* dx_hi,
-                                  void* dx_lo, const float* bias, float* stats, int N, int Ho, int Wo, int Cy, int Cx, int Cx_pad,
-                                  int K, int pad, int ldc, int act, int nsplit, void* stream_) {
+        return finish_bn_bwd(launch_gemm_2cta(p, block_n, nsplit, stream), p, bn, stream);
+    }
+    return finish_bn_bwd(dispatch_gemm(p, block_n, nsplit, stream), p, bn, stream);
+}
+
+extern "C" int gdrn_conv_dgrad_s2_bn(const void* du_hi, const void* du_lo, const void* w_hi, const void* w_lo, void* dx_hi,
+                                  void* dx_lo, const float* bias, const void* res_hi, const void* res_lo, float* stats, int N, int Ho,
+                                  int Wo, int Cy, int Cx, int Cx_pad, int K, int pad, int ldc, int act, int nsplit,
+                                  const void* bn_mask, const void* bn_u_hi, const void* bn_u_lo, const float* bn_mean,
+                                  const float* bn_invstd, float* bn_part, long bn_part_floats, void* stream_) {
     cudaStream_t stream = reinterpret_cast<cudaStream_t>(stream_);
     if (nsplit != 1 && nsplit != 3) return set_error(GDRN_ERR_ARG, "conv_dgrad_s2: nsplit must be 1 or 3");
     if (nsplit == 3 && (du_lo == nullptr || w_lo == nullptr)) return set_error(GDRN_ERR_ARG, "conv_dgrad_s2: lo planes missing");
     if (!((K == 3 && pad == 1) || (K == 1 && pad == 0))) return set_error(GDRN_ERR_ARG, "conv_dgrad_s2: k3 p1 or k1 p0 only");
     if (Cy % 64 != 0) return set_error(GDRN_ERR_ARG, "conv_dgrad_s2: Cy=%d must be a multiple of 64", Cy);
     if (ldc % 8 != 0 || ldc < Cx) return set_error(GDRN_ERR_ARG, "conv_dgrad_s2: bad ldc=%d", ldc);
+    if (res_hi != nullptr && (Cx % 32 != 0 || K != 3))
+        return set_error(GDRN_ERR_ARG, "conv_dgrad_s2: a residual needs Cx %% 32 == 0 and k = 3 (every output pixel written)");
+    if (bn_u_hi != nullptr && K != 3) return set_error(GDRN_ERR_ARG, "conv_dgrad_s2: a BatchNorm-backward epilogue needs k = 3");
     if (Wo > 128 || 128 % Wo != 0 || (Ho & (Ho - 1)) != 0) return set_error(GDRN_ERR_ARG, "conv_dgrad_s2: unsupported dY size %dx%d", Ho, Wo);
     int TH = 128 / Wo;
     if (TH > Ho) TH = Ho;
@@ -511,6 +555,8 @@
     p.out_hi = dx_hi;
     p.out_lo = dx_lo;
     p.ldc = ldc;
+    p.res_hi = res_hi;
+    p.res_lo = res_lo;
     p.bias = bias;
     p.act = act;
     p.stats = stats;
@@ -537,12 +583,15 @@
     p.num_kb = nt * p.cchunks;
     for (p.pw_log2 = 0; (1 << p.pw_log2) < Wo; ++p.pw_log2) {}
     for (p.ph_log2 = 0; (1 << p.ph_log2) < Ho; ++p.ph_log2) {}
-    return dispatch_gemm(p, block_n, nsplit, stream);
-}
-
-extern "C" int gdrn_gemm_fwd(const void* a_hi, const void* a_lo, const void* w_hi, const void* w_lo, void* y_hi,
+    BnBwdArgs bn = {bn_mask, bn_u_hi, bn_u_lo, bn_mean, bn_invstd, stats, bn_part, bn_part_floats, 0};
+    if (int rc = set_bn_bwd(p, bn, "conv_dgrad_s2")) return rc;
+    return finish_bn_bwd(dispatch_gemm(p, block_n, nsplit, stream), p, bn, stream);
+}
+
+extern "C" int gdrn_gemm_fwd_bn(const void* a_hi, const void* a_lo, const void* w_hi, const void* w_lo, void* y_hi,
                              void* y_lo, float* y_f32, const float* bias, float* stats, int M, int N, int N_pad, int K,
-                             int ldc, int act, int nsplit, void* stream_) {
+                             int ldc, int act, int nsplit, const void* bn_mask, const void* bn_u_hi, const void* bn_u_lo,
+                             const float* bn_mean, const float* bn_invstd, float* bn_part, long bn_part_floats, void* stream_) {
     cudaStream_t stream = reinterpret_cast<cudaStream_t>(stream_);
     if (nsplit != 1 && nsplit != 3) return set_error(GDRN_ERR_ARG, "gemm_fwd: nsplit must be 1 or 3");
     if (nsplit == 3 && (a_lo == nullptr || w_lo == nullptr)) return set_error(GDRN_ERR_ARG, "gemm_fwd: lo planes missing");
@@ -579,7 +628,29 @@
     p.bias = bias;
     p.act = act;
     p.stats = stats;
-    return dispatch_gemm(p, block_n, nsplit, stream);
+    BnBwdArgs bn = {bn_mask, bn_u_hi, bn_u_lo, bn_mean, bn_invstd, stats, bn_part, bn_part_floats, 0};
+    if (int rc = set_bn_bwd(p, bn, "gemm_fwd")) return rc;
+    return finish_bn_bwd(dispatch_gemm(p, block_n, nsplit, stream), p, bn, stream);
+}
+
+extern "C" int gdrn_conv_fwd(const void* x_hi, const void* x_lo, const void* w_hi, const void* w_lo, void* y_hi,
+                             void* y_lo, float* y_f32, const float* bias, const void* res_hi, const void* res_lo, float* stats,
+                             int N, int H, int W, int Cin, int Cout, int Cout_pad, int KH, int KW, int stride, int pad, int ldc,
+                             int act, int nsplit, void* stream) {
+    return gdrn_conv_fwd_bn(x_hi, x_lo, w_hi, w_lo, y_hi, y_lo, y_f32, bias, res_hi, res_lo, stats, N, H, W, Cin, Cout, Cout_pad, KH,
+                            KW, stride, pad, ldc, act, nsplit, nullptr, nullptr, nullptr, nullptr, nullptr, nullptr, 0, stream);
+}
+extern "C" int gdrn_conv_dgrad_s2(const void* du_hi, const void* du_lo, const void* w_hi, const void* w_lo, void* dx_hi,
+                                  void* dx_lo, const float* bias, float* stats, int N, int Ho, int Wo, int Cy, int Cx, int Cx_pad,
+                                  int K, int pad, int ldc, int act, int nsplit, void* stream) {
+    return gdrn_conv_dgrad_s2_bn(du_hi, du_lo, w_hi, w_lo, dx_hi, dx_lo, bias, nullptr, nullptr, stats, N, Ho, Wo, Cy, Cx, Cx_pad, K,
+                                 pad, ldc, act, nsplit, nullptr, nullptr, nullptr, nullptr, nullptr, nullptr, 0, stream);
+}
+extern "C" int gdrn_gemm_fwd(const void* a_hi, const void* a_lo, const void* w_hi, const void* w_lo, void* y_hi,
+                             void* y_lo, float* y_f32, const float* bias, float* stats, int M, int N, int N_pad, int K,
+                             int ldc, int act, int nsplit, void* stream) {
+    return gdrn_gemm_fwd_bn(a_hi, a_lo, w_hi, w_lo, y_hi, y_lo, y_f32, bias, stats, M, N, N_pad, K, ldc, act, nsplit, nullptr,
+                            nullptr, nullptr, nullptr, nullptr, nullptr, 0, stream);
 }
 
 extern "C" int gdrn_last_gemm_variant() { return g_last_variant; }
diff --git a/gdr_net_b200/csrc/gemm_params.h b/gdr_net_b200/csrc/gemm_params.h
--- a/gdr_net_b200/csrc/gemm_params.h
+++ b/gdr_net_b200/csrc/gemm_params.h
@@ -27,6 +27,12 @@
     signed char tap_dh[12], tap_dw[12], tap_w[12];
     int pw_log2, ph_log2;
     int no_split_epi;
+    const uint8_t* bn_mask;
+    const void* bn_u_hi;
+    const void* bn_u_lo;
+    const float* bn_mean;
+    const float* bn_invstd;
+    float* bn_part;
 };
 
 
diff --git a/gdr_net_b200/engine.py b/gdr_net_b200/engine.py
--- a/gdr_net_b200/engine.py
+++ b/gdr_net_b200/engine.py
@@ -12,9 +12,7 @@
 
 _DGRAD_ZERO_INSERT = os.environ.get("GDRN_DGRAD_ZERO_INSERT") == "1"
 
-_BN_MASK_FROM_U = os.environ.get("GDRN_BN_MASK_FROM_U") == "1"
 _DECONV_PHASES = os.environ.get("GDRN_DECONV_PHASES", "1") == "1"
-_BN_BITMASK = os.environ.get("GDRN_BN_BITMASK", "1") == "1"
 
 LOSS_NAMES = ["loss_coor_x", "loss_coor_y", "loss_coor_z", "loss_mask", "loss_region", "loss_PM_R", "loss_centroid", "loss_z"]
 HEAD_CONVS = [(3, 4, False), (6, 7, False), (10, 11, True), (13, 14, False), (17, 18, True), (20, 21, False)]
@@ -94,6 +92,7 @@
         self._side_stream, self._side_keep = None, []
         self.deterministic = os.environ.get("GDRN_DETERMINISTIC") == "1"
         self._det_ws = None
+        self._bn_part_ws = None
         self.fold_eval = os.environ.get("GDRN_NO_FOLD_EVAL") != "1"
         self.with_2d = int(model.pnp_net.features[0].in_channels == 69)
         assert model.pnp_net.features[0].in_channels in (67, 69), model.pnp_net.features[0].in_channels
@@ -389,7 +388,7 @@
             C.gdrn_bn_stats(u.hi_ptr, u.lo_ptr, self._det_workspace().data_ptr(), st.stats.data_ptr(), count, Cc, _stream())
         y = ops.like(u)
         mask = None
-        if relu and getattr(self, "_want_masks", False) and _BN_BITMASK:
+        if relu and getattr(self, "_want_masks", False):
             mask = torch.empty(u.numel() // 8, dtype=torch.uint8, device=self.dev)
         self._last_mask = mask
         C.gdrn_bn_fwd(u.hi_ptr, u.lo_ptr, res.hi_ptr if res else None, res.lo_ptr if res else None, y.hi_ptr, y.lo_ptr,
@@ -616,20 +615,32 @@
 
         self._on_side(work, keep=(du, x_in))
 
-    def _dgrad_conv(self, du: PT, conv, wkey: str) -> PT:
+    def _dgrad_conv(self, du: PT, conv, wkey: str, res: Optional[PT] = None, bn: Optional[ops.BnFeed] = None) -> PT:
         k, stride, pad = conv.kernel_size[0], conv.stride[0], conv.padding[0]
         if stride == 2 and not _DGRAD_ZERO_INSERT:
-            return ops.conv_dgrad_s2(du, self.wd[wkey], conv.in_channels, k, pad)
+            return ops.conv_dgrad_s2(du, self.wd[wkey], conv.in_channels, k, pad, res=res, bn=bn)
         z = ops.zero_insert(du) if stride == 2 else du
-        return ops.conv_fwd(z, self.wd[wkey], conv.in_channels, k, k, 1, k - 1 - pad, algo_scale=0.25 if stride == 2 else 1.0)
-
-    def _bn_bwd(self, bkey: str, ga: PT, gb: Optional[PT], y: Optional[PT], u: PT, want_gout=False, relu_from_u=False, mask=None):
+        return ops.conv_fwd(z, self.wd[wkey], conv.in_channels, k, k, 1, k - 1 - pad, algo_scale=0.25 if stride == 2 else 1.0,
+                            res=res, bn=bn)
+
+    def _bn_feed(self, bkey: str, mask, u: PT) -> ops.BnFeed:
+        st = self.bn[bkey]
+        if self.deterministic and self._bn_part_ws is None:
+            self._bn_part_ws = ops.Workspace(self.dev)
+        return ops.BnFeed(mask, u, st.mean, st.invstd, st.sums, self._bn_part_ws if self.deterministic else None)
+
+    def _bn_apply(self, bkey: str, g: PT, u: PT) -> PT:
         mod, st = self._bn_mods[bkey], self.bn[bkey]
-        relu_from_u = relu_from_u and _BN_MASK_FROM_U and mask is None
-        return ops.bn_bwd(ga, gb, None if (relu_from_u or mask is not None) else y, u, st.mean, st.invstd, mod.weight, st.sums,
-                          self.grads[bkey + ".weight"], self.grads[bkey + ".bias"], self.saved["train_bn"], want_gout=want_gout,
-                          beta=mod.bias, relu_from_u=relu_from_u, sums_zeroed=True, relu_mask=mask,
-                          det_ws=self._det_workspace() if self.deterministic else None)
+        du, _ = ops.bn_bwd(g, None, None, u, st.mean, st.invstd, mod.weight, st.sums, self.grads[bkey + ".weight"],
+                           self.grads[bkey + ".bias"], self.saved["train_bn"], apply_only=True)
+        return du
+
+    def _bn_bwd_reduce_apply(self, bkey: str, g: PT, u: PT) -> PT:
+        mod, st = self._bn_mods[bkey], self.bn[bkey]
+        du, _ = ops.bn_bwd(g, None, None, u, st.mean, st.invstd, mod.weight, st.sums, self.grads[bkey + ".weight"],
+                           self.grads[bkey + ".bias"], self.saved["train_bn"], sums_zeroed=True,
+                           det_ws=self._det_workspace() if self.deterministic else None)
+        return du
 
     def backward(self, grad_losses: torch.Tensor):
         S, m, dev = self.saved, self.model, self.dev
@@ -692,17 +703,22 @@
         tmp128 = torch.empty(128, device=dev)
         C.gdrn_colsum(dlog.hi_ptr, dlog.lo_ptr, tmp128.data_ptr(), B * 4096, 128, _stream())
         self.grads["rot_head_net.features.23.bias"].copy_(tmp128[:69])
-        g = ops.gemm_fwd(dlog, self.wd["rot_head_net.features.23"], 256).view(B, 64, 64, 256)
-
-        for L in reversed(S["head"]):
+        heads = S["head"]
+        D = S["deconv"]
+        feeds = [self._bn_feed("rot_head_net.features.1", D["m"], h(D["u"]))]
+        feeds += [self._bn_feed(f"rot_head_net.features.{L['bi']}", L["m"], h(L["u"])) for L in heads]
+        g = ops.gemm_fwd(dlog, self.wd["rot_head_net.features.23"], 256, bn=feeds[-1]).view(B, 64, 64, 256)
+
+        for i in reversed(range(len(heads))):
+            L = heads[i]
             ci, bi = L["ci"], L["bi"]
-            du, _ = self._bn_bwd(f"rot_head_net.features.{bi}", g, None, h(L["y"]), h(L["u"]), relu_from_u=True, mask=L["m"])
+            du = self._bn_apply(f"rot_head_net.features.{bi}", g, h(L["u"]))
             self._wgrad_conv(du, h(L["x_in"]), hf[ci], f"rot_head_net.features.{ci}.weight")
-            g = self._dgrad_conv(du, hf[ci], f"rot_head_net.features.{ci}")
             if L["up"]:
-                g = ops.upsample2x_bwd(g)
-        D = S["deconv"]
-        du, _ = self._bn_bwd("rot_head_net.features.1", g, None, h(D["y"]), h(D["u"]), relu_from_u=True, mask=D["m"])
+                g = ops.upsample2x_bwd(self._dgrad_conv(du, hf[ci], f"rot_head_net.features.{ci}"), bn=feeds[i])
+            else:
+                g = self._dgrad_conv(du, hf[ci], f"rot_head_net.features.{ci}", bn=feeds[i])
+        du = self._bn_apply("rot_head_net.features.1", g, h(D["u"]))
         def deconv_wgrad(du=du):
             if _DECONV_PHASES:
                 buf, ks, kss = ops.conv_wgrad(h(D["z"]), du, self.ws, 512, 3, 3, 2, 1)
@@ -712,31 +728,35 @@
             ops.unpack_wgrad(buf, self.grads["rot_head_net.features.0.weight"], 256, 512, 3, 3, 512, ks, kss, 9, 256 * 9, 3, 1, flip=1)
 
         self._on_side(deconv_wgrad, keep=(du,))
-        g = ops.conv_fwd(du, self.wd["deconv"], 512, 3, 3, 2, 1)
+        blocks = S["blocks"]
+
+        def bn2_feed(i):
+            return self._bn_feed(blocks[i]["p"] + ".bn2", blocks[i]["m2"], h(blocks[i]["u2"]))
+
+        g = ops.conv_fwd(du, self.wd["deconv"], 512, 3, 3, 2, 1, bn=bn2_feed(len(blocks) - 1))
         self._segment_done("rot_head_net")
 
-        ga, gb = g, None
-        for Lb in reversed(S["blocks"]):
+        for i in reversed(range(len(blocks))):
+            Lb = blocks[i]
             p, blk = Lb["p"], Lb["blk"]
-            du2, gout = self._bn_bwd(p + ".bn2", ga, gb, h(Lb["out"]), h(Lb["u2"]), want_gout=True, mask=Lb["m2"])
+            du2 = self._bn_apply(p + ".bn2", g, h(Lb["u2"]))
             self._wgrad_conv(du2, h(Lb["a1"]), blk.conv2, p + ".conv2.weight")
-            da1 = self._dgrad_conv(du2, blk.conv2, p + ".conv2")
-            du1, _ = self._bn_bwd(p + ".bn1", da1, None, h(Lb["a1"]), h(Lb["u1"]), relu_from_u=True, mask=Lb["m1"])
+            da1 = self._dgrad_conv(du2, blk.conv2, p + ".conv2", bn=self._bn_feed(p + ".bn1", Lb["m1"], h(Lb["u1"])))
+            du1 = self._bn_apply(p + ".bn1", da1, h(Lb["u1"]))
             self._wgrad_conv(du1, h(Lb["x_in"]), blk.conv1, p + ".conv1.weight")
-            dx_main = self._dgrad_conv(du1, blk.conv1, p + ".conv1")
+            nxt = bn2_feed(i - 1) if i > 0 else None
             if blk.downsample is not None:
-                dud, _ = self._bn_bwd(p + ".downsample.1", gout, None, None, h(Lb["ud"]))
+                dud = self._bn_bwd_reduce_apply(p + ".downsample.1", g, h(Lb["ud"]))
                 self._wgrad_conv(dud, h(Lb["x_in"]), blk.downsample[0], p + ".downsample.0.weight")
-                dx_ds = self._dgrad_conv(dud, blk.downsample[0], p + ".downsample.0")
-                ga, gb = dx_main, dx_ds
+                skip = self._dgrad_conv(dud, blk.downsample[0], p + ".downsample.0")
             else:
-                ga, gb = dx_main, gout
+                skip = g
+            g = self._dgrad_conv(du1, blk.conv1, p + ".conv1", res=skip, bn=nxt)
             if p.endswith(".0") and not p.startswith("backbone.layer1"):
                 self._segment_done(p[:-2])
-        g_pool = ops.add2(ga, gb)
         St = S["stem"]
-        g_a0 = ops.maxpool_bwd(St["pool_arg"], g_pool)
-        du0, _ = self._bn_bwd("backbone.bn1", g_a0, None, h(St["a0"]), h(St["u0"]), relu_from_u=True, mask=St["m0"])
+        g_a0 = ops.maxpool_bwd(St["pool_arg"], g, bn=self._bn_feed("backbone.bn1", St["m0"], h(St["u0"])))
+        du0 = self._bn_apply("backbone.bn1", g_a0, h(St["u0"]))
         def stem_wgrad():
             buf, ks, kss = ops.gemm_wgrad(du0.view(B * 128 * 128, 64), h(St["a_col"]), self.ws)
             ops.unpack_wgrad(buf, self.grads["backbone.conv1.weight"], 64, 3, 7, 7, 3, ks, kss, 147, 49, 7, 1, krow=192)
diff --git a/gdr_net_b200/ops.py b/gdr_net_b200/ops.py
--- a/gdr_net_b200/ops.py
+++ b/gdr_net_b200/ops.py
@@ -178,40 +178,68 @@
     return out
 
 
+class BnFeed:
+
+    __slots__ = ("mask", "u", "mean", "invstd", "sums", "det_ws")
+
+    def __init__(self, mask, u: "PT", mean, invstd, sums, det_ws=None):
+        self.mask, self.u, self.mean, self.invstd, self.sums, self.det_ws = mask, u, mean, invstd, sums, det_ws
+
+
+def _gemm_bn_args(bn: BnFeed | None, rows: int, Cout: int, nphase: int = 1):
+    if bn is None:
+        return (None, None, None, None, None, None, 0)
+    part, nfl = None, 0
+    if bn.det_ws is not None:
+        nfl = nphase * 4 * -(-rows // 128) * 2 * Cout
+        part = bn.det_ws.get(nfl).data_ptr()
+    return (ptr(bn.mask), bn.u.hi_ptr, bn.u.lo_ptr, bn.mean.data_ptr(), bn.invstd.data_ptr(), part, nfl)
+
+
+def _gather_bn_args(bn: BnFeed | None, Cc: int):
+    if bn is None:
+        return (None, None, None, None, None, None, None)
+    det = bn.det_ws.get(2 * Cc * int(C.load().gdrn_det_parts())).data_ptr() if bn.det_ws is not None else None
+    return (ptr(bn.mask), bn.u.hi_ptr, bn.u.lo_ptr, bn.mean.data_ptr(), bn.invstd.data_ptr(), bn.sums.data_ptr(), det)
+
+
 def conv_fwd(x: PT, wp: PT, Cout: int, KH: int, KW: int, stride: int, pad: int, *, out: PT | None = None,
              out_f32: torch.Tensor | None = None, bias=None, stats=None, act: int = 0, ldc: int | None = None,
-             want_planes: bool = True, algo_scale: float = 1.0, res: PT | None = None) -> PT | None:
+             want_planes: bool = True, algo_scale: float = 1.0, res: PT | None = None, bn: BnFeed | None = None) -> PT | None:
     N, H, W, Cin = x.shape
     Ho, Wo = H // stride, W // stride
     ldc = ldc or _round_up(Cout, 64)
     if want_planes and out is None:
         out = PT((N, Ho, Wo, ldc), x.planes, device=x.buf.device, zero=(ldc != Cout))
-    C.gdrn_conv_fwd(x.hi_ptr, x.lo_ptr, wp.hi_ptr, wp.lo_ptr, out.hi_ptr if out is not None else None,
+    C.gdrn_conv_fwd_bn(x.hi_ptr, x.lo_ptr, wp.hi_ptr, wp.lo_ptr, out.hi_ptr if out is not None else None,
                     out.lo_ptr if out is not None else None, ptr(out_f32), ptr(bias), res.hi_ptr if res is not None else None,
-                    res.lo_ptr if res is not None else None, ptr(stats), N, H, W, Cin, Cout, wp.shape[0], KH, KW, stride, pad,
-                    ldc, act, x.nsplit, _stream())
-    return out
-
-
-def conv_dgrad_s2(du: PT, wd: PT, Cx: int, K: int, pad: int, *, out: PT | None = None, bias=None, stats=None, act: int = 0) -> PT:
+                    res.lo_ptr if res is not None else None, ptr(bn.sums if bn is not None else stats), N, H, W, Cin, Cout,
+                    wp.shape[0], KH, KW, stride, pad, ldc, act, x.nsplit, *_gemm_bn_args(bn, N * Ho * Wo, Cout), _stream())
+    return out
+
+
+def conv_dgrad_s2(du: PT, wd: PT, Cx: int, K: int, pad: int, *, out: PT | None = None, bias=None, stats=None, act: int = 0,
+                  res: PT | None = None, bn: BnFeed | None = None) -> PT:
     N, Ho, Wo, Cy = du.shape
     ldc = _round_up(Cx, 64)
     if out is None:
         out = PT((N, 2 * Ho, 2 * Wo, ldc), du.planes, device=du.buf.device, zero=(K == 1 or ldc != Cx))
-    C.gdrn_conv_dgrad_s2(du.hi_ptr, du.lo_ptr, wd.hi_ptr, wd.lo_ptr, out.hi_ptr, out.lo_ptr, ptr(bias), ptr(stats), N, Ho, Wo, Cy, Cx,
-                         wd.shape[0], K, pad, ldc, act, du.nsplit, _stream())
+    C.gdrn_conv_dgrad_s2_bn(du.hi_ptr, du.lo_ptr, wd.hi_ptr, wd.lo_ptr, out.hi_ptr, out.lo_ptr, ptr(bias),
+                         res.hi_ptr if res is not None else None, res.lo_ptr if res is not None else None,
+                         ptr(bn.sums if bn is not None else stats), N, Ho, Wo, Cy, Cx, wd.shape[0], K, pad, ldc, act, du.nsplit,
+                         *_gemm_bn_args(bn, N * Ho * Wo, Cx, 4 if K == 3 else 1), _stream())
     return out
 
 
 def gemm_fwd(a: PT, wp: PT, N: int, *, out: PT | None = None, out_f32: torch.Tensor | None = None, bias=None, stats=None,
-             act: int = 0, ldc: int | None = None, want_planes: bool = True) -> PT | None:
+             act: int = 0, ldc: int | None = None, want_planes: bool = True, bn: BnFeed | None = None) -> PT | None:
     M, K = a.shape
     ldc = ldc or _round_up(N, 64)
     if want_planes and out is None:
         out = PT((M, ldc), a.planes, device=a.buf.device, zero=(ldc != N))
-    C.gdrn_gemm_fwd(a.hi_ptr, a.lo_ptr, wp.hi_ptr, wp.lo_ptr, out.hi_ptr if out is not None else None,
-                    out.lo_ptr if out is not None else None, ptr(out_f32), ptr(bias), ptr(stats), M, N, wp.shape[0], K, ldc,
-                    act, a.nsplit, _stream())
+    C.gdrn_gemm_fwd_bn(a.hi_ptr, a.lo_ptr, wp.hi_ptr, wp.lo_ptr, out.hi_ptr if out is not None else None,
+                    out.lo_ptr if out is not None else None, ptr(out_f32), ptr(bias), ptr(bn.sums if bn is not None else stats), M, N,
+                    wp.shape[0], K, ldc, act, a.nsplit, *_gemm_bn_args(bn, M, N), _stream())
     return out
 
 
@@ -277,7 +305,8 @@
 
 
 def bn_bwd(ga: PT, gb: PT | None, y: PT | None, u: PT, mean, invstd, gamma, sums, dgamma, dbeta, train: bool,
-           want_gout: bool = False, beta=None, relu_from_u: bool = False, sums_zeroed: bool = False, relu_mask=None, det_ws=None):
+           want_gout: bool = False, beta=None, relu_from_u: bool = False, sums_zeroed: bool = False, relu_mask=None, det_ws=None,
+           apply_only: bool = False):
     du = like(u)
     gout = like(u) if want_gout else None
     Cc = u.shape[-1]
@@ -287,7 +316,8 @@
                   u.hi_ptr, u.lo_ptr, mean.data_ptr(), invstd.data_ptr(), gamma.data_ptr(), ptr(beta), sums.data_ptr(), du.hi_ptr,
                   du.lo_ptr, gout.hi_ptr if gout else None, gout.lo_ptr if gout else None, ptr(dgamma), ptr(dbeta), ptr(relu_mask),
                   ptr(det_ws), rows, Cc, int(train),
-                  (1 if relu_from_u else 0) | (2 if sums_zeroed else 0) | (4 if det_ws is not None else 0), _stream())
+                  (1 if relu_from_u else 0) | (2 if sums_zeroed else 0) | (4 if det_ws is not None else 0) | (8 if apply_only else 0),
+                  _stream())
     return du, gout
 
 
@@ -299,10 +329,11 @@
     return (out, arg) if want_arg else out
 
 
-def maxpool_bwd(arg: torch.Tensor, g: PT) -> PT:
+def maxpool_bwd(arg: torch.Tensor, g: PT, bn: BnFeed | None = None) -> PT:
     B, Ho, Wo, Cc = g.shape
     out = like(g, (B, 2 * Ho, 2 * Wo, Cc))
-    C.gdrn_maxpool_bwd(arg.data_ptr(), g.hi_ptr, g.lo_ptr, out.hi_ptr, out.lo_ptr, B, 2 * Ho, 2 * Wo, Cc, _stream())
+    C.gdrn_maxpool_bwd_bn(arg.data_ptr(), g.hi_ptr, g.lo_ptr, out.hi_ptr, out.lo_ptr, B, 2 * Ho, 2 * Wo, Cc, *_gather_bn_args(bn, Cc),
+                       _stream())
     return out
 
 
@@ -313,10 +344,10 @@
     return out
 
 
-def upsample2x_bwd(g: PT) -> PT:
+def upsample2x_bwd(g: PT, bn: BnFeed | None = None) -> PT:
     B, Ho, Wo, Cc = g.shape
     out = like(g, (B, Ho // 2, Wo // 2, Cc))
-    C.gdrn_upsample2x_bwd(g.hi_ptr, g.lo_ptr, out.hi_ptr, out.lo_ptr, B, Ho // 2, Wo // 2, Cc, _stream())
+    C.gdrn_upsample2x_bwd_bn(g.hi_ptr, g.lo_ptr, out.hi_ptr, out.lo_ptr, B, Ho // 2, Wo // 2, Cc, *_gather_bn_args(bn, Cc), _stream())
     return out
 
 
diff --git a/include/gdrn_b200.h b/include/gdrn_b200.h
--- a/include/gdrn_b200.h
+++ b/include/gdrn_b200.h
@@ -25,14 +25,28 @@
                   float* y_f32, const float* bias, const void* res_hi, const void* res_lo, float* stats, int N, int H, int W,
                   int Cin, int Cout, int Cout_pad, int KH, int KW, int stride, int pad, int ldc, int act, int nsplit,
                   void* stream);
+int gdrn_conv_fwd_bn(const void* x_hi, const void* x_lo, const void* w_hi, const void* w_lo, void* y_hi, void* y_lo,
+                  float* y_f32, const float* bias, const void* res_hi, const void* res_lo, float* stats, int N, int H, int W,
+                  int Cin, int Cout, int Cout_pad, int KH, int KW, int stride, int pad, int ldc, int act, int nsplit,
+                  const void* bn_mask, const void* bn_u_hi, const void* bn_u_lo, const float* bn_mean, const float* bn_invstd,
+                  float* bn_part, long bn_part_floats, void* stream);
 
 int gdrn_conv_dgrad_s2(const void* du_hi, const void* du_lo, const void* w_hi, const void* w_lo, void* dx_hi, void* dx_lo,
                        const float* bias, float* stats, int N, int Ho, int Wo, int Cy, int Cx, int Cx_pad, int K, int pad, int ldc,
                        int act, int nsplit, void* stream);
+int gdrn_conv_dgrad_s2_bn(const void* du_hi, const void* du_lo, const void* w_hi, const void* w_lo, void* dx_hi, void* dx_lo,
+                       const float* bias, const void* res_hi, const void* res_lo, float* stats, int N, int Ho, int Wo, int Cy,
+                       int Cx, int Cx_pad, int K, int pad, int ldc, int act, int nsplit, const void* bn_mask, const void* bn_u_hi,
+                       const void* bn_u_lo, const float* bn_mean, const float* bn_invstd, float* bn_part, long bn_part_floats,
+                       void* stream);
 
 int gdrn_gemm_fwd(const void* a_hi, const void* a_lo, const void* w_hi, const void* w_lo, void* y_hi, void* y_lo,
                   float* y_f32, const float* bias, float* stats, int M, int N, int N_pad, int K, int ldc, int act,
                   int nsplit, void* stream);
+int gdrn_gemm_fwd_bn(const void* a_hi, const void* a_lo, const void* w_hi, const void* w_lo, void* y_hi, void* y_lo,
+                  float* y_f32, const float* bias, float* stats, int M, int N, int N_pad, int K, int ldc, int act,
+                  int nsplit, const void* bn_mask, const void* bn_u_hi, const void* bn_u_lo, const float* bn_mean,
+                  const float* bn_invstd, float* bn_part, long bn_part_floats, void* stream);
 
 int gdrn_conv_wgrad(const void* dy_hi, const void* dy_lo, const void* x_hi, const void* x_lo, float* ws, long ws_floats,
                     long* ws_need_out, int* ksplit_out, int N, int H, int W, int Cin, int Cout, int KH, int KW,
@@ -68,8 +82,14 @@
                      void* stream);
 int gdrn_maxpool_bwd(const void* arg_in, const void* g_hi, const void* g_lo, void* dx_hi, void* dx_lo, int B, int H, int W,
                      int C, void* stream);
+int gdrn_maxpool_bwd_bn(const void* arg_in, const void* g_hi, const void* g_lo, void* dx_hi, void* dx_lo, int B, int H, int W,
+                     int C, const void* bn_mask, const void* bn_u_hi, const void* bn_u_lo, const float* bn_mean,
+                     const float* bn_invstd, float* bn_sums, float* det_ws, void* stream);
 int gdrn_upsample2x_fwd(const void* x_hi, const void* x_lo, void* y_hi, void* y_lo, int B, int H, int W, int C, void* stream);
 int gdrn_upsample2x_bwd(const void* g_hi, const void* g_lo, void* dx_hi, void* dx_lo, int B, int H, int W, int C, void* stream);
+int gdrn_upsample2x_bwd_bn(const void* g_hi, const void* g_lo, void* dx_hi, void* dx_lo, int B, int H, int W, int C,
+                        const void* bn_mask, const void* bn_u_hi, const void* bn_u_lo, const float* bn_mean,
+                        const float* bn_invstd, float* bn_sums, float* det_ws, void* stream);
 int gdrn_zero_insert(const void* x_hi, const void* x_lo, void* y_hi, void* y_lo, int B, int H, int W, int C, int mode,
                      void* stream);
 int gdrn_gn_relu_fwd(const void* u_hi, const void* u_lo, void* y_hi, void* y_lo, const float* gamma, const float* beta,
```
